# samson6460/tf2_YOLO

Hardware: AMD Instinct MI355X
Metric: images/sec training YOLOv3 416x416 bs=32/GPU (higher is better)
Workload: dtype f32-storage/fp16x2-mfma

## Files before the change

### include/yolo_hip.h

```cpp
#ifndef YOLO_HIP_H_
#define YOLO_HIP_H_

#include <stddef.h>
#include <stdint.h>

#ifdef __cplusplus
extern "C" {
#endif

typedef enum yolo_status {
  YOLO_OK = 0,
  YOLO_ERR_INVALID_ARG = -1,
  YOLO_ERR_LAUNCH = -2,
  YOLO_ERR_WORKSPACE = -3
} yolo_status;

enum { YOLO_ACT_LINEAR = 0, YOLO_ACT_LEAKY = 1, YOLO_ACT_MISH = 2 };
enum { YOLO_HEAD_V3 = 3, YOLO_HEAD_V2 = 2, YOLO_HEAD_V1 = 1, YOLO_HEAD_V4 = 4 };
enum { YOLO_NMS_HARD = 1, YOLO_NMS_SOFT = 2, YOLO_NMS_DIOU = 3 };

const char* yolo_last_error(void);
int yolo_abi_version(void);
int yolo_device_available(void);
int yolo_mfma_probe(const void* operands_f16, float* sink, int workgroups, int iters, double* flops_host, void* stream);
// ... 8 lines not shown
int yolo_set_debug_buffer(void* p, size_t bytes);

typedef struct yolo_conv_desc {
  int N, H, W, Cin;
  int Cout, kh, kw;
  int Ho, Wo;
  int sh, sw;
  int pad_t, pad_l;
} yolo_conv_desc;

#define YOLO_BN_STAT_SLOTS 64
#define YOLO_BN_RED_SLOTS 512
#define YOLO_SPLIT_BATCH_UNITS 4

int yolo_conv2d_fwd(const yolo_conv_desc* d, const float* x, const float* w,
                    const float* bias, float* y, double* stats, void* stream);
int yolo_conv2d_fwd_absmax(const yolo_conv_desc* d, const float* x, const float* w, const float* bias,
                           float* y, double* stats, unsigned* absmax, void* stream);

int yolo_conv2d_dgrad(const yolo_conv_desc* d, const float* dy, const float* wT,
                      float* dx, int accumulate, void* stream);

int yolo_conv2d_wgrad(const yolo_conv_desc* d, const float* x, const float* dy,
                      float* dw, float* dbias, void* stream);

int yolo_conv2d_wgrad_bias(const float* dy, long long P, int Cout, float* dbias, void* stream);

int yolo_filter_transpose(const float* w, float* wT, int Cout, int taps, int Cin, void* stream);

size_t yolo_planes_bytes(long long rows, int C);
int yolo_split_planes(const float* x, long long rows, int C, void* planes, void* stream);
int yolo_split_planes_padded(const float* x, long long rows, int C_src, int C, void* planes, void* stream);

int yolo_split_planes_batch(const void* jobs, int njobs, long long total_blocks, void* stream);
int yolo_filter_transpose_batch(const void* jobs, int njobs, long long total_blocks, void* stream);

int yolo_conv2d_fwd_planes(const yolo_conv_desc* d, const void* x_planes, const void* w_planes,
                           const float* bias, float* y, double* stats, unsigned* absmax, void* stream);
int yolo_conv2d_dgrad_planes(const yolo_conv_desc* d, const void* dy_planes, const void* wT_planes,
                             float* dx, int accumulate, void* stream);
enum { YOLO_EPI_NONE = 0, YOLO_EPI_AFFINE = 1, YOLO_EPI_AFFINE_LEAKY = 2, YOLO_EPI_AFFINE_MISH = 3 };
int yolo_conv2d_fwd_planes_epi(const yolo_conv_desc* d, const void* x_planes, const void* w_planes, const float* bias,
                               int epilogue, const float* scale, const float* shift, const float* residual, float* y,
                               unsigned* absmax, void* stream);
int yolo_split_planes_absmax(const float* x, long long rows, int C, const unsigned* absmax, const float* extra_bound,
                             void* planes, float* out_bound, void* stream);
#define YOLO_INFER_BOUND_WORDS 4096
int yolo_conv_pred_bound(const float* w, int Cout, int kdim, const float* scale, const float* shift, const float* bias,
                         float* pred2, void* stream);
int yolo_conv2d_fwd_infer_unit(const yolo_conv_desc* d, const void* x_planes, const void* w_planes, const float* bias,
                               int epilogue, const float* scale, const float* shift, const float* residual, float* y,
                               unsigned* absmax, const float* pred2, const void* in_bound, int in_n,
                               const void* residual_bound, int residual_n, void* out_planes, unsigned* out_words,
                               float* out_bound, int* out_n_host, void* stream);
int yolo_fold_bound(const void* words, int n, float* out_bound, void* stream);
int yolo_absmax_words(const float* x, long long n, unsigned* words, int* n_words_host, void* stream);
int yolo_stem_filter_prep(const float* w, const float* bias, float* wt, void* stream);
int yolo_stem_fwd_infer_unit(const yolo_conv_desc* d, const float* x, const float* wt, int epilogue, const float* scale,
                             const float* shift, const float* pred2, const void* in_bound, int in_n, float* y,
                             void* out_planes, unsigned* out_words, int* out_n_host, void* stream);
int yolo_split_planes_concat(const float* const* srcs_host, const int* channels_host, const float* const* bounds_host,
                             int nsrc, long long rows, void* planes, float* dst32, float* out_bound, void* stream);
int yolo_split_planes_concat_ex(const float* const* srcs_host, const int* channels_host, const float* const* bounds_host,
                                const int* bound_words_host, const int* upsample_host, int H, int W, int nsrc,
                                long long rows, void* planes, float* dst32, float* out_bound, void* stream);
int yolo_conv2d_fwd_head_unit(const yolo_conv_desc* d, const void* x_planes, const void* w_planes, const float* bias,
                              int A, int C, int version, const float* anchors, float* t, float* y, void* stream);
enum { YOLO_PREC_F32 = 0, YOLO_PREC_F16 = 1 };
int yolo_conv2d_fwd_planes_ex(const yolo_conv_desc* d, const void* x_planes, const void* w_planes, const float* bias,
                              float* y, double* stats, unsigned* absmax, int precision, void* stream);
int yolo_conv2d_fwd_planes_epi_ex(const yolo_conv_desc* d, const void* x_planes, const void* w_planes, const float* bias,
                                  int epilogue, const float* scale, const float* shift, const float* residual, float* y,
                                  unsigned* absmax, int precision, void* stream);
int yolo_conv2d_fwd_infer_unit_ex(const yolo_conv_desc* d, const void* x_planes, const void* w_planes, const float* bias,
                                  int epilogue, const float* scale, const float* shift, const float* residual, float* y,
                                  unsigned* absmax, const float* pred2, const void* in_bound, int in_n,
                                  const void* residual_bound, int residual_n, void* out_planes, unsigned* out_words,
                                  float* out_bound, int* out_n_host, int precision, void* stream);
int yolo_conv2d_fwd_head_unit_ex(const yolo_conv_desc* d, const void* x_planes, const void* w_planes, const float* bias,
                                 int A, int C, int version, const float* anchors, float* t, float* y, int precision,
                                 void* stream);
int yolo_conv2d_wgrad_planes(const yolo_conv_desc* d, const void* x_planes, const void* dy_planes,
                             float* dw, void* stream);

size_t yolo_wgrad_workspace_bytes(void);
int yolo_set_wgrad_workspace(void* p, size_t bytes);


int yolo_bn_stats(const float* x, long long P, int C, double* stats, void* stream);

int yolo_bn_finalize(double* stats, long long P, int C, const float* gamma, const float* beta,
                     float eps, float momentum, int unbiased_moving_var,
                     float* moving_mean, float* moving_var,
                     float* scale, float* shift, float* save_mean, float* save_invstd,
                     void* stream);

int yolo_bn_fold_inference(int C, const float* gamma, const float* beta,
                           const float* moving_mean, const float* moving_var, float eps,
                           float* scale, float* shift, void* stream);

int yolo_bn_act_fwd(const float* x, long long P, int C, const float* scale, const float* shift,
                    int act, const float* residual, float* out, void* stream);

int yolo_bn_act_bwd_reduce(const float* x, const float* dout, long long P, int C,
                           const float* scale, const float* shift,
                           const float* save_mean, const float* save_invstd,
                           int act, double* red, void* stream);
int yolo_bn_act_bwd_apply(const float* x, const float* dout, long long P, int C,
                          const float* gamma, const float* scale, const float* shift,
                          const float* save_mean, const float* save_invstd,
                          int act, double* red, float* dgamma, float* dbeta,
                          float* dx, void* stream);

int yolo_bn_finalize_bound(double* stats, long long P, int C, const float* gamma, const float* beta, float eps,
                           float momentum, int unbiased_moving_var, float* moving_mean, float* moving_var,
                           float* scale, float* shift, float* save_mean, float* save_invstd,
                           const unsigned* absmax, unsigned* bound, void* stream);
int yolo_bn_finalize_offset(double* stats, long long P, int C, const float* gamma, const float* beta, float eps,
                            float momentum, int unbiased_moving_var, float* moving_mean, float* moving_var, float* scale,
                            float* shift, float* save_mean, float* save_invstd, const unsigned* absmax, unsigned* bound,
                            const float* mean_offset, void* stream);
int yolo_bn_infer_bound(int C, const float* scale, const float* shift, const unsigned* absmax,
                        unsigned* bound, void* stream);
int yolo_bn_act_fwd_planes(const float* x, long long P, int C, const float* scale, const float* shift,
                           int act, const float* residual, float* out, void* planes,
                           const unsigned* bn_bound, const float* residual_bound, float* out_bound,
                           void* stream);
int yolo_bn_act_maxpool2x2_fwd(const float* y, int N, int Ho, int Wo, int C, const float* scale, const float* shift,
                               int act, float* out, int* argmax, void* planes, const unsigned* bn_bound,
                               float* out_bound, void* stream);
int yolo_bn_act_fwd_res_planes(const float* x, long long P, int C, const float* scale, const float* shift, int act,
                               const void* residual_planes, float* out, void* planes, const unsigned* bn_bound,
                               float* out_bound, void* stream);
int yolo_bn_act_bwd_reduce_bound(const float* x, const float* dout, long long P, int C, const float* scale,
                                 const float* shift, const float* save_mean, const float* save_invstd,
                                 int act, double* red, unsigned* bound_aux, void* stream);
size_t yolo_stem_bwd_scratch_bytes(void);
int yolo_stem_bn_bwd_wgrad(const yolo_conv_desc* d, const float* y, const float* dout, const float* image, const float* scale,
                           const float* shift, const float* save_mean, const float* save_invstd, int act, const double* red,
                           float* dgamma, float* dbeta, float* dw, void* scratch, size_t scratch_bytes, void* stream);
int yolo_bn_act_bwd_apply_planes(const float* x, const float* dout, long long P, int C, const float* gamma,
                                 const float* scale, const float* shift, const float* save_mean,
                                 const float* save_invstd, int act, double* red, float* dgamma, float* dbeta,
                                 float* dx, void* planes, const unsigned* bound_aux, void* stream);
int yolo_bn_act_bwd_reduce_bound_ld(const float* x, const float* dout, long long ld_dout, long long P, int C,
                                    const float* scale, const float* shift, const float* save_mean,
                                    const float* save_invstd, int act, double* red, unsigned* bound_aux, void* stream);
#define YOLO_BN_FOLD_TICKET_WORDS 36
int yolo_bn_act_bwd_reduce_fold_ld(const float* x, const float* dout, long long ld_dout, long long P, int C,
                                   const float* scale, const float* shift, const float* save_mean,
                                   const float* save_invstd, int act, double* red, unsigned* bound_aux,
                                   unsigned* tickets, void* stream);
int yolo_bn_act_bwd_apply_planes_ld(const float* x, const float* dout, long long ld_dout, long long P, int C,
                                    const float* gamma, const float* scale, const float* shift, const float* save_mean,
                                    const float* save_invstd, int act, double* red, float* dgamma, float* dbeta,
                                    float* dx, void* planes, const unsigned* bound_aux, void* stream);

int yolo_bnred_slots_cap(const yolo_conv_desc* d);
int yolo_conv2d_dgrad_planes_bnred(const yolo_conv_desc* d, const void* dy_planes, const void* wT_planes, float* dx,
                                   int accumulate, const float* y, const float* scale, const float* shift,
                                   const float* save_mean, const float* save_invstd, int act, float* partials,
                                   int slots_cap, unsigned* bound_aux, int* nslots, void* stream);
int yolo_bn_act_bwd_sum_partials(const float* partials, int nslots, long long P, int C, const float* scale, double* red,
                                 unsigned* bound_aux, void* stream);

int yolo_act_fwd(const float* x, long long n, int act, float* out, void* stream);
int yolo_act_bwd(const float* x, const float* dout, long long n, int act, float* dx, void* stream);

int yolo_copy_channels_in(const float* src, long long P, int Csrc, float* dst, int Cdst,
                          int c_off, void* stream);
int yolo_copy_channels_out(const float* src, long long P, int Csrc, int c_off, float* dst,
                           int Cdst, int accumulate, void* stream);
int yolo_upsample2x_fwd(const float* x, int N, int H, int W, int C, float* y, int Cy, int c_off,
                        void* stream);
int yolo_upsample2x_bwd(const float* dy, int N, int H, int W, int C, int Cy, int c_off, float* dx,
                        int accumulate, void* stream);
int yolo_axpy(float* a, const float* b, long long n, void* stream);
int yolo_maxpool_fwd(const float* x, int N, int H, int W, int C, int k, int s, int pad_t, int pad_l,
                     int Ho, int Wo, float* y, int Cy, int c_off, int* argmax, void* stream);
int yolo_maxpool_bwd(const float* dy, int N, int Ho, int Wo, int C, int Cy, int c_off,
                     const int* argmax, float* dx, void* stream);
int yolo_maxpool_bwd_same(const float* dy, int N, int H, int W, int C, int Cy, int c_off, const int* argmax, int k,
                          int pad_t, int pad_l, float* dx, void* stream);
int yolo_maxpool2x2_bwd(const float* dy, int N, int Ho, int Wo, int C, const int* argmax, float* dx, int accumulate,
                        void* stream);
int yolo_space_to_depth2_fwd(const float* x, int N, int H, int W, int C, float* y, int Cy, int c_off,
                             void* stream);
int yolo_space_to_depth2_bwd(const float* dy, int N, int H, int W, int C, int Cy, int c_off, float* dx,
                             int accumulate, void* stream);

int yolo_head_act_fwd(const float* t, long long P, int A, int C, int version,
                      const float* anchors, float* y, void* stream);
int yolo_head_act_bwd(const float* y, const float* dy, long long P, int A, int C, int version,
                      const float* anchors, float* dt, float* danchors, void* stream);

typedef struct yolo_loss_cfg {
  int version;
  int N, gh, gw, A, C;
  float anchors[32];
  int   use_anchors;
  float binary_weight;
  float loss_weight[4];
  float ignore_thresh;
  int   use_focal_loss;
  float focal_gamma;
  int   use_scale;
  float wh_reg_weight;
  float truth_thresh;
  float label_smooth;
} yolo_loss_cfg;

size_t yolo_loss_workspace_bytes(const yolo_loss_cfg* cfg);
int yolo_loss_fwd_bwd(const yolo_loss_cfg* cfg, const float* y_true, const float* y_pred,
                      double* loss_out, float* dpred, float grad_scale,
                      void* workspace, size_t workspace_bytes, void* stream);

int yolo_metrics(const yolo_loss_cfg* cfg, const float* y_true, const float* y_pred,
                 float recall_thresh, double* out, void* stream);

int yolo_adam_step(float* p, float* g, float* m, float* v, long long n, float lr, float beta1,
                   float beta2, float eps, int step, float grad_scale, int zero_grad, void* stream);
float yolo_adam_lr_t(float lr, float beta1, float beta2, int step);
int yolo_adam_step_dev(float* p, float* g, float* m, float* v, long long n, const float* hyper, int zero_grad, void* stream);
int yolo_sgd_step(float* p, float* g, long long n, float lr, float grad_scale, int zero_grad,
                  void* stream);
int yolo_fill(float* p, long long n, float value, void* stream);

size_t yolo_grad_sqnorm_workspace_bytes(int n_chunks);
int yolo_grad_sqnorm(const float* g, const long long* chunk_off, const int* chunk_len, int n_chunks,
                     const int* var_first, int n_vars, double* var_sq, double* total_sq, void* workspace,
                     size_t workspace_bytes, void* stream);
int yolo_clip_factors(const double* var_sq, int n_vars, const double* total_sq, const double* total_sq_extra,
                      const float* hyper, int mode, float* factors, float* norm_out, void* stream);
int yolo_adam_step_clip(float* p, float* g, float* m, float* v, float* vhat, const long long* chunk_off,
                        const int* chunk_len, const int* chunk_var, int n_chunks, const float* hyper,
                        const float* factors, int clip_mode, int zero_grad, void* stream);
int yolo_sgd_step_clip(float* p, float* g, float* accum, int nesterov, const long long* chunk_off,
                       const int* chunk_len, const int* chunk_var, int n_chunks, const float* hyper,
                       const float* factors, int clip_mode, int zero_grad, void* stream);

int yolo_decode_level(const float* pred, int gh, int gw, int A, int C, int version,
                      float threshold, double* rows_out, int max_rows, int* count,
                      void* workspace, size_t workspace_bytes, void* stream);
int yolo_decode_level_f64(const double* pred, int gh, int gw, int A, int C, int version,
                          double threshold, double* rows_out, int max_rows, int* count,
                          void* workspace, size_t workspace_bytes, void* stream);
size_t yolo_decode_workspace_bytes(int gh, int gw, int A, int C);

size_t yolo_nms_workspace_bytes(int n, int class_num);
int yolo_nms(const double* rows, int n, int class_num, int mode, double nms_threshold,
             double conf_threshold, double sigma, unsigned char* keep_out,
             void* workspace, size_t workspace_bytes, void* stream);
int yolo_nms_select(const double* rows, int n, int class_num, int mode, double nms_threshold, double conf_threshold,
                    double sigma, unsigned char* keep_out, double* rows_out, int* count_out, void* workspace,
                    size_t workspace_bytes, void* stream);

int yolo_cal_iou(const void* xywh_true, const void* xywh_pred, void* out, void* out2, int is_f64, int mode, int ndim,
                 const long long* shape_host, const long long* true_strides_host, const long long* pred_strides_host,
                 double grid_w, double grid_h, void* stream);


int yolo_match_detections(const double* gt_rows, int ngt, const double* det_rows, int ndet, int class_num,
                          double iou_threshold, int* best_gt, unsigned char* matched, double* best_iou,
                          unsigned char* gt_flags, long long* class_counts, void* stream);

int yolo_rank_desc(const double* key, const int* segment, int n, int* rank, void* stream);

size_t yolo_pr_curve_workspace_bytes(int n, int num_gts);
int yolo_pr_curve(const double* joint, const int* gt_id, const unsigned char* matched, int n, int num_gts,
                  int precision_mode, void* workspace, size_t workspace_bytes, double* precision,
                  double* recall, void* stream);

int yolo_allreduce_bucket(void* rccl_comm, float* grads, long long count, void* stream);

int yolo_encode_labels(const double* boxes, const int* cls, const int* first, int N, double img_h, double img_w,
                       int gh, int gw, int C, double* label64, float* label32, void* stream);
int yolo_down2xlabel(const double* label_in, int N, int gh, int gw, int ch, double* label_out, float* out32,
                     void* stream);

#ifdef __cplusplus
}
#endif
#endif
```

### tf2_yolo_amd/_lib.py

```python
import ctypes
import os
from ctypes import (POINTER, Structure, c_char_p, c_double, c_float, c_int, c_longlong,
                    c_size_t, c_void_p)

from . import tape as _tape

_HERE = os.path.dirname(os.path.abspath(__file__))
LIB_PATH = os.path.join(_HERE, "libyolo_hip.so")

ACT_LINEAR, ACT_LEAKY, ACT_MISH = 0, 1, 2
PREC_F32, PREC_F16 = 0, 1
_PRECISIONS = {"fp32": PREC_F32, "fp16": PREC_F16}


def precision_enum(precision):
    try:
        return _PRECISIONS[precision]
    except (KeyError, TypeError):
        raise ValueError(f"precision must be 'fp32' or 'fp16', got {precision!r}") from None
NMS_HARD, NMS_SOFT, NMS_DIOU = 1, 2, 3


class YoloHipError(RuntimeError):
    pass


class ConvDesc(Structure):
    _fields_ = [(n, c_int) for n in
                ("N", "H", "W", "Cin", "Cout", "kh", "kw", "Ho", "Wo", "sh", "sw", "pad_t", "pad_l")]


class LossCfg(Structure):
    _fields_ = [("version", c_int), ("N", c_int), ("gh", c_int), ("gw", c_int), ("A", c_int),
                ("C", c_int), ("anchors", c_float * 32), ("use_anchors", c_int),
                ("binary_weight", c_float), ("loss_weight", c_float * 4),
                ("ignore_thresh", c_float), ("use_focal_loss", c_int), ("focal_gamma", c_float),
                ("use_scale", c_int), ("wh_reg_weight", c_float), ("truth_thresh", c_float),
                ("label_smooth", c_float)]


_P = c_void_p
_LL = c_longlong
SIGNATURES = {
    "yolo_last_error": (c_char_p, []),
    "yolo_abi_version": (c_int, []),
    "yolo_device_available": (c_int, []),
    "yolo_set_option": (c_int, [c_int, c_int]),
    "yolo_last_conv_kernel": (c_char_p, [POINTER(c_int)]),
    "yolo_mfma_probe": (c_int, [_P, _P, c_int, c_int, POINTER(c_double), _P]),
    "yolo_set_debug_buffer": (c_int, [_P, c_size_t]),
    "yolo_encode_labels": (c_int, [_P, _P, _P, c_int, c_double, c_double, c_int, c_int, c_int, _P, _P, _P]),
    "yolo_down2xlabel": (c_int, [_P, c_int, c_int, c_int, c_int, _P, _P, _P]),
    "yolo_conv_workspace_bytes": (c_size_t, []),
    "yolo_set_conv_workspace": (c_int, [_P, c_size_t, _P]),
    "yolo_conv2d_fwd": (c_int, [POINTER(ConvDesc), _P, _P, _P, _P, _P, _P]),
    "yolo_conv2d_dgrad": (c_int, [POINTER(ConvDesc), _P, _P, _P, c_int, _P]),
    "yolo_conv2d_wgrad": (c_int, [POINTER(ConvDesc), _P, _P, _P, _P, _P]),
    "yolo_conv2d_wgrad_bias": (c_int, [_P, _LL, c_int, _P, _P]),
    "yolo_filter_transpose": (c_int, [_P, _P, c_int, c_int, c_int, _P]),
    "yolo_planes_bytes": (c_size_t, [_LL, c_int]),
    "yolo_split_planes": (c_int, [_P, _LL, c_int, _P, _P]),
    "yolo_split_planes_padded": (c_int, [_P, _LL, c_int, c_int, _P, _P]),
    "yolo_split_planes_batch": (c_int, [_P, c_int, _LL, _P]),
    "yolo_filter_transpose_batch": (c_int, [_P, c_int, _LL, _P]),
    "yolo_conv2d_fwd_planes": (c_int, [POINTER(ConvDesc), _P, _P, _P, _P, _P, _P, _P]),
    "yolo_stem_bwd_scratch_bytes": (c_size_t, []),
    "yolo_stem_bn_bwd_wgrad": (c_int, [POINTER(ConvDesc), _P, _P, _P, _P, _P, _P, _P, c_int, _P, _P, _P, _P, _P, c_size_t, _P]),
    "yolo_conv2d_fwd_planes_epi": (c_int, [POINTER(ConvDesc), _P, _P, _P, c_int, _P, _P, _P, _P, _P, _P]),
    "yolo_split_planes_absmax": (c_int, [_P, _LL, c_int, _P, _P, _P, _P, _P]),
    "yolo_conv_pred_bound": (c_int, [_P, c_int, c_int, _P, _P, _P, _P, _P]),
    "yolo_conv2d_fwd_infer_unit": (c_int, [POINTER(ConvDesc), _P, _P, _P, c_int, _P, _P, _P, _P, _P, _P, _P, c_int, _P, c_int,
                                           _P, _P, _P, POINTER(c_int), _P]),
    "yolo_fold_bound": (c_int, [_P, c_int, _P, _P]),
    "yolo_absmax_words": (c_int, [_P, _LL, _P, POINTER(c_int), _P]),
    "yolo_stem_filter_prep": (c_int, [_P, _P, _P, _P]),
    "yolo_stem_fwd_infer_unit": (c_int, [POINTER(ConvDesc), _P, _P, c_int, _P, _P, _P, _P, c_int, _P, _P, _P, POINTER(c_int), _P]),
    "yolo_split_planes_concat": (c_int, [POINTER(c_void_p), POINTER(c_int), POINTER(c_void_p), c_int, _LL, _P, _P, _P, _P]),
    "yolo_split_planes_concat_ex": (c_int, [POINTER(c_void_p), POINTER(c_int), POINTER(c_void_p), POINTER(c_int), POINTER(c_int),
                                            c_int, c_int, c_int, _LL, _P, _P, _P, _P]),
    "yolo_conv2d_fwd_head_unit": (c_int, [POINTER(ConvDesc), _P, _P, _P, c_int, c_int, c_int, _P, _P, _P, _P]),
    "yolo_conv2d_fwd_planes_ex": (c_int, [POINTER(ConvDesc), _P, _P, _P, _P, _P, _P, c_int, _P]),
    "yolo_conv2d_fwd_planes_epi_ex": (c_int, [POINTER(ConvDesc), _P, _P, _P, c_int, _P, _P, _P, _P, _P, c_int, _P]),
    "yolo_conv2d_fwd_infer_unit_ex": (c_int, [POINTER(ConvDesc), _P, _P, _P, c_int, _P, _P, _P, _P, _P, _P, _P, c_int, _P, c_int,
                                              _P, _P, _P, POINTER(c_int), c_int, _P]),
    "yolo_conv2d_fwd_head_unit_ex": (c_int, [POINTER(ConvDesc), _P, _P, _P, c_int, c_int, c_int, _P, _P, _P, c_int, _P]),
    "yolo_conv2d_fwd_absmax": (c_int, [POINTER(ConvDesc), _P, _P, _P, _P, _P, _P, _P]),
    "yolo_conv2d_dgrad_planes": (c_int, [POINTER(ConvDesc), _P, _P, _P, c_int, _P]),
    "yolo_conv2d_wgrad_planes": (c_int, [POINTER(ConvDesc), _P, _P, _P, _P]),
    "yolo_wgrad_workspace_bytes": (c_size_t, []),
    "yolo_set_wgrad_workspace": (c_int, [_P, c_size_t]),
    "yolo_bn_stats": (c_int, [_P, _LL, c_int, _P, _P]),
    "yolo_bn_finalize": (c_int, [_P, _LL, c_int, _P, _P, c_float, c_float, c_int, _P, _P, _P, _P, _P, _P, _P]),
    "yolo_bn_fold_inference": (c_int, [c_int, _P, _P, _P, _P, c_float, _P, _P, _P]),
    "yolo_bn_act_fwd": (c_int, [_P, _LL, c_int, _P, _P, c_int, _P, _P, _P]),
    "yolo_bn_act_bwd_reduce": (c_int, [_P, _P, _LL, c_int, _P, _P, _P, _P, c_int, _P, _P]),
    "yolo_bn_act_bwd_apply": (c_int, [_P, _P, _LL, c_int, _P, _P, _P, _P, _P, c_int, _P, _P, _P, _P, _P]),
    "yolo_bn_act_fwd_planes": (c_int, [_P, _LL, c_int, _P, _P, c_int, _P, _P, _P, _P, _P, _P, _P]),
    "yolo_bn_act_fwd_res_planes": (c_int, [_P, _LL, c_int, _P, _P, c_int, _P, _P, _P, _P, _P, _P]),
    "yolo_bn_act_bwd_apply_planes": (c_int, [_P, _P, _LL, c_int, _P, _P, _P, _P, _P, c_int, _P, _P, _P, _P, _P, _P,
                                             _P]),
    "yolo_bn_infer_bound": (c_int, [c_int, _P, _P, _P, _P, _P]),
    "yolo_bn_finalize_bound": (c_int, [_P, _LL, c_int, _P, _P, c_float, c_float, c_int, _P, _P, _P, _P, _P, _P, _P,
                                       _P, _P]),
    "yolo_bn_finalize_offset": (c_int, [_P, _LL, c_int, _P, _P, c_float, c_float, c_int, _P, _P, _P, _P, _P, _P, _P,
                                        _P, _P, _P]),
    "yolo_bn_act_bwd_reduce_bound": (c_int, [_P, _P, _LL, c_int, _P, _P, _P, _P, c_int, _P, _P, _P]),
    "yolo_bn_act_bwd_reduce_bound_ld": (c_int, [_P, _P, _LL, _LL, c_int, _P, _P, _P, _P, c_int, _P, _P, _P]),
    "yolo_bn_act_bwd_reduce_fold_ld": (c_int, [_P, _P, _LL, _LL, c_int, _P, _P, _P, _P, c_int, _P, _P, _P, _P]),
    "yolo_bn_act_bwd_apply_planes_ld": (c_int, [_P, _P, _LL, _LL, c_int, _P, _P, _P, _P, _P, c_int, _P, _P, _P, _P, _P, _P,
                                                _P]),
    "yolo_bnred_slots_cap": (c_int, [POINTER(ConvDesc)]),
    "yolo_conv2d_dgrad_planes_bnred": (c_int, [POINTER(ConvDesc), _P, _P, _P, c_int, _P, _P, _P, _P, _P, c_int, _P, c_int, _P,
                                               POINTER(c_int), _P]),
    "yolo_bn_act_bwd_sum_partials": (c_int, [_P, c_int, _LL, c_int, _P, _P, _P, _P]),
    "yolo_allreduce_bucket": (c_int, [_P, _P, _LL, _P]),
    "yolo_act_fwd": (c_int, [_P, _LL, c_int, _P, _P]),
    "yolo_act_bwd": (c_int, [_P, _P, _LL, c_int, _P, _P]),
    "yolo_copy_channels_in": (c_int, [_P, _LL, c_int, _P, c_int, c_int, _P]),
    "yolo_copy_channels_out": (c_int, [_P, _LL, c_int, c_int, _P, c_int, c_int, _P]),
    "yolo_upsample2x_fwd": (c_int, [_P, c_int, c_int, c_int, c_int, _P, c_int, c_int, _P]),
    "yolo_upsample2x_bwd": (c_int, [_P, c_int, c_int, c_int, c_int, c_int, c_int, _P, c_int, _P]),
    "yolo_axpy": (c_int, [_P, _P, _LL, _P]),
    "yolo_maxpool_fwd": (c_int, [_P, c_int, c_int, c_int, c_int, c_int, c_int, c_int, c_int, c_int, c_int,
                                 _P, c_int, c_int, _P, _P]),
    "yolo_maxpool_bwd": (c_int, [_P, c_int, c_int, c_int, c_int, c_int, c_int, _P, _P, _P]),
    "yolo_maxpool2x2_bwd": (c_int, [_P, c_int, c_int, c_int, c_int, _P, _P, c_int, _P]),
    "yolo_bn_act_maxpool2x2_fwd": (c_int, [_P, c_int, c_int, c_int, c_int, _P, _P, c_int, _P, _P, _P, _P, _P, _P]),
    "yolo_maxpool_bwd_same": (c_int, [_P, c_int, c_int, c_int, c_int, c_int, c_int, _P, c_int, c_int, c_int, _P, _P]),
    "yolo_space_to_depth2_fwd": (c_int, [_P, c_int, c_int, c_int, c_int, _P, c_int, c_int, _P]),
    "yolo_space_to_depth2_bwd": (c_int, [_P, c_int, c_int, c_int, c_int, c_int, c_int, _P, c_int, _P]),
    "yolo_head_act_fwd": (c_int, [_P, _LL, c_int, c_int, c_int, _P, _P, _P]),
    "yolo_head_act_bwd": (c_int, [_P, _P, _LL, c_int, c_int, c_int, _P, _P, _P, _P]),
    "yolo_loss_workspace_bytes": (c_size_t, [POINTER(LossCfg)]),
    "yolo_loss_fwd_bwd": (c_int, [POINTER(LossCfg), _P, _P, _P, _P, c_float, _P, c_size_t, _P]),
    "yolo_metrics": (c_int, [POINTER(LossCfg), _P, _P, c_float, _P, _P]),
    "yolo_adam_step": (c_int, [_P, _P, _P, _P, _LL, c_float, c_float, c_float, c_float, c_int, c_float, c_int, _P]),
    "yolo_adam_lr_t": (c_float, [c_float, c_float, c_float, c_int]),
    "yolo_adam_step_dev": (c_int, [_P, _P, _P, _P, _LL, _P, c_int, _P]),
    "yolo_sgd_step": (c_int, [_P, _P, _LL, c_float, c_float, c_int, _P]),
    "yolo_fill": (c_int, [_P, _LL, c_float, _P]),
    "yolo_grad_sqnorm_workspace_bytes": (c_size_t, [c_int]),
    "yolo_grad_sqnorm": (c_int, [_P, _P, _P, c_int, _P, c_int, _P, _P, _P, c_size_t, _P]),
    "yolo_clip_factors": (c_int, [_P, c_int, _P, _P, _P, c_int, _P, _P, _P]),
    "yolo_adam_step_clip": (c_int, [_P, _P, _P, _P, _P, _P, _P, _P, c_int, _P, _P, c_int, c_int, _P]),
    "yolo_sgd_step_clip": (c_int, [_P, _P, _P, c_int, _P, _P, _P, c_int, _P, _P, c_int, c_int, _P]),
    "yolo_decode_level": (c_int, [_P, c_int, c_int, c_int, c_int, c_int, c_float, _P, c_int, _P, _P, c_size_t, _P]),
    "yolo_decode_level_f64": (c_int, [_P, c_int, c_int, c_int, c_int, c_int, c_double, _P, c_int, _P, _P,
                                      c_size_t, _P]),
    "yolo_decode_workspace_bytes": (c_size_t, [c_int, c_int, c_int, c_int]),
    "yolo_nms_workspace_bytes": (c_size_t, [c_int, c_int]),
    "yolo_cal_iou": (c_int, [_P, _P, _P, _P, c_int, c_int, c_int, POINTER(c_longlong), POINTER(c_longlong),
                             POINTER(c_longlong), c_double, c_double, _P]),
    "yolo_match_detections": (c_int, [_P, c_int, _P, c_int, c_int, c_double, _P, _P, _P, _P, _P, _P]),
    "yolo_rank_desc": (c_int, [_P, _P, c_int, _P, _P]),
    "yolo_pr_curve_workspace_bytes": (c_size_t, [c_int, c_int]),
    "yolo_pr_curve": (c_int, [_P, _P, _P, c_int, c_int, c_int, _P, c_size_t, _P, _P, _P]),
    "yolo_nms": (c_int, [_P, c_int, c_int, c_int, c_double, c_double, c_double, _P, _P, c_size_t, _P]),
    "yolo_nms_select": (c_int, [_P, c_int, c_int, c_int, c_double, c_double, c_double, _P, _P, _P, _P, c_size_t, _P]),
}

_lib = None

_QUERIES = {"yolo_last_error", "yolo_last_conv_kernel", "yolo_abi_version", "yolo_bnred_slots_cap", "yolo_device_available", "yolo_conv_workspace_bytes", "yolo_planes_bytes",
            "yolo_stem_bwd_scratch_bytes", "yolo_loss_workspace_bytes", "yolo_decode_workspace_bytes",
            "yolo_nms_workspace_bytes", "yolo_pr_curve_workspace_bytes", "yolo_wgrad_workspace_bytes", "yolo_adam_lr_t",
            "yolo_grad_sqnorm_workspace_bytes",
            "yolo_set_option", "yolo_set_debug_buffer", "yolo_set_conv_workspace", "yolo_set_wgrad_workspace"}


class _Recorded:
    __slots__ = ("f", "name")
# ... 53 lines not shown
```

### tf2_yolo_amd/capture.py

```python
import torch

from ._lib import YoloHipError


_LEAKED = []


class _StaticInputs:

    def __init__(self, x, y_list):
        self.x = x.clone()
        self.ys = [y.clone() for y in y_list]
        self._last = [(x, x._version)] + [(y, y._version) for y in y_list]

    def load(self, x, y_list):
        for i, (dst, src) in enumerate(zip([self.x] + self.ys, [x] + list(y_list))):
            last, ver = self._last[i]
            if src is last and src._version == ver:
                continue
            dst.copy_(src, non_blocking=True)
            self._last[i] = (src, src._version)


class StepGraphs:

    def __init__(self, model, x, y_list):
        self.model = model
        self.key = self.key_of(model, x)
        net = model.net
        opt = model.optimizer
        if not getattr(opt, "capturable", False):
            raise YoloHipError("this optimizer has no capturable form")
        self.inputs = _StaticInputs(x, y_list)
        self.x, self.ys = self.inputs.x, self.inputs.ys
        self.segments = []
        opt._hyper_buffers()
        net.mark_params_changed()
        torch.cuda.synchronize()
        self._capture(net, opt)

    @staticmethod
    def key_of(model, x):
        return (tuple(x.shape), getattr(model.net, "alloc_gen", 0), tuple(id(l) for l in model.loss), id(model.optimizer),
                id(model._reducer), model.net.anchors_trainable)

    def _capture(self, net, opt):
        model = self.model
        red = model._reducer if (model._reducer is not None and model._reducer.active) else None
        pool = torch.cuda.graph_pool_handle()
        stream = torch.cuda.Stream()
        stream.wait_stream(torch.cuda.current_stream())
        state = {"g": None}

        def begin():
            g = torch.cuda.CUDAGraph()
            g.capture_begin(pool=pool, capture_error_mode="thread_local")
            state["g"] = g

        def end(action):
            state["g"].capture_end()
            self.segments.append((state["g"], action))
            state["g"] = None

        net._dyp_events = [None, None]
        net._wp_event = net._wT_event = None
        old_hook, old_overlap = net.grad_ready_hook, net._overlap_wgrad
        net._overlap_wgrad = False
        if red is not None:
            index = model._dp_unit_index

            def cut_hook(u):
                for b in red.closes[index[id(u)]]:
                    net._join_wgrad()
                    net._dyp_events = [None, None]
                    end(("reduce", b))
                    begin()
            net.grad_ready_hook = cut_hook
        try:
            with torch.cuda.stream(stream):
                begin()
                outs = net.forward(self.x, training=True)
                for i, (o, yt) in enumerate(zip(outs, self.ys)):
                    model.loss[i].fwd_bwd(yt, o, grad_scale=1.0, dpred=model._dpred[i], loss_out=model._loss_bufs[i])
                net.backward(model._dpred)
                net._dyp_events = [None, None]
                if red is not None:
                    end(("finish",))
                    begin()
                opt.step_captured()
                end(None)
        except Exception:
            _LEAKED.extend(g for g, _ in self.segments)
            if state["g"] is not None:
                _LEAKED.append(state["g"])
                try:
                    if net._wgrad_stream is not None:
                        torch.cuda.current_stream().wait_stream(net._wgrad_stream)
                    state["g"].capture_end()
                except Exception:
                    pass
            self.segments = []
            net._dyp_events = [None, None]
            net._wp_event = net._wT_event = None
            net._wgrad_pending = False
            raise
        finally:
            net.grad_ready_hook = old_hook
            net._overlap_wgrad = old_overlap
        torch.cuda.current_stream().wait_stream(stream)
        net.mark_params_changed()

    def replay(self, x, y_list):
        model, net, opt = self.model, self.model.net, self.model.optimizer
        red = model._reducer if (model._reducer is not None and model._reducer.active) else None
        self.inputs.load(x, y_list)
        opt.refresh_hyper(grad_scale=(1.0 / red.world) if red is not None else 1.0)
        for g, action in self.segments:
            g.replay()
            if action is None:
                continue
            if action[0] == "reduce":
                red.reduce_bucket(action[1])
            else:
                if net.anchors_trainable and red.world > 1:
                    import torch.distributed as dist
                    dist.all_reduce(net.anchor_grads, group=red.pg)
                red.finish()
        net.mark_params_changed()
        return model._loss_bufs


class StepTape:

    def __init__(self, model, x, y_list):
        from . import tape as tape_mod
        self.model = model
        self.key = StepGraphs.key_of(model, x)
        opt, net = model.optimizer, model.net
        if not getattr(opt, "capturable", False):
            raise YoloHipError("this optimizer has no capturable form")
        self.inputs = _StaticInputs(x, y_list)
        self.x, self.ys = self.inputs.x, self.inputs.ys
        opt._hyper_buffers()
        red = model._reducer if (model._reducer is not None and model._reducer.active) else None
        net._dyp_events = [None, None]
        net.mark_params_changed()
        self.tape = tape_mod.Tape()
        opt.refresh_hyper(grad_scale=(1.0 / red.world) if red is not None else 1.0)
        tape_mod.ACTIVE = self.tape
        try:
            outs = net.forward(self.x, training=True)
            for i, (o, yt) in enumerate(zip(outs, self.ys)):
                model.loss[i].fwd_bwd(yt, o, grad_scale=1.0, dpred=model._dpred[i], loss_out=model._loss_bufs[i])
            net.backward(model._dpred)
            if red is not None:
                if net.anchors_trainable and red.world > 1:
                    import torch.distributed as dist
                    tape_mod.host_call(lambda: dist.all_reduce(net.anchor_grads, group=red.pg))
                tape_mod.host_call(red.finish)
            opt.step_captured()
        finally:
            tape_mod.ACTIVE = None
        net.mark_params_changed()

    def replay(self, x, y_list):
        model, net, opt = self.model, self.model.net, self.model.optimizer
        red = model._reducer if (model._reducer is not None and model._reducer.active) else None
        self.inputs.load(x, y_list)
        opt.refresh_hyper(grad_scale=(1.0 / red.world) if red is not None else 1.0)
        self.tape.replay()
        net.mark_params_changed()
        return model._loss_bufs
```

### tf2_yolo_amd/csrc/conv.hip

```cpp
#include "conv_args.hpp"
#include <cstdlib>
#include <type_traits>

namespace yolo {

template <int BM, int BN, int WGM, int WGN, bool FLAT>
__global__ __launch_bounds__(256) void gather_conv_kernel(const GatherConvArgs a) {
  constexpr int BK = 32;
  constexpr int LD = BK + 4;
  constexpr int TM = BM / WGM / 32;
  constexpr int TN = BN / WGN / 32;
  constexpr int AR = BM / 32;
  constexpr int BR = BN / 32;
  static_assert(WGM * WGN == 4, "4 waves per block");
  static_assert(TM >= 1 && TN >= 1, "wave tile");

  extern __shared__ __attribute__((aligned(16))) float smem[];
  constexpr int BUF = (BM + BN) * LD;

  const int tid = threadIdx.x;
  const int lane = tid & 63;
  const int wave = tid >> 6;
  const int wm = wave / WGN, wn = wave % WGN;

// ... 1161 lines not shown
          a.taps[nt++] = Tap{ty / d->sh, tx / d->sw, (r * d->kw + s) * d->Cout};
        }
      }
      a.ntaps = nt;
      if (nt == 0) {
        if (!accumulate) {
          a.ntaps = 1;
          a.taps[0] = Tap{-(1 << 20), -(1 << 20), 0};
        } else {
          continue;
        }
      }
      if (planes) {
        YOLO_REQUIRE(gather_planes_supported(a), "conv_dgrad_planes: needs Cout %% 16 == 0 and Cin >= 32");
        set_bnred(a, bnred);
        if (int rc = launch_gather_planes(a, as_stream(stream))) return rc;
        if (bnred != nullptr) bnred->nslots = a.bwd_nslots;
      } else if (int rc = dispatch_gather(a, flat, as_stream(stream))) {
        return rc;
      }
    }
  }
  return YOLO_OK;
}

extern "C" int yolo_conv2d_dgrad(const yolo_conv_desc* d, const float* dy, const float* wT, float* dx, int accumulate,
                                 void* stream) {
  return dgrad_impl(d, dy, wT, dx, accumulate, stream, false);
}

extern "C" int yolo_conv2d_dgrad_planes(const yolo_conv_desc* d, const void* dy_planes, const void* wT_planes, float* dx,
                                        int accumulate, void* stream) {
  return dgrad_impl(d, reinterpret_cast<const float*>(dy_planes), reinterpret_cast<const float*>(wT_planes), dx,
                    accumulate, stream, true);
}

extern "C" int yolo_bnred_slots_cap(const yolo_conv_desc* d) {
  if (d == nullptr) return 0;
  const long long px = (long long)d->N * d->H * d->W;
  const long long cap = px / 64 + 2LL * d->N + 64;
  return cap > 0x7fffffffLL ? 0 : (int)cap;
}

extern "C" int yolo_conv2d_dgrad_planes_bnred(const yolo_conv_desc* d, const void* dy_planes, const void* wT_planes, float* dx,
                                              int accumulate, const float* y, const float* scale, const float* shift,
                                              const float* save_mean, const float* save_invstd, int act, float* partials,
                                              int slots_cap, unsigned* bound_aux, int* nslots, void* stream) {
  YOLO_REQUIRE(d && y && scale && shift && save_mean && save_invstd && partials && nslots && slots_cap > 0,
               "conv_dgrad_planes_bnred: bad args");
  YOLO_REQUIRE(d->Cin % 4 == 0, "conv_dgrad_planes_bnred: Cin=%d must be a multiple of 4", d->Cin);
  YOLO_REQUIRE(act >= 0 && act <= 2, "conv_dgrad_planes_bnred: bad activation %d", act);
  BnRedArgs b{y, scale, shift, save_mean, save_invstd, act, partials, slots_cap, bound_aux, 0};
  const int rc = dgrad_impl(d, reinterpret_cast<const float*>(dy_planes), reinterpret_cast<const float*>(wT_planes), dx,
                            accumulate, stream, true, &b);
  *nslots = b.nslots;
  return rc;
}

static void fill_wgrad_args(const yolo_conv_desc* d, WgradArgs& a) {
  a.N = d->N; a.Hs = d->H; a.Ws = d->W; a.Cs = d->Cin;
  a.Hg = d->Ho; a.Wg = d->Wo;
  a.sy = d->sh; a.sx = d->sw;
  a.Cout = d->Cout;
  a.ldw = d->kh * d->kw * d->Cin;
  a.ntaps = d->kh * d->kw;
  a.kw = d->kw; a.pad_t = d->pad_t; a.pad_l = d->pad_l;
  a.M = (long long)d->N * d->Ho * d->Wo;
}

extern "C" int yolo_conv2d_wgrad_planes(const yolo_conv_desc* d, const void* x_planes, const void* dy_planes, float* dw,
                                        void* stream) {
  if (int rc = validate_desc(d)) return rc;
  YOLO_REQUIRE(x_planes && dy_planes && dw, "conv_wgrad_planes: null pointer");
  WgradArgs a{};
  a.src = reinterpret_cast<const float*>(x_planes);
  a.dy = reinterpret_cast<const float*>(dy_planes);
  a.dw = dw;
  fill_wgrad_args(d, a);
  YOLO_REQUIRE(wgrad_planes_supported(a),
               "conv_wgrad_planes: needs Cin %% 16 == 0, Cout %% 16 == 0, Cout >= 32 and kh*kw*Cin >= 64");
  return launch_wgrad_planes(a, as_stream(stream));
}

extern "C" int yolo_conv2d_wgrad(const yolo_conv_desc* d, const float* x, const float* dy, float* dw, float* dbias,
                                 void* stream) {
  if (int rc = validate_desc(d)) return rc;
  YOLO_REQUIRE(x && dy && dw, "conv_wgrad: null pointer");
  WgradArgs a{};
  a.src = x;
  a.dy = dy;
  a.dw = dw;
  fill_wgrad_args(d, a);
  const bool ascalar = (d->Cout % 4) != 0;
  const bool bflat = (d->Cin % 4) != 0;
  int rc;
  hipStream_t st = as_stream(stream);
  if (g_conv_mode == 1 && wgrad_split_supported(a)) rc = launch_wgrad_split(a, st);
  else if (ascalar && bflat) rc = dispatch_wgrad<true, true>(a, st);
  else if (ascalar) rc = dispatch_wgrad<true, false>(a, st);
  else if (bflat) rc = dispatch_wgrad<false, true>(a, st);
  else rc = dispatch_wgrad<false, false>(a, st);
  if (rc) return rc;
  if (dbias != nullptr) return yolo_conv2d_wgrad_bias(dy, a.M, d->Cout, dbias, stream);
  return YOLO_OK;
}

extern "C" int yolo_conv2d_wgrad_bias(const float* dy, long long P, int Cout, float* dbias, void* stream) {
  YOLO_REQUIRE(dy && dbias && P > 0 && Cout > 0, "conv_wgrad_bias: bad args");
  int cw = 32;
  while (cw < Cout && cw < 256) cw <<= 1;
  dim3 block(cw, 256 / cw);
  const int gy = (Cout + cw - 1) / cw;
  long long gx = (P + block.y * 64 - 1) / (block.y * 64);
  if (gx > 1024) gx = 1024;
  if (gx < 1) gx = 1;
  size_t ws_bytes = 0;
  float* part = reinterpret_cast<float*>(wgrad_workspace(&ws_bytes));
  if (part != nullptr) {
    const long long cap = (long long)(WGRAD_WS_COLSUM_BYTES / 4) / ((long long)block.y * Cout);
    if (cap < 1) part = nullptr;
    else if (gx > cap) gx = cap;
  }
  hipLaunchKernelGGL(colsum_kernel, dim3((unsigned)gx, gy), block, 0, as_stream(stream), dy, P, Cout, dbias, part);
  if (int rc = check_launch("colsum_kernel")) return rc;
  if (part != nullptr) {
    hipLaunchKernelGGL(colsum_finish_kernel, dim3((Cout + 63) / 64), dim3(64, 16), 0, as_stream(stream), part,
                       (int)(gx * block.y), Cout, dbias);
    return check_launch("colsum_finish_kernel");
  }
  return YOLO_OK;
}

extern "C" int yolo_filter_transpose(const float* w, float* wT, int Cout, int taps, int Cin, void* stream) {
  YOLO_REQUIRE(w && wT && Cout > 0 && taps > 0 && Cin > 0, "filter_transpose: bad args");
  dim3 grid((Cin + 31) / 32, (Cout + 31) / 32, taps);
  hipLaunchKernelGGL(filter_transpose_kernel, grid, dim3(256), 0, as_stream(stream), w, wT, Cout, taps, Cin);
  return check_launch("filter_transpose_kernel");
}
```

### tf2_yolo_amd/csrc/conv_args.hpp

```cpp
#pragma once
#include "common.hpp"

namespace yolo {

constexpr int MAX_TAPS = 49;

struct Tap {
  int oy, ox, woff;
};

struct ClassGeom {
  long long M;
  int Hg, Wg, ooy, oox, tap0, ntaps;
};

struct GatherConvArgs {
  const float* src;
  const float* wgt;
  const float* bias;
  float* dst;
  double* stats;
  unsigned* absmax;
  long long M;
  int N, Hs, Ws, Cs;
  int Hg, Wg;
  int sy, sx;
  int Hd, Wd, Cd;
  int osy, osx, ooy, oox;
  int Cout, ldw;
  int ntaps, accumulate;
  int kw, pad_t, pad_l;
  int tiles_n;
  int nblocks;
  unsigned src_bytes, wgt_bytes;
  int zero_blk_src, zero_blk_wgt;
  int nt_store;
  int vec_store;
  int kc;
  int dbg;
  int one_pass;
  const float* epi_scale;
  const float* epi_shift;
  const float* epi_res;
  int epi_act;
  unsigned char* out_planes;
  const float* pl_pred;
  const unsigned* pl_in_bound;
  const unsigned* pl_res_bound;
  int pl_in_n, pl_res_n;
  unsigned* pl_out_words;
  float* head_y;
  const float* head_anchors;
  int head_A, head_C;
  int sk_grid;
  int tile_order;
  float* sk_slabs;
  unsigned* sk_tickets;
  int split_parts;
  int ncls;
  ClassGeom cls[4];
  unsigned long long* stamps;
  const float* bwd_y;
  const float* bwd_scale;
  const float* bwd_shift;
  const float* bwd_mean;
  const float* bwd_invstd;
  float* bwd_part;
  unsigned* bwd_aux;
  int bwd_act;
  int bwd_nslots;
  int bwd_cap;
  Tap taps[MAX_TAPS];
};

#define YOLO_BNRED_CHECK(a)                                                                                          \
  if ((a).bwd_y != nullptr && (a).bwd_nslots > (a).bwd_cap) {                                                        \
    set_error("conv_dgrad(bn reduce): %d partial slots needed, room for %d", (a).bwd_nslots, (a).bwd_cap);           \
    return YOLO_ERR_INVALID_ARG;                                                                                     \
  }

__device__ __forceinline__ int xcd_remap(int bid, int nblocks) {
  const int xcd = bid & 7, idx = bid >> 3;
  const int q = nblocks >> 3, r = nblocks & 7;
  const int start = (xcd < r) ? xcd * (q + 1) : r * (q + 1) + (xcd - r) * q;
  return start + idx;
}


struct WgradArgs {
  const float* src;
  const float* dy;
  float* dw;
  long long M;
  int N, Hs, Ws, Cs;
  int Hg, Wg;
  int sy, sx;
  int Cout, ldw;
  int ntaps;
  int kw, pad_t, pad_l;
  int tiles_co, tiles_j;
  int nblocks;
  long long chunk;
  unsigned src_bytes, dy_bytes;
  int zero_blk_src, zero_blk_dy;
  float* slabs;
  int splits;
};

int launch_gather_split(GatherConvArgs& a, hipStream_t st);
bool gather_split_supported(const GatherConvArgs& a);
long long planes_bytes(long long rows, int C);
int launch_split_planes(const float* x, long long rows, int C, void* planes, hipStream_t st);
int launch_split_planes_absmax(const float* x, long long rows, int C, const unsigned* absmax, const float* extra_bound, int extra_n,
                               void* planes, float* out_bound, hipStream_t st);
int launch_split_planes_concat(const float* const* xs, const int* Cs, const float* const* bounds, int nsrc, long long rows,
                               void* planes, float* dst32, float* out_bound, hipStream_t st,
                               const int* bound_words = nullptr, const int* upsample = nullptr, int H = 0, int W = 0);
int launch_split_planes_padded(const float* x, long long rows, int Csrc, int C, void* planes, hipStream_t st);
int launch_split_planes_batch(const void* jobs, int njobs, long long total_blocks, hipStream_t st);
int launch_filter_transpose_batch(const void* jobs, int njobs, long long total_blocks, hipStream_t st);
int launch_gather_planes(GatherConvArgs& a, hipStream_t st);
bool conv_small_supported(const GatherConvArgs& a);
bool conv_small_head_supported(const GatherConvArgs& a);
int launch_conv_small(GatherConvArgs& a, hipStream_t st, int* nwg);
bool gather_planes_supported(const GatherConvArgs& a);
int conv_split_parts(const GatherConvArgs& a, long long nb, int bm, int min_cb, int idle_div);
int launch_split_reduce(GatherConvArgs& a, int bm, hipStream_t st);
float* conv_split_slabs();
int launch_conv_win(GatherConvArgs& a, int variant, hipStream_t st);
bool conv_win_supported(const GatherConvArgs& a);
enum { OPT_CONV_WIN = 0, OPT_STAMPS = 1, OPT_CONV_SK = 2, OPT_DBG = 3, OPT_TILE_ORDER = 4, OPT_CONV_PATCH = 5, OPT_WGRAD_WIN = 6, OPT_NMS_WALK = 7, OPT_EXP = 8, OPT_COUNT = 16 };
int set_conv_workspace(void* p, size_t bytes, hipStream_t st);
extern void* g_dbg_buf;
extern size_t g_dbg_bytes;
extern int g_opt[OPT_COUNT];
void init_options();
void note_conv_launch(const char* family, int a = 0, int b = 0, int c = 0, int d = 0);
int launch_wgrad_planes(WgradArgs& a, hipStream_t st);
bool wgrad_planes_supported(const WgradArgs& a);
int launch_wgrad_win(WgradArgs& a, hipStream_t st);
bool wgrad_win_supported(const WgradArgs& a);
constexpr size_t WGRAD_WS_COLSUM_BYTES = 1 << 20;
void* wgrad_workspace(size_t* bytes);
bool stem_fwd_supported(const yolo_conv_desc* d);
struct StemEpiArgs {
  const float* scale;
  const float* shift;
  int act;
  void* planes;
  const float* pred;
  const unsigned* in_words;
  int in_n;
  unsigned* out_words;
};
bool stem_infer_supported(const yolo_conv_desc* d);
int launch_stem_filter_prep(const float* w, const float* bias, float* wt, hipStream_t st);
int launch_absmax_words(const float* x, long long n, unsigned* words, int* n_words, hipStream_t st);
int launch_stem_infer(const yolo_conv_desc* d, const float* x, const float* wt, float* y, const StemEpiArgs& e, int* out_n,
                      hipStream_t st);
size_t stem_bwd_scratch_bytes();
int launch_stem_bn_bwd_wgrad(const yolo_conv_desc* d, const float* y, const float* dout, const float* img, const float* scale,
                             const float* shift, const float* smean, const float* sinv, int act, const double* redsum,
                             float* dgamma, float* dbeta, float* dw, float* scratch, size_t scratch_bytes, hipStream_t st);
int launch_stem_fwd(const yolo_conv_desc* d, const float* x, const float* w, const float* bias, float* y, double* stats,
                    unsigned* absmax, hipStream_t st);
int launch_wgrad_split(WgradArgs& a, hipStream_t st);
bool wgrad_split_supported(const WgradArgs& a);

}
```

### tf2_yolo_amd/csrc/conv_wgrad_planes.hip

```cpp
#include "planes.hpp"
#include <type_traits>
#include <cstdlib>

namespace yolo {

typedef short s16x4 __attribute__((ext_vector_type(4)));
typedef short s16x8 __attribute__((ext_vector_type(8)));

template <int BM, int BN, int WGM, int WGN, int NB = 3, int KO = 0>
__global__ __launch_bounds__(64 * WGM * WGN, (NB * (BM / 32 + BN / 32) * PL_PLANES * 1024 > 80 * 1024 ? 1 : 2)) void wgrad_planes_kernel(const WgradArgs a) {
  constexpr int NW = WGM * WGN;
  constexpr int TM = BM / WGM / 32;
  constexpr int TN = BN / WGN / 32;
  constexpr int RBA = BM / 32, RBB = BN / 32;
  constexpr int STAGE_BYTES = (RBA + RBB) * PL_PLANES * 1024;
  constexpr int NBUF = NB;

  extern __shared__ __attribute__((aligned(16))) unsigned char smem[];
  const unsigned lds_base = (unsigned)(size_t)smem;

  const int tid = threadIdx.x;
  const int lane = tid & 63;
  const int wave = __builtin_amdgcn_readfirstlane(tid >> 6);
  const int wm = wave / WGN, wn = wave % WGN;

  const int lid = xcd_remap(blockIdx.x, a.nblocks);
  const int tiles = a.tiles_co * a.tiles_j;
  const int split = lid / tiles;
  const int tile = lid - split * tiles;
  const int tile_co = tile % a.tiles_co;
  const int j0 = (tile / a.tiles_co) * BN;
  const int co0 = tile_co * BM;
  const long long p_begin = (long long)split * a.chunk;
  long long p_end = p_begin + a.chunk;
  if (p_end > a.M) p_end = a.M;
  if (p_begin >= p_end) return;
  const int nk = (int)((p_end - p_begin + 15) / 16);
  const int Ktot = a.ntaps * a.Cs;

  constexpr bool BOTH = (RBA + RBB > NW);
  constexpr int NA = BOTH ? RBA / NW : 1, NQ = BOTH ? RBB / NW : 1;
  static_assert(!BOTH || (RBA % NW == 0 && RBB % NW == 0), "loader layout");
  constexpr int ND = PL_PLANES * (BOTH ? NA + NQ : 1);
  const bool hasA = BOTH || wave < RBA, hasB = BOTH || wave >= RBA;
  const int lpix = 4 * (lane >> 4) + (lane & 3);
  const int lsb = (lane >> 2) & 3;
  const unsigned strideA = (unsigned)((a.Cout >> 4) * PL_RECORD);
  const unsigned strideB = (unsigned)((a.Cs >> 4) * PL_RECORD);
  const unsigned zeroA = (unsigned)a.zero_blk_dy * strideA, zeroB = (unsigned)a.zero_blk_src * strideB;
  const i32x4 rsrcA = planes_rsrc(a.dy, a.dy_bytes), rsrcB = planes_rsrc(a.src, a.src_bytes);
  unsigned ldsA[NA], ldsB[NQ];

  bool okA[NA], okB[NQ];
  unsigned voffA[NA], voffB[NQ];
  int b_oy[NQ], b_ox[NQ], b_chan[NQ];
  int pn = 0, py = 0, px = 0;
  long long pcur = p_begin + lpix;
#pragma unroll
  for (int i = 0; i < NA; ++i) {
    const int rb = BOTH ? wave + i * NW : wave;
    ldsA[i] = lds_base + rb * PL_PLANES * 1024;
    okA[i] = false;
    voffA[i] = zeroA;
    if (hasA) {
      const int co16 = ((co0 + rb * 32) >> 4) + (lsb >> 1);
      okA[i] = co16 * 16 < a.Cout;
      voffA[i] = okA[i] ? (unsigned)(p_begin >> 4) * strideA + (unsigned)co16 * PL_RECORD + (lsb & 1) * 256 + lpix * 16 : zeroA;
    }
  }
#pragma unroll
  for (int i = 0; i < NQ; ++i) {
    const int rb = BOTH ? wave + i * NW : (wave - RBA) % RBB;
    ldsB[i] = lds_base + (RBA + rb) * PL_PLANES * 1024;
    okB[i] = false;
    voffB[i] = zeroB;
    b_oy[i] = b_ox[i] = b_chan[i] = 0;
    if (hasB) {
      const int j16 = ((j0 + rb * 32) >> 4) + (lsb >> 1);
      okB[i] = j16 * 16 < Ktot;
      const int cpt = a.Cs >> 4;
      const int t = okB[i] ? j16 / cpt : 0;
      const int r = t / a.kw;
      b_oy[i] = r - a.pad_t;
// ... 131 lines not shown
    asm volatile("s_waitcnt lgkmcnt(0)" ::: "memory");
    __builtin_amdgcn_s_barrier();
    read_frags(rbuf, NXT);
    __builtin_amdgcn_sched_barrier(0);
    mfma_stage(CUR, wbuf);
  };
  {
    int rbuf = 1, wbuf = 0;
    int kt = 0;
    for (; kt + 1 < nk; kt += 2) {
      step(rbuf, wbuf, S0{}, S1{});
      rbuf = (rbuf + 1 == NBUF) ? 0 : rbuf + 1;
      wbuf = (wbuf + 1 == NBUF) ? 0 : wbuf + 1;
      step(rbuf, wbuf, S1{}, S0{});
      rbuf = (rbuf + 1 == NBUF) ? 0 : rbuf + 1;
      wbuf = (wbuf + 1 == NBUF) ? 0 : wbuf + 1;
    }
    if (kt < nk) step(rbuf, wbuf, S0{}, S1{});
  }
  asm volatile("s_waitcnt vmcnt(0)" ::: "memory");

  const float unscale =
      reinterpret_cast<const float*>(reinterpret_cast<const unsigned char*>(a.dy) + a.dy_bytes - PL_HEADER)[2] *
      reinterpret_cast<const float*>(reinterpret_cast<const unsigned char*>(a.src) + a.src_bytes - PL_HEADER)[2];
  if (a.slabs != nullptr) {
    float* mine = a.slabs + (size_t)lid * (BM * BN);
#pragma unroll
    for (int i = 0; i < TM; ++i)
#pragma unroll
      for (int j = 0; j < TN; ++j)
#pragma unroll
        for (int q4 = 0; q4 < 4; ++q4) {
          const f32x4 f = {acc[i][j][4 * q4], acc[i][j][4 * q4 + 1], acc[i][j][4 * q4 + 2], acc[i][j][4 * q4 + 3]};
          *reinterpret_cast<f32x4*>(mine + ((((wave * TM + i) * TN + j) * 4 + q4) * 64 + lane) * 4) = f;
        }
    return;
  }
#pragma unroll
  for (int j = 0; j < TN; ++j) {
    const int cj = j0 + (wn * TN + j) * 32 + (lane & 31);
    const bool cok = cj < Ktot;
#pragma unroll
    for (int i = 0; i < TM; ++i) {
#pragma unroll
      for (int r = 0; r < 16; ++r) {
        const int co = co0 + (wm * TM + i) * 32 + (r & 3) + 8 * (r >> 2) + 4 * (lane >> 5);
        if (cok && co < a.Cout) atomicAdd(&a.dw[(long long)co * a.ldw + cj], acc[i][j][r] * unscale);
      }
    }
  }
}

template <int BM, int BN, int WGM, int WGN>
__global__ __launch_bounds__(256) void wgrad_reduce_kernel(const WgradArgs a) {
  constexpr int TM = BM / WGM / 32, TN = BN / WGN / 32;
  constexpr int PER_TILE = BM * BN / 4;
  const int tiles = a.tiles_co * a.tiles_j;
  const long long idx = (long long)blockIdx.x * 256 + threadIdx.x;
  const int tile = (int)(idx / PER_TILE);
  if (tile >= tiles) return;
  const int q = (int)(idx - (long long)tile * PER_TILE);
  const int lane = q & 63, piece = q >> 6;
  const int q4 = piece & 3, j = (piece >> 2) % TN, i = (piece / (4 * TN)) % TM, wave = piece / (4 * TN * TM);
  const int wm = wave / WGN, wn = wave % WGN;
  const int co0 = (tile % a.tiles_co) * BM, j0 = (tile / a.tiles_co) * BN;
  const int cj = j0 + (wn * TN + j) * 32 + (lane & 31);
  const int co = co0 + (wm * TM + i) * 32 + 8 * q4 + 4 * (lane >> 5);
  if (cj >= a.ntaps * a.Cs || co >= a.Cout) return;
  const f32x4* sl = reinterpret_cast<const f32x4*>(a.slabs) + (size_t)tile * PER_TILE + q;
  const size_t sstride = (size_t)tiles * PER_TILE;
  f32x4 t = {0.f, 0.f, 0.f, 0.f};
  int s = 0;
  for (; s + 8 <= a.splits; s += 8) {
    f32x4 v[8];
#pragma unroll
    for (int u = 0; u < 8; ++u) v[u] = __builtin_nontemporal_load(sl + (size_t)(s + u) * sstride);
#pragma unroll
    for (int u = 0; u < 8; ++u) t = t + v[u];
  }
  for (; s < a.splits; ++s) t = t + __builtin_nontemporal_load(sl + (size_t)s * sstride);
  const float unscale =
      reinterpret_cast<const float*>(reinterpret_cast<const unsigned char*>(a.dy) + a.dy_bytes - PL_HEADER)[2] *
      reinterpret_cast<const float*>(reinterpret_cast<const unsigned char*>(a.src) + a.src_bytes - PL_HEADER)[2];
#pragma unroll
  for (int e = 0; e < 4; ++e)
    if (co + e < a.Cout) a.dw[(long long)(co + e) * a.ldw + cj] += t[e] * unscale;
}

static void* g_wgrad_ws = nullptr;
static size_t g_wgrad_ws_bytes = 0;
void* wgrad_workspace(size_t* bytes) {
  if (bytes != nullptr) *bytes = g_wgrad_ws_bytes;
  return g_wgrad_ws;
}

template <int BM, int BN, int WGM, int WGN, int NB = 3, int KO = 0>
static int launch_wp(WgradArgs& a, hipStream_t st) {
  a.tiles_co = (a.Cout + BM - 1) / BM;
  const int cols = a.ntaps * a.Cs;
  a.tiles_j = (cols + BN - 1) / BN;
  const long long tiles = (long long)a.tiles_co * a.tiles_j;
  static const long long target_env = env_ll("YOLO_WGRAD_TARGET", 0LL);
  constexpr size_t lds = NB * (BM / 32 + BN / 32) * PL_PLANES * 1024;
  constexpr auto kernel = &wgrad_planes_kernel<BM, BN, WGM, WGN, NB, KO>;
  int resident = resident_workgroups<kernel, lds>(64 * WGM * WGN, "wgrad_planes_kernel");
  if (resident <= 0) resident = 512;
  static const long long target_1x1_env = env_ll("YOLO_WGRAD_TARGET_1X1", 0LL);
  long long target = a.ntaps == 1 ? (target_1x1_env > 0 ? target_1x1_env : 256)
                                  : (target_env > 0 ? target_env : 1024);
  if (target_env <= 0 && a.ntaps > 1) {
    const long long s1 = resident / tiles, s2 = 2LL * resident / tiles;
    if (s1 >= 1 && tiles * s1 * 10 >= 7LL * resident) target = tiles * s1;
    else if (s2 >= 1 && tiles * s2 * 10 >= 17LL * resident) target = tiles * s2;
  }
  long long splits = target / tiles > 0 ? (target_env > 0 || a.ntaps == 1 ? (target + tiles - 1) / tiles : target / tiles) : 1;
  const long long max_splits = (a.M + 255) / 256;
  if (splits > max_splits) splits = max_splits;
  if (splits > 65535) splits = 65535;
  if (splits < 1) splits = 1;
  a.slabs = nullptr;
  static const bool det_env = env_int("YOLO_WGRAD_DETERMINISTIC", 1) != 0;
  if (det_env && g_wgrad_ws != nullptr && g_wgrad_ws_bytes > WGRAD_WS_COLSUM_BYTES) {
    const long long cap = (long long)((g_wgrad_ws_bytes - WGRAD_WS_COLSUM_BYTES) / ((size_t)BM * BN * 4));
    if (cap >= tiles) {
      if (tiles * splits > cap) splits = cap / tiles;
      a.slabs = reinterpret_cast<float*>(reinterpret_cast<unsigned char*>(g_wgrad_ws) + WGRAD_WS_COLSUM_BYTES);
    }
  }
  long long chunk = (a.M + splits - 1) / splits;
  chunk = (chunk + 15) / 16 * 16;
  splits = (a.M + chunk - 1) / chunk;
  a.chunk = chunk;
  a.splits = (int)splits;
  if (tiles * splits > 0x7fffffffLL || splits > 65535) {
    set_error("wgrad(planes): bad grid %lld x %lld", tiles, splits);
    return YOLO_ERR_INVALID_ARG;
  }
  a.nblocks = (int)(tiles * splits);
  note_conv_launch("wgrad_planes_kernel<%d,%d,%d,%d>", BM, BN, WGM, WGN);
  if (int rc = launch_lds<kernel, lds>(dim3((unsigned)(tiles * splits)), dim3(64 * WGM * WGN), st, a, "wgrad_planes_kernel")) return rc;
  if (a.slabs != nullptr) {
    const long long pieces = tiles * (BM * BN / 4);
    hipLaunchKernelGGL((wgrad_reduce_kernel<BM, BN, WGM, WGN>), dim3((unsigned)((pieces + 255) / 256)), dim3(256), 0, st, a);
    return check_launch("wgrad_reduce_kernel");
  }
  return YOLO_OK;
}

bool wgrad_planes_supported(const WgradArgs& a) {
  return (a.Cout % 16) == 0 && (a.Cs % 16) == 0 && a.Cout >= 32 && a.ntaps * a.Cs >= 64;
}

int launch_wgrad_planes(WgradArgs& a, hipStream_t st) {
  const long long rowsX = (long long)a.N * a.Hs * a.Ws;
  const long long bytesX = planes_bytes(rowsX, a.Cs), bytesDy = planes_bytes(a.M, a.Cout);
  if (bytesX >= (1LL << 32) || bytesDy >= (1LL << 32)) {
    set_error("wgrad(planes): operand planes exceed 4 GiB (%lld, %lld bytes)", bytesX, bytesDy);
    return YOLO_ERR_INVALID_ARG;
  }
  a.src_bytes = (unsigned)bytesX;
  a.dy_bytes = (unsigned)bytesDy;
  a.zero_blk_src = (int)((rowsX + 15) / 16);
  a.zero_blk_dy = (int)((a.M + 15) / 16);
  const int cols = a.ntaps * a.Cs;
  init_options();
  if (g_opt[OPT_WGRAD_WIN] != 0 && wgrad_win_supported(a)) {
// ... 36 lines not shown
```

### tf2_yolo_amd/csrc/conv_wgrad_win.hip

```cpp
#include "planes.hpp"
#include <cstdlib>

namespace yolo {

typedef short ws16x4 __attribute__((ext_vector_type(4)));
typedef short ws16x8 __attribute__((ext_vector_type(8)));

constexpr int WW_CO = 128;
constexpr int WW_CI = 32;
constexpr int WW_STAGE_PX = 32;
constexpr int WW_TILE_FLOATS = WW_CO * 9 * WW_CI;

template <int RING, int KO = 0, int PF = 1>
__global__ __launch_bounds__(256, 2) void wgrad_win_kernel(const WgradArgs a) {
  constexpr int A_STAGE = 2 * 4 * PL_PLANES * 1024;
  constexpr int WIN_PLANE = RING * 64 + 64;
  constexpr int WIN_OFF = 2 * A_STAGE;
  constexpr unsigned RMASK = RING * 64 - 1;
  constexpr unsigned ZSLOT = RING * 64;

  extern __shared__ __attribute__((aligned(16))) unsigned char smem[];
  const unsigned lds_base = (unsigned)(size_t)smem;

  const int tid = threadIdx.x;
  const int lane = tid & 63;
  const int wave = __builtin_amdgcn_readfirstlane(tid >> 6);

  const int lid = xcd_remap(blockIdx.x, a.nblocks);
  const int tiles = a.tiles_co * a.tiles_j;
  const int split = lid / tiles;
  const int tile = lid - split * tiles;
  const int co0 = (tile % a.tiles_co) * WW_CO;
  const int ci0 = (tile / a.tiles_co) * WW_CI;
  const int p_begin = (int)((long long)split * a.chunk);
  int p_end = p_begin + (int)a.chunk;
  if (p_end > (int)a.M) p_end = (int)a.M;
  if (p_begin >= p_end) return;
  const int nst = (p_end - p_begin + WW_STAGE_PX - 1) / WW_STAGE_PX;
  const int W = a.Ws, H = a.Hs, M = (int)a.M;

  if (tid < 32) reinterpret_cast<unsigned*>(smem + WIN_OFF + (tid >> 4) * WIN_PLANE + ZSLOT)[tid & 15] = 0u;

  const unsigned strideA = (unsigned)((a.Cout >> 4) * PL_RECORD);
  const unsigned strideB = (unsigned)((a.Cs >> 4) * PL_RECORD);
  const unsigned zeroA = (unsigned)a.zero_blk_dy * strideA, zeroB = (unsigned)a.zero_blk_src * strideB;
  const i32x4 rsrcA = planes_rsrc(a.dy, a.dy_bytes), rsrcB = planes_rsrc(a.src, a.src_bytes);
  const int lpix = 4 * (lane >> 4) + (lane & 3), lsb = (lane >> 2) & 3;
  const unsigned a_lane = (unsigned)(((co0 + wave * 32) >> 4) + (lsb >> 1)) * PL_RECORD + (lsb & 1) * 256 + lpix * 16;
  auto issue_A = [&](int stage, int buf) {
#pragma unroll
    for (int j = 0; j < 2; ++j) {
      const int pb16 = p_begin + stage * WW_STAGE_PX + j * 16;
      const unsigned v = (pb16 < p_end) ? (unsigned)(pb16 >> 4) * strideA + a_lane : zeroA;
#pragma unroll
      for (int p = 0; p < PL_PLANES; ++p) {
        const unsigned l = __builtin_amdgcn_readfirstlane(lds_base + buf * A_STAGE + ((j * 4 + wave) * PL_PLANES + p) * 1024);
        dma16(rsrcA, v, (unsigned)(p * 512), l);
      }
    }
  };
  const int bpx = lane >> 2, bch = lane & 3;
  const unsigned b_lane = (unsigned)((ci0 >> 4) + (bch >> 1)) * PL_RECORD + (bch & 1) * 256;
  auto issue_B = [&](int P0, int plane) {
    const int P = P0 + bpx;
    const unsigned v = ((unsigned)P < (unsigned)M) ? (unsigned)(P >> 4) * strideB + b_lane + (P & 15) * 16 : zeroB;
    const unsigned l = __builtin_amdgcn_readfirstlane(lds_base + WIN_OFF + plane * WIN_PLANE + (unsigned)((P0 & (RING - 1)) * 64));
    dma16(rsrcB, v, (unsigned)(plane * 512), l);
  };

  const int lo = (p_begin - W - 1) & ~15;
  const int Lbase = (p_begin + W + 33 + 15) & ~15;
  {
    const int npieces = ((Lbase - lo) >> 4) * PL_PLANES;
    for (int idx = wave; idx < npieces; idx += 4) issue_B(lo + (idx >> 1) * 16, idx & 1);
  }
  issue_A(0, 0);

  const int grp = lane >> 4, i16 = lane & 15;
  const int qq = i16 >> 2, pq = i16 & 3;
  const int tr_off = ((2 * (grp >> 1)) * 16 + ((grp & 1) * 2 + (pq >> 1)) * 4 + qq) * 16 + (pq & 1) * 8;
  const unsigned lc = (unsigned)((2 * (grp & 1) + (pq >> 1)) * 16 + (pq & 1) * 8);
  typedef ws16x4 __attribute__((address_space(3))) * lds_p;
  unsigned pb[2][2];
// ... 328 lines not shown
            x -= W;
            ++y;
          }
          if (y >= H) y -= H;
          px[jj][r] = x;
          py[jj][r] = y;
        }
        __builtin_amdgcn_sched_barrier(0);
      }
    }
    asm volatile("s_waitcnt vmcnt(0)" ::: "memory");
    asm volatile("s_waitcnt lgkmcnt(0)" ::: "memory");
    __builtin_amdgcn_s_barrier();
  }

  if (half == 1) {
#pragma unroll
    for (int t = 0; t < 9; ++t)
#pragma unroll
      for (int q4 = 0; q4 < 4; ++q4) {
        const f32x4 f = {acc[t][4 * q4], acc[t][4 * q4 + 1], acc[t][4 * q4 + 2], acc[t][4 * q4 + 3]};
        *reinterpret_cast<f32x4*>(smem + ((((wave * 9 + t) * 4 + q4) * 64 + lane) * 16)) = f;
      }
  }
  __syncthreads();
  if (half == 1) return;
  if (a.slabs != nullptr) {
    float* mine = a.slabs + (size_t)lid * WW_TILE_FLOATS;
#pragma unroll
    for (int t = 0; t < 9; ++t)
#pragma unroll
      for (int q4 = 0; q4 < 4; ++q4) {
        const f32x4 u = *reinterpret_cast<const f32x4*>(smem + ((((wave * 9 + t) * 4 + q4) * 64 + lane) * 16));
        const f32x4 f = {acc[t][4 * q4] + u[0], acc[t][4 * q4 + 1] + u[1], acc[t][4 * q4 + 2] + u[2], acc[t][4 * q4 + 3] + u[3]};
        *reinterpret_cast<f32x4*>(mine + (((wave * 9 + t) * 4 + q4) * 64 + lane) * 4) = f;
      }
    return;
  }
  const float unscale =
      reinterpret_cast<const float*>(reinterpret_cast<const unsigned char*>(a.dy) + a.dy_bytes - PL_HEADER)[2] *
      reinterpret_cast<const float*>(reinterpret_cast<const unsigned char*>(a.src) + a.src_bytes - PL_HEADER)[2];
#pragma unroll
  for (int t = 0; t < 9; ++t) {
    const long long cj = (long long)t * a.Cs + ci0 + (lane & 31);
#pragma unroll
    for (int q4 = 0; q4 < 4; ++q4) {
      const f32x4 u = *reinterpret_cast<const f32x4*>(smem + ((((wave * 9 + t) * 4 + q4) * 64 + lane) * 16));
#pragma unroll
      for (int e = 0; e < 4; ++e) {
        const int r = 4 * q4 + e;
        const int co = co0 + wave * 32 + (r & 3) + 8 * (r >> 2) + 4 * (lane >> 5);
        atomicAdd(&a.dw[(long long)co * a.ldw + cj], (acc[t][r] + u[e]) * unscale);
      }
    }
  }
}

__global__ __launch_bounds__(256) void wgrad_win_reduce_kernel(const WgradArgs a) {
  constexpr int PER_TILE = WW_TILE_FLOATS / 4;
  const int tiles = a.tiles_co * a.tiles_j;
  const long long idx = (long long)blockIdx.x * 256 + threadIdx.x;
  const int tile = (int)(idx / PER_TILE);
  if (tile >= tiles) return;
  const int q = (int)(idx - (long long)tile * PER_TILE);
  const int lane = q & 63, piece = q >> 6;
  const int q4 = piece & 3, t = (piece >> 2) % 9, wave = piece / 36;
  const int co = (tile % a.tiles_co) * WW_CO + wave * 32 + 8 * q4 + 4 * (lane >> 5);
  const long long cj = (long long)t * a.Cs + (tile / a.tiles_co) * WW_CI + (lane & 31);
  const f32x4* sl = reinterpret_cast<const f32x4*>(a.slabs) + (size_t)tile * PER_TILE + q;
  const size_t sstride = (size_t)tiles * PER_TILE;
  f32x4 sum = {0.f, 0.f, 0.f, 0.f};
  int s = 0;
  for (; s + 8 <= a.splits; s += 8) {
    f32x4 v[8];
#pragma unroll
    for (int u = 0; u < 8; ++u) v[u] = __builtin_nontemporal_load(sl + (size_t)(s + u) * sstride);
#pragma unroll
    for (int u = 0; u < 8; ++u) sum = sum + v[u];
  }
  for (; s < a.splits; ++s) sum = sum + __builtin_nontemporal_load(sl + (size_t)s * sstride);
  const float unscale =
      reinterpret_cast<const float*>(reinterpret_cast<const unsigned char*>(a.dy) + a.dy_bytes - PL_HEADER)[2] *
      reinterpret_cast<const float*>(reinterpret_cast<const unsigned char*>(a.src) + a.src_bytes - PL_HEADER)[2];
#pragma unroll
  for (int e = 0; e < 4; ++e) a.dw[(long long)(co + e) * a.ldw + cj] += sum[e] * unscale;
}


template <int RING, int KO = 0>
__global__ __launch_bounds__(256, 2) void wgrad_win16_kernel(const WgradArgs a) {
  constexpr int A_STAGE = 2 * 4 * PL_PLANES * 1024;
  constexpr int WIN_PLANE = RING * 64 + 64;
  constexpr int WIN_OFF = 2 * A_STAGE;
  constexpr unsigned RMASK = RING * 64 - 1;
  constexpr unsigned ZSLOT = RING * 64;

  extern __shared__ __attribute__((aligned(16))) unsigned char smem[];
  const unsigned lds_base = (unsigned)(size_t)smem;
  const int tid = threadIdx.x;
  const int lane = tid & 63;
  const int wave = __builtin_amdgcn_readfirstlane(tid >> 6);
  const int lid = xcd_remap(blockIdx.x, a.nblocks);
  const int tiles = a.tiles_co * a.tiles_j;
  const int split = lid / tiles;
  const int tile = lid - split * tiles;
  const int co0 = (tile % a.tiles_co) * WW_CO;
  const int ci0 = (tile / a.tiles_co) * WW_CI;
  const int p_begin = (int)((long long)split * a.chunk);
  int p_end = p_begin + (int)a.chunk;
  if (p_end > (int)a.M) p_end = (int)a.M;
  if (p_begin >= p_end) return;
  const int nst = (p_end - p_begin + WW_STAGE_PX - 1) / WW_STAGE_PX;
  const int W = a.Ws, H = a.Hs, M = (int)a.M;
  if (tid < 32) reinterpret_cast<unsigned*>(smem + WIN_OFF + (tid >> 4) * WIN_PLANE + ZSLOT)[tid & 15] = 0u;

  const unsigned strideA = (unsigned)((a.Cout >> 4) * PL_RECORD);
  const unsigned strideB = (unsigned)((a.Cs >> 4) * PL_RECORD);
  const unsigned zeroA = (unsigned)a.zero_blk_dy * strideA, zeroB = (unsigned)a.zero_blk_src * strideB;
  const i32x4 rsrcA = planes_rsrc(a.dy, a.dy_bytes), rsrcB = planes_rsrc(a.src, a.src_bytes);
  const int lq = lane >> 4, lpix = 4 * lq + (lane & 3), lsb = ((lane >> 2) & 3) ^ (2 * (lq >> 1));
  const unsigned a_lane = (unsigned)(((co0 + wave * 32) >> 4) + (lsb >> 1)) * PL_RECORD + (lsb & 1) * 256 + lpix * 16;
  auto issue_A = [&](int stage, int buf) {
#pragma unroll
    for (int j = 0; j < 2; ++j) {
      const int pb16 = p_begin + stage * WW_STAGE_PX + j * 16;
      const unsigned v = (pb16 < p_end) ? (unsigned)(pb16 >> 4) * strideA + a_lane : zeroA;
#pragma unroll
      for (int p = 0; p < PL_PLANES; ++p) {
        const unsigned l = __builtin_amdgcn_readfirstlane(lds_base + buf * A_STAGE + ((j * 4 + wave) * PL_PLANES + p) * 1024);
        dma16(rsrcA, v, (unsigned)(p * 512), l);
      }
    }
  };
  const int bpx = lane >> 2, bch = (lane & 3) ^ (2 * (bpx >> 3));
  const unsigned b_lane = (unsigned)((ci0 >> 4) + (bch >> 1)) * PL_RECORD + (bch & 1) * 256;
  auto issue_B = [&](int P0, int plane) {
    const int P = P0 + bpx;
    const unsigned v = ((unsigned)P < (unsigned)M) ? (unsigned)(P >> 4) * strideB + b_lane + (P & 15) * 16 : zeroB;
    const unsigned l = __builtin_amdgcn_readfirstlane(lds_base + WIN_OFF + plane * WIN_PLANE + (unsigned)((P0 & (RING - 1)) * 64));
    dma16(rsrcB, v, (unsigned)(plane * 512), l);
  };
  const int lo = (p_begin - W - 1) & ~15;
  const int Lbase = (p_begin + W + 33 + 15) & ~15;
  {
    const int npieces = ((Lbase - lo) >> 4) * PL_PLANES;
    for (int idx = wave; idx < npieces; idx += 4) issue_B(lo + (idx >> 1) * 16, idx & 1);
  }
  issue_A(0, 0);

  const int grp = lane >> 4, i16 = lane & 15;
  const int qq = i16 >> 2, pq = i16 & 3;
  typedef ws16x4 __attribute__((address_space(3))) * lds_p;
  auto rd_pair = [&](unsigned a0, unsigned a1, int off) -> f16x8 {
    const ws16x4 v0 = __builtin_amdgcn_ds_read_tr16_b64_v4i16((lds_p)(size_t)(a0 + off));
    const ws16x4 v1 = __builtin_amdgcn_ds_read_tr16_b64_v4i16((lds_p)(size_t)(a1 + off));
    const ws16x8 v = {v0[0], v0[1], v0[2], v0[3], v1[0], v1[1], v1[2], v1[3]};
    return __builtin_bit_cast(f16x8, v);
  };
  unsigned abase[2];
#pragma unroll
  for (int m = 0; m < 2; ++m)
    abase[m] = (unsigned)((grp >> 1) * 4 * PL_PLANES * 1024 + wave * PL_PLANES * 1024 + 512 * (grp & 1) +
                          64 * ((2 * m + (pq >> 1)) ^ (2 * (grp & 1))) + 16 * qq + 8 * (pq & 1));
  const unsigned lc = (unsigned)((pq >> 1) * 16 + (pq & 1) * 8);
  unsigned pb[2];
  int px[2], py[2];
// ... 88 lines not shown
      if (hf == 0 && t + 1 < 9) calc(t + 1, adt[(t + 1) & 1]);
      __builtin_amdgcn_sched_barrier(0);
      if constexpr (!(KO & 4)) {
        acc[t][hf][0] = __builtin_amdgcn_mfma_f32_16x16x32_f16(ah[0], bh[cur], acc[t][hf][0], 0, 0, 0);
        acc[t][hf][1] = __builtin_amdgcn_mfma_f32_16x16x32_f16(ah[1], bh[cur], acc[t][hf][1], 0, 0, 0);
      }
      __builtin_amdgcn_sched_barrier(0);
      if (i == 17) {
#pragma unroll
        for (int r = 0; r < 2; ++r) {
          pb[r] = (pb[r] + WW_STAGE_PX * 64) & RMASK;
          int x = px[r] + adv_rem, y = py[r] + adv_rows;
          if (x >= W) {
            x -= W;
            ++y;
          }
          if (y >= H) y -= H;
          px[r] = x;
          py[r] = y;
        }
        __builtin_amdgcn_sched_barrier(0);
      }
    }
    asm volatile("s_waitcnt vmcnt(0)" ::: "memory");
    asm volatile("s_waitcnt lgkmcnt(0)" ::: "memory");
    __builtin_amdgcn_s_barrier();
  }

  const float unscale =
      reinterpret_cast<const float*>(reinterpret_cast<const unsigned char*>(a.dy) + a.dy_bytes - PL_HEADER)[2] *
      reinterpret_cast<const float*>(reinterpret_cast<const unsigned char*>(a.src) + a.src_bytes - PL_HEADER)[2];
  if (a.slabs != nullptr) {
    float* mine = a.slabs + (size_t)lid * WW_TILE_FLOATS;
#pragma unroll
    for (int t = 0; t < 9; ++t)
#pragma unroll
      for (int hf = 0; hf < 2; ++hf)
#pragma unroll
        for (int m = 0; m < 2; ++m)
          *reinterpret_cast<f32x4*>(mine + (((((wave * 9 + t) * 2 + hf) * 2 + m) * 64) + lane) * 4) = acc[t][hf][m];
    return;
  }
#pragma unroll
  for (int t = 0; t < 9; ++t)
#pragma unroll
    for (int hf = 0; hf < 2; ++hf) {
      const long long cj = (long long)t * a.Cs + ci0 + 16 * hf + (lane & 15);
#pragma unroll
      for (int m = 0; m < 2; ++m)
#pragma unroll
        for (int e = 0; e < 4; ++e) {
          const int co = co0 + wave * 32 + 16 * m + 4 * (lane >> 4) + e;
          atomicAdd(&a.dw[(long long)co * a.ldw + cj], acc[t][hf][m][e] * unscale);
        }
    }
}

__global__ __launch_bounds__(256) void wgrad_win16_reduce_kernel(const WgradArgs a) {
  constexpr int PER_TILE = WW_TILE_FLOATS / 4;
  const int tiles = a.tiles_co * a.tiles_j;
  const long long idx = (long long)blockIdx.x * 256 + threadIdx.x;
  const int tile = (int)(idx / PER_TILE);
  if (tile >= tiles) return;
  const int q = (int)(idx - (long long)tile * PER_TILE);
  const int lane = q & 63, piece = q >> 6;
  const int m = piece & 1, hf = (piece >> 1) & 1, t = (piece >> 2) % 9, wave = piece / 36;
  const int co = (tile % a.tiles_co) * WW_CO + wave * 32 + 16 * m + 4 * (lane >> 4);
  const long long cj = (long long)t * a.Cs + (tile / a.tiles_co) * WW_CI + 16 * hf + (lane & 15);
  const f32x4* sl = reinterpret_cast<const f32x4*>(a.slabs) + (size_t)tile * PER_TILE + q;
  const size_t sstride = (size_t)tiles * PER_TILE;
  f32x4 sum = {0.f, 0.f, 0.f, 0.f};
  int s = 0;
  for (; s + 8 <= a.splits; s += 8) {
    f32x4 v[8];
#pragma unroll
    for (int u = 0; u < 8; ++u) v[u] = __builtin_nontemporal_load(sl + (size_t)(s + u) * sstride);
#pragma unroll
    for (int u = 0; u < 8; ++u) sum = sum + v[u];
  }
  for (; s < a.splits; ++s) sum = sum + __builtin_nontemporal_load(sl + (size_t)s * sstride);
  const float unscale =
      reinterpret_cast<const float*>(reinterpret_cast<const unsigned char*>(a.dy) + a.dy_bytes - PL_HEADER)[2] *
      reinterpret_cast<const float*>(reinterpret_cast<const unsigned char*>(a.src) + a.src_bytes - PL_HEADER)[2];
#pragma unroll
  for (int e = 0; e < 4; ++e) a.dw[(long long)(co + e) * a.ldw + cj] += sum[e] * unscale;
}

bool wgrad_win_supported(const WgradArgs& a) {
  if (a.ntaps != 9 || a.kw != 3 || a.sy != 1 || a.sx != 1 || a.pad_t != 1 || a.pad_l != 1) return false;
  if (a.Hg != a.Hs || a.Wg != a.Ws) return false;
  if ((a.Cout % WW_CO) != 0 || (a.Cs % WW_CI) != 0 || a.ldw != 9 * a.Cs) return false;
  if (a.Ws < 4 || 2 * a.Ws + 81 > 512 || 32 / a.Ws + 2 > a.Hs) return false;
  if (a.M < 64 || a.M >= (1LL << 31) - 4096) return false;
  return true;
}

template <auto Kernel>
static bool lds_starts_at_zero() {
  static const bool ok = [] {
    hipFuncAttributes fa{};
    return hipFuncGetAttributes(&fa, reinterpret_cast<const void*>(Kernel)) == hipSuccess && fa.sharedSizeBytes == 0;
  }();
  return ok;
}

template <int RING, int KO, int PF, bool M16>
constexpr auto ww_kernel = M16 ? &wgrad_win16_kernel<RING, KO> : &wgrad_win_kernel<RING, KO, PF>;

template <int RING, int KO, int PF = 1, bool M16 = false>
static int launch_ww(WgradArgs& a, hipStream_t st) {
  constexpr auto kernel = ww_kernel<RING, KO, PF, M16>;
  a.tiles_co = a.Cout / WW_CO;
  a.tiles_j = a.Cs / WW_CI;
  const long long tiles = (long long)a.tiles_co * a.tiles_j;
  constexpr size_t lds = 2 * (2 * 4 * PL_PLANES * 1024) + 2 * (RING * 64 + 64);
  if (!lds_starts_at_zero<kernel>() || !lds_limit_ok<kernel, lds>("wgrad_win_kernel")) return 1;
  int resident = resident_workgroups<kernel, lds>(256, "wgrad_win_kernel");
  if (resident <= 0) resident = 512;
  static const long long target_env = env_ll("YOLO_WGRAD_WIN_TARGET", 0LL);
  const long long target = target_env > 0 ? target_env : (resident >= 2 ? resident / 2 : resident);
  long long splits = target / tiles;
  const long long max_splits = (a.M + 255) / 256;
  if (splits > max_splits) splits = max_splits;
  if (splits < 1) splits = 1;
  a.slabs = nullptr;
  static const bool det_env = env_int("YOLO_WGRAD_DETERMINISTIC", 1) != 0;
  size_t ws_bytes = 0;
  void* ws = wgrad_workspace(&ws_bytes);
  if (det_env && ws != nullptr && ws_bytes > WGRAD_WS_COLSUM_BYTES) {
    const long long cap = (long long)((ws_bytes - WGRAD_WS_COLSUM_BYTES) / ((size_t)WW_TILE_FLOATS * 4));
    if (cap >= tiles) {
      if (tiles * splits > cap) splits = cap / tiles;
      a.slabs = reinterpret_cast<float*>(reinterpret_cast<unsigned char*>(ws) + WGRAD_WS_COLSUM_BYTES);
    }
  }
  long long chunk = (a.M + splits - 1) / splits;
  chunk = (chunk + 31) / 32 * 32;
  splits = (a.M + chunk - 1) / chunk;
  a.chunk = chunk;
  a.splits = (int)splits;
  a.nblocks = (int)(tiles * splits);
  note_conv_launch(M16 ? "wgrad_win_planes_kernel<%d,%d,mfma16>" : "wgrad_win_planes_kernel<%d,%d>", WW_CO, 9 * WW_CI);
  if (int rc = launch_lds<kernel, lds>(dim3((unsigned)a.nblocks), dim3(256), st, a, "wgrad_win_kernel")) return rc;
  if (a.slabs != nullptr) {
    const long long pieces = tiles * (WW_TILE_FLOATS / 4);
    if constexpr (M16) hipLaunchKernelGGL(wgrad_win16_reduce_kernel, dim3((unsigned)((pieces + 255) / 256)), dim3(256), 0, st, a);
    else hipLaunchKernelGGL(wgrad_win_reduce_kernel, dim3((unsigned)((pieces + 255) / 256)), dim3(256), 0, st, a);
    return check_launch("wgrad_win_reduce_kernel");
  }
  return YOLO_OK;
}

static int launch_ww2(WgradArgs& a, hipStream_t st) {
  constexpr int RING = 256;
  constexpr auto kernel = &wgrad_win2_kernel<RING>;
  a.tiles_co = a.Cout / WW_CO;
  a.tiles_j = a.Cs / WW_CI;
  const long long tiles = (long long)a.tiles_co * a.tiles_j;
  constexpr size_t half_bytes = 2 * (2 * 4 * PL_PLANES * 1024) + 2 * (RING * 64 + 64);
  constexpr size_t handover = (size_t)WW_TILE_FLOATS * 4;
  constexpr size_t lds = 2 * half_bytes > handover ? 2 * half_bytes : handover;
  if (!lds_starts_at_zero<kernel>()) return 1;
  const int resident = resident_workgroups<kernel, lds>(512, "wgrad_win2_kernel");
  if (resident <= 0) return 1;
  size_t ws_bytes = 0;
  void* ws = wgrad_workspace(&ws_bytes);
// ... 48 lines not shown
```

### tf2_yolo_amd/csrc/elementwise.hip

```cpp
#include "common.hpp"
#include "planes.hpp"
#include <cfloat>

namespace yolo {

__global__ void copy_in_kernel(const float* __restrict__ src, long long P, int Cs, float* __restrict__ dst, int Cd,
                               int c_off, int vec) {
  if (vec) {
    const int Cs4 = Cs >> 2;
    const long long n = P * Cs4;
    for (long long i = (long long)blockIdx.x * blockDim.x + threadIdx.x; i < n;
         i += (long long)gridDim.x * blockDim.x) {
      const long long p = i / Cs4;
      const int c = (int)(i - p * Cs4) * 4;
      *reinterpret_cast<f32x4*>(dst + p * Cd + c_off + c) = *reinterpret_cast<const f32x4*>(src + p * Cs + c);
    }
  } else {
    const long long n = P * Cs;
    for (long long i = (long long)blockIdx.x * blockDim.x + threadIdx.x; i < n;
         i += (long long)gridDim.x * blockDim.x) {
      const long long p = i / Cs;
      const int c = (int)(i - p * Cs);
      dst[p * Cd + c_off + c] = src[i];
    }
  }
}

__global__ void copy_out_kernel(const float* __restrict__ src, long long P, int Cs, int c_off,
                                float* __restrict__ dst, int Cd, int accumulate, int vec) {
  if (vec) {
    const int Cd4 = Cd >> 2;
    const long long n = P * Cd4;
    for (long long i = (long long)blockIdx.x * blockDim.x + threadIdx.x; i < n;
         i += (long long)gridDim.x * blockDim.x) {
      const long long p = i / Cd4;
      const int c = (int)(i - p * Cd4) * 4;
      f32x4 v = *reinterpret_cast<const f32x4*>(src + p * Cs + c_off + c);
      if (accumulate) {
        const f32x4 o = *reinterpret_cast<const f32x4*>(dst + p * Cd + c);
        v += o;
      }
      *reinterpret_cast<f32x4*>(dst + p * Cd + c) = v;
    }
  } else {
    const long long n = P * Cd;
    for (long long i = (long long)blockIdx.x * blockDim.x + threadIdx.x; i < n;
         i += (long long)gridDim.x * blockDim.x) {
      const long long p = i / Cd;
      const int c = (int)(i - p * Cd);
      float v = src[p * Cs + c_off + c];
      if (accumulate) v += dst[i];
      dst[i] = v;
    }
  }
}

__global__ void upsample_fwd_kernel(const float* __restrict__ x, int N, int H, int W, int C4, float* __restrict__ y,
                                    int Cy, int c_off) {
  const int Ho = 2 * H, Wo = 2 * W;
  const long long n = (long long)N * Ho * Wo * C4;
  for (long long i = (long long)blockIdx.x * blockDim.x + threadIdx.x; i < n; i += (long long)gridDim.x * blockDim.x) {
    const int c = (int)(i % C4);
    long long p = i / C4;
    const int wo = (int)(p % Wo);
    p /= Wo;
    const int ho = (int)(p % Ho);
    const int b = (int)(p / Ho);
    const f32x4 v = *reinterpret_cast<const f32x4*>(x + (((long long)b * H + (ho >> 1)) * W + (wo >> 1)) * (C4 * 4) + c * 4);
    *reinterpret_cast<f32x4*>(y + (((long long)b * Ho + ho) * Wo + wo) * Cy + c_off + c * 4) = v;
  }
}

__global__ void upsample_bwd_kernel(const float* __restrict__ dy, int N, int H, int W, int C4, int Cy, int c_off,
                                    float* __restrict__ dx, int accumulate) {
  const int Ho = 2 * H, Wo = 2 * W;
  const long long n = (long long)N * H * W * C4;
  for (long long i = (long long)blockIdx.x * blockDim.x + threadIdx.x; i < n; i += (long long)gridDim.x * blockDim.x) {
    const int c = (int)(i % C4);
    long long p = i / C4;
    const int w = (int)(p % W);
    p /= W;
    const int h = (int)(p % H);
    const int b = (int)(p / H);
// ... 256 lines not shown
    const float v = t[i];
    float o;
    if (k == 2 || k == 3) o = expf(v) * anchors[a * 2 + (k - 2)];
    else o = sigmoid_f(v);
    y[i] = o;
  }
}

__global__ void head_softmax_fwd_kernel(const float* __restrict__ t, long long groups, int D, int off, int C,
                                        float* __restrict__ y) {
  for (long long g = (long long)blockIdx.x * blockDim.x + threadIdx.x; g < groups;
       g += (long long)gridDim.x * blockDim.x) {
    const float* tp = t + g * D + off;
    float* yp = y + g * D + off;
    float m = -FLT_MAX;
    for (int c = 0; c < C; ++c) m = fmaxf(m, tp[c]);
    float s = 0.f;
    for (int c = 0; c < C; ++c) s += expf(tp[c] - m);
    const float inv = 1.f / s;
    for (int c = 0; c < C; ++c) yp[c] = expf(tp[c] - m) * inv;
  }
}

__global__ void head_sigmoid_fwd_kernel(const float* __restrict__ t, long long P, int D, int nsig,
                                        float* __restrict__ y) {
  const long long n = P * nsig;
  for (long long i = (long long)blockIdx.x * blockDim.x + threadIdx.x; i < n; i += (long long)gridDim.x * blockDim.x) {
    const long long p = i / nsig;
    const int k = (int)(i - p * nsig);
    y[p * D + k] = sigmoid_f(t[p * D + k]);
  }
}

__global__ void head_bwd_pointwise_kernel(const float* __restrict__ y, const float* __restrict__ dy, long long P,
                                          int A, int C, int sigmoid_classes, float* __restrict__ dt) {
  const int D = 5 + C;
  const long long n = P * A * D;
  for (long long i = (long long)blockIdx.x * blockDim.x + threadIdx.x; i < n; i += (long long)gridDim.x * blockDim.x) {
    const int k = (int)(i % D);
    if (k >= 5 && !sigmoid_classes) continue;
    const float yv = y[i], g = dy[i];
    dt[i] = (k == 2 || k == 3) ? g * yv : g * yv * (1.f - yv);
  }
}

__global__ void head_softmax_bwd_kernel(const float* __restrict__ y, const float* __restrict__ dy, long long groups,
                                        int D, int off, int C, float* __restrict__ dt) {
  for (long long g = (long long)blockIdx.x * blockDim.x + threadIdx.x; g < groups;
       g += (long long)gridDim.x * blockDim.x) {
    const float* yp = y + g * D + off;
    const float* gp = dy + g * D + off;
    float* dp = dt + g * D + off;
    float dot = 0.f;
    for (int c = 0; c < C; ++c) dot += gp[c] * yp[c];
    for (int c = 0; c < C; ++c) dp[c] = yp[c] * (gp[c] - dot);
  }
}

__global__ void head_sigmoid_bwd_kernel(const float* __restrict__ y, const float* __restrict__ dy, long long P, int D,
                                        int nsig, float* __restrict__ dt) {
  const long long n = P * nsig;
  for (long long i = (long long)blockIdx.x * blockDim.x + threadIdx.x; i < n; i += (long long)gridDim.x * blockDim.x) {
    const long long p = i / nsig;
    const int k = (int)(i - p * nsig);
    const float yv = y[p * D + k];
    dt[p * D + k] = dy[p * D + k] * yv * (1.f - yv);
  }
}

__global__ void head_danchor_kernel(const float* __restrict__ y, const float* __restrict__ dy, long long P, int A,
                                    int C, const float* __restrict__ anchors, float* __restrict__ danchors) {
  const int D = 5 + C;
  const int slot = blockIdx.y;
  const int a = slot >> 1, j = slot & 1;
  double s = 0.0;
  for (long long p = (long long)blockIdx.x * blockDim.x + threadIdx.x; p < P; p += (long long)gridDim.x * blockDim.x) {
    const long long i = (p * A + a) * D + 2 + j;
    s += (double)dy[i] * (double)y[i];
  }
  s = wave_reduce_sum(s);
  if ((threadIdx.x & 63) == 0) atomicAdd(&danchors[slot], (float)(s / (double)anchors[slot]));
}

__global__ __launch_bounds__(256) void adam_kernel(float* __restrict__ p, float* __restrict__ g,
                                                   float* __restrict__ m, float* __restrict__ v, long long n,
                                                   float lr_t, float b1, float b2, float eps, float gs, int zero,
                                                   const float* __restrict__ hyper) {
  if (hyper != nullptr) {
    lr_t = hyper[0];
    b1 = hyper[1];
    b2 = hyper[2];
    eps = hyper[3];
    gs = hyper[4];
  }
  const long long n4 = n >> 2;
  for (long long i = (long long)blockIdx.x * blockDim.x + threadIdx.x; i < n4; i += (long long)gridDim.x * blockDim.x) {
    f32x4 pv = reinterpret_cast<f32x4*>(p)[i];
    f32x4 gv = reinterpret_cast<f32x4*>(g)[i];
    f32x4 mv = reinterpret_cast<f32x4*>(m)[i];
    f32x4 vv = reinterpret_cast<f32x4*>(v)[i];
#pragma unroll
    for (int e = 0; e < 4; ++e) {
      const float gg = gv[e] * gs;
      mv[e] = b1 * mv[e] + (1.f - b1) * gg;
      vv[e] = b2 * vv[e] + (1.f - b2) * gg * gg;
      pv[e] -= lr_t * mv[e] / (sqrtf(vv[e]) + eps);
    }
    reinterpret_cast<f32x4*>(p)[i] = pv;
    reinterpret_cast<f32x4*>(m)[i] = mv;
    reinterpret_cast<f32x4*>(v)[i] = vv;
    if (zero) reinterpret_cast<f32x4*>(g)[i] = f32x4{0.f, 0.f, 0.f, 0.f};
  }
  for (long long i = (n4 << 2) + (long long)blockIdx.x * blockDim.x + threadIdx.x; i < n;
       i += (long long)gridDim.x * blockDim.x) {
    const float gg = g[i] * gs;
    const float mm = b1 * m[i] + (1.f - b1) * gg;
    const float vv = b2 * v[i] + (1.f - b2) * gg * gg;
    m[i] = mm;
    v[i] = vv;
    p[i] -= lr_t * mm / (sqrtf(vv) + eps);
    if (zero) g[i] = 0.f;
  }
}

__global__ void sgd_kernel(float* __restrict__ p, float* __restrict__ g, long long n, float lr, float gs, int zero) {
  for (long long i = (long long)blockIdx.x * blockDim.x + threadIdx.x; i < n; i += (long long)gridDim.x * blockDim.x) {
    p[i] -= lr * gs * g[i];
    if (zero) g[i] = 0.f;
  }
}

}

using namespace yolo;

extern "C" int yolo_copy_channels_in(const float* src, long long P, int Csrc, float* dst, int Cdst, int c_off,
                                     void* stream) {
  YOLO_REQUIRE(src && dst && P > 0 && Csrc > 0 && c_off >= 0 && c_off + Csrc <= Cdst, "copy_channels_in: bad args");
  const int vec = (Csrc % 4 == 0 && Cdst % 4 == 0 && c_off % 4 == 0) ? 1 : 0;
  const long long n = vec ? P * (Csrc / 4) : P * Csrc;
  hipLaunchKernelGGL(copy_in_kernel, dim3(stream_grid(n, 256)), dim3(256), 0, as_stream(stream), src, P, Csrc, dst,
                     Cdst, c_off, vec);
  return check_launch("copy_in_kernel");
}

extern "C" int yolo_copy_channels_out(const float* src, long long P, int Csrc, int c_off, float* dst, int Cdst,
                                      int accumulate, void* stream) {
  YOLO_REQUIRE(src && dst && P > 0 && Cdst > 0 && c_off >= 0 && c_off + Cdst <= Csrc, "copy_channels_out: bad args");
  const int vec = (Csrc % 4 == 0 && Cdst % 4 == 0 && c_off % 4 == 0) ? 1 : 0;
  const long long n = vec ? P * (Cdst / 4) : P * Cdst;
  hipLaunchKernelGGL(copy_out_kernel, dim3(stream_grid(n, 256)), dim3(256), 0, as_stream(stream), src, P, Csrc, c_off,
                     dst, Cdst, accumulate, vec);
  return check_launch("copy_out_kernel");
}

extern "C" int yolo_upsample2x_fwd(const float* x, int N, int H, int W, int C, float* y, int Cy, int c_off,
                                   void* stream) {
  YOLO_REQUIRE(x && y && N > 0 && H > 0 && W > 0 && C > 0 && c_off >= 0 && c_off + C <= Cy, "upsample_fwd: bad args");
  YOLO_REQUIRE(C % 4 == 0 && Cy % 4 == 0 && c_off % 4 == 0, "upsample_fwd: channels must be multiples of 4");
  const long long n = (long long)N * 4 * H * W * (C / 4);
  hipLaunchKernelGGL(upsample_fwd_kernel, dim3(stream_grid(n, 256)), dim3(256), 0, as_stream(stream), x, N, H, W,
                     C / 4, y, Cy, c_off);
  return check_launch("upsample_fwd_kernel");
}

extern "C" int yolo_upsample2x_bwd(const float* dy, int N, int H, int W, int C, int Cy, int c_off, float* dx,
                                   int accumulate, void* stream) {
  YOLO_REQUIRE(dy && dx && N > 0 && H > 0 && W > 0 && C > 0 && c_off >= 0 && c_off + C <= Cy, "upsample_bwd: bad args");
  YOLO_REQUIRE(C % 4 == 0 && Cy % 4 == 0 && c_off % 4 == 0, "upsample_bwd: channels must be multiples of 4");
  const long long n = (long long)N * H * W * (C / 4);
  hipLaunchKernelGGL(upsample_bwd_kernel, dim3(stream_grid(n, 256)), dim3(256), 0, as_stream(stream), dy, N, H, W,
                     C / 4, Cy, c_off, dx, accumulate);
  return check_launch("upsample_bwd_kernel");
}

extern "C" int yolo_axpy(float* a, const float* b, long long n, void* stream) {
// ... 88 lines not shown
  hipLaunchKernelGGL(s2d_fwd_kernel, dim3(stream_grid(n, 256)), dim3(256), 0, as_stream(stream), x, N, H, W, C, y, Cy,
                     c_off);
  return check_launch("s2d_fwd_kernel");
}

extern "C" int yolo_space_to_depth2_bwd(const float* dy, int N, int H, int W, int C, int Cy, int c_off, float* dx,
                                        int accumulate, void* stream) {
  YOLO_REQUIRE(dy && dx && N > 0 && H > 0 && W > 0 && C > 0 && (H % 2 == 0) && (W % 2 == 0), "space_to_depth_bwd: bad args");
  YOLO_REQUIRE(c_off >= 0 && c_off + 4 * C <= Cy, "space_to_depth_bwd: bad channel slice");
  const long long n = (long long)N * H * W * C;
  hipLaunchKernelGGL(s2d_bwd_kernel, dim3(stream_grid(n, 256)), dim3(256), 0, as_stream(stream), dy, N, H, W, C, Cy,
                     c_off, dx, accumulate);
  return check_launch("s2d_bwd_kernel");
}

extern "C" int yolo_head_act_fwd(const float* t, long long P, int A, int C, int version, const float* anchors,
                                 float* y, void* stream) {
  YOLO_REQUIRE(t && y && P > 0 && A > 0 && C > 0, "head_act_fwd: bad args");
  hipStream_t st = as_stream(stream);
  if (version == YOLO_HEAD_V3 || version == YOLO_HEAD_V4 || version == YOLO_HEAD_V2) {
    YOLO_REQUIRE(anchors != nullptr, "head_act_fwd: anchors required");
    const long long n = P * A * (5 + C);
    hipLaunchKernelGGL(head_fwd_pointwise_kernel, dim3(stream_grid(n, 256)), dim3(256), 0, st, t, P, A, C, anchors, y);
    if (int rc = check_launch("head_fwd_pointwise_kernel")) return rc;
    if (version == YOLO_HEAD_V2) {
      hipLaunchKernelGGL(head_softmax_fwd_kernel, dim3(stream_grid(P * A, 256)), dim3(256), 0, st, t, P * A, 5 + C, 5, C,
                         y);
      return check_launch("head_softmax_fwd_kernel");
    }
    return YOLO_OK;
  }
  if (version == YOLO_HEAD_V1) {
    const int D = 5 * A + C;
    hipLaunchKernelGGL(head_sigmoid_fwd_kernel, dim3(stream_grid(P * 5 * A, 256)), dim3(256), 0, st, t, P, D, 5 * A, y);
    if (int rc = check_launch("head_sigmoid_fwd_kernel")) return rc;
    hipLaunchKernelGGL(head_softmax_fwd_kernel, dim3(stream_grid(P, 256)), dim3(256), 0, st, t, P, D, 5 * A, C, y);
    return check_launch("head_softmax_fwd_kernel");
  }
  set_error("head_act_fwd: bad version %d", version);
  return YOLO_ERR_INVALID_ARG;
}

extern "C" int yolo_head_act_bwd(const float* y, const float* dy, long long P, int A, int C, int version,
                                 const float* anchors, float* dt, float* danchors, void* stream) {
  YOLO_REQUIRE(y && dy && dt && P > 0 && A > 0 && C > 0, "head_act_bwd: bad args");
  hipStream_t st = as_stream(stream);
  if (version == YOLO_HEAD_V3 || version == YOLO_HEAD_V4 || version == YOLO_HEAD_V2) {
    const long long n = P * A * (5 + C);
    hipLaunchKernelGGL(head_bwd_pointwise_kernel, dim3(stream_grid(n, 256)), dim3(256), 0, st, y, dy, P, A, C,
                       version == YOLO_HEAD_V2 ? 0 : 1, dt);
    if (int rc = check_launch("head_bwd_pointwise_kernel")) return rc;
    if (version == YOLO_HEAD_V2) {
      hipLaunchKernelGGL(head_softmax_bwd_kernel, dim3(stream_grid(P * A, 256)), dim3(256), 0, st, y, dy, P * A, 5 + C, 5,
                         C, dt);
      if (int rc = check_launch("head_softmax_bwd_kernel")) return rc;
    }
    if (danchors != nullptr) {
      YOLO_REQUIRE(anchors != nullptr, "head_act_bwd: anchors required for danchors");
      long long gx = (P + 255) / 256;
      if (gx > 256) gx = 256;
      hipLaunchKernelGGL(head_danchor_kernel, dim3((unsigned)gx, 2 * A), dim3(256), 0, st, y, dy, P, A, C, anchors,
                         danchors);
      return check_launch("head_danchor_kernel");
    }
    return YOLO_OK;
  }
  if (version == YOLO_HEAD_V1) {
    const int D = 5 * A + C;
    hipLaunchKernelGGL(head_sigmoid_bwd_kernel, dim3(stream_grid(P * 5 * A, 256)), dim3(256), 0, st, y, dy, P, D, 5 * A,
                       dt);
    if (int rc = check_launch("head_sigmoid_bwd_kernel")) return rc;
    hipLaunchKernelGGL(head_softmax_bwd_kernel, dim3(stream_grid(P, 256)), dim3(256), 0, st, y, dy, P, D, 5 * A, C, dt);
    return check_launch("head_softmax_bwd_kernel");
  }
  set_error("head_act_bwd: bad version %d", version);
  return YOLO_ERR_INVALID_ARG;
}

extern "C" int yolo_adam_step(float* p, float* g, float* m, float* v, long long n, float lr, float beta1, float beta2,
                              float eps, int step, float grad_scale, int zero_grad, void* stream) {
  YOLO_REQUIRE(p && g && m && v && n > 0 && step >= 1, "adam_step: bad args");
  const double lr_t = (double)lr * sqrt(1.0 - pow((double)beta2, (double)step)) / (1.0 - pow((double)beta1, (double)step));
  hipLaunchKernelGGL(adam_kernel, dim3(stream_grid(n / 4 + 1, 256)), dim3(256), 0, as_stream(stream), p, g, m, v, n,
                     (float)lr_t, beta1, beta2, eps, grad_scale, zero_grad, (const float*)nullptr);
  return check_launch("adam_kernel");
}

extern "C" float yolo_adam_lr_t(float lr, float beta1, float beta2, int step) {
  return (float)((double)lr * sqrt(1.0 - pow((double)beta2, (double)step)) / (1.0 - pow((double)beta1, (double)step)));
}

extern "C" int yolo_adam_step_dev(float* p, float* g, float* m, float* v, long long n, const float* hyper, int zero_grad,
                                  void* stream) {
  YOLO_REQUIRE(p && g && m && v && hyper && n > 0, "adam_step_dev: bad args");
  hipLaunchKernelGGL(adam_kernel, dim3(stream_grid(n / 4 + 1, 256)), dim3(256), 0, as_stream(stream), p, g, m, v, n, 0.f,
                     0.f, 0.f, 0.f, 0.f, zero_grad, hyper);
  return check_launch("adam_kernel");
}

extern "C" int yolo_sgd_step(float* p, float* g, long long n, float lr, float grad_scale, int zero_grad,
                             void* stream) {
  YOLO_REQUIRE(p && g && n > 0, "sgd_step: bad args");
  hipLaunchKernelGGL(sgd_kernel, dim3(stream_grid(n, 256)), dim3(256), 0, as_stream(stream), p, g, n, lr, grad_scale,
                     zero_grad);
  return check_launch("sgd_kernel");
}
```

### tf2_yolo_amd/csrc/optim.hip

```cpp
#include <cmath>
#include "common.hpp"

#pragma clang fp contract(off)

namespace yolo {

constexpr int OPT_THREADS = 256;
enum { CLIP_NONE = 0, CLIP_NORM = 1, CLIP_GLOBAL = 2, CLIP_VALUE = 3 };

__global__ __launch_bounds__(OPT_THREADS) void sqnorm_chunk_kernel(const float* __restrict__ g,
                                                                   const long long* __restrict__ chunk_off,
                                                                   const int* __restrict__ chunk_len,
                                                                   double* __restrict__ partial) {
  const long long off = chunk_off[blockIdx.x];
  const int len = chunk_len[blockIdx.x];
  const float* gc = g + off;
  const int n4 = (off & 3) == 0 ? len >> 2 : 0;
  double s = 0.0;
  for (int i = threadIdx.x; i < n4; i += OPT_THREADS) {
    const f32x4 x = reinterpret_cast<const f32x4*>(gc)[i];
#pragma unroll
    for (int e = 0; e < 4; ++e) s += (double)x[e] * (double)x[e];
  }
  for (int i = (n4 << 2) + threadIdx.x; i < len; i += OPT_THREADS) s += (double)gc[i] * (double)gc[i];
  s = wave_reduce_sum(s);
  __shared__ double wave_sum[OPT_THREADS / 64];
  if ((threadIdx.x & 63) == 0) wave_sum[threadIdx.x >> 6] = s;
  __syncthreads();
  if (threadIdx.x == 0) {
    double t = wave_sum[0];
#pragma unroll
    for (int w = 1; w < OPT_THREADS / 64; ++w) t += wave_sum[w];
    partial[blockIdx.x] = t;
  }
}

__device__ __forceinline__ double ordered_sum(const double* __restrict__ x, int first, int last) {
  const int lane = threadIdx.x & 63;
  double s = 0.0;
  for (int base = first; base < last; base += 64) {
    const double mine = base + lane < last ? x[base + lane] : 0.0;
#pragma unroll
    for (int l = 0; l < 64; ++l) s += __shfl(mine, l, 64);
  }
  return s;
}

constexpr int SUM_THREADS = 1024;
__global__ __launch_bounds__(SUM_THREADS) void sqnorm_sum_kernel(const double* __restrict__ partial,
                                                                 const int* __restrict__ var_first, int n_vars,
                                                                 double* __restrict__ var_sq, double* __restrict__ total_sq) {
  const int wave = threadIdx.x >> 6, lane = threadIdx.x & 63;
  for (int v = wave; v < n_vars; v += SUM_THREADS / 64) {
    const double s = ordered_sum(partial, var_first[v], var_first[v + 1]);
    if (lane == 0) var_sq[v] = s;
  }
  __syncthreads();
  if (wave == 0) {
    const double t = ordered_sum(var_sq, 0, n_vars);
    if (lane == 0) *total_sq = t;
  }
}

__global__ void clip_factors_kernel(const double* __restrict__ var_sq, int n_vars, const double* __restrict__ total_a,
                                    const double* __restrict__ total_b, const float* __restrict__ hyper, int mode,
                                    float* __restrict__ factors, float* __restrict__ norm_out) {
  const double gs = fabs((double)hyper[4]);
  const double thr = (double)hyper[6];
  const double total = total_b != nullptr ? *total_a + *total_b : *total_a;
  const double gnorm = gs * sqrt(total);
  const int i = blockIdx.x * blockDim.x + threadIdx.x;
  if (i == 0 && norm_out != nullptr) *norm_out = (float)gnorm;
  if (mode == CLIP_GLOBAL) {
    if (i == 0) factors[0] = (float)(thr / fmax(gnorm, thr));
  } else if (i < n_vars) {
    factors[i] = (float)(thr / fmax(gs * sqrt(var_sq[i]), thr));
  }
}

struct ClipArgs {
  float gs, c, t;
  int value;
};
__device__ __forceinline__ float clipped(float g, const ClipArgs& k) {
  const float x = g * k.gs;
  return k.value ? fminf(fmaxf(x, -k.t), k.t) : x * k.c;
}
__device__ __forceinline__ ClipArgs clip_args(const float* __restrict__ hyper, const float* __restrict__ factors, int mode,
                                              int var) {
  ClipArgs k;
  k.gs = hyper[4];
  k.t = hyper[6];
  k.value = mode == CLIP_VALUE;
  k.c = mode == CLIP_NORM ? factors[var] : mode == CLIP_GLOBAL ? factors[0] : 1.f;
  return k;
}

struct AdamArgs {
  float lr_t, b1, b2, eps;
};
template <bool AMSGRAD>
__device__ __forceinline__ void adam_update(float& p, float& m, float& v, float& vhat, float gg, const AdamArgs& h) {
  m = fmaf(h.b1, m, (1.f - h.b1) * gg);
  v = fmaf(h.b2, v, ((1.f - h.b2) * gg) * gg);
  if (AMSGRAD) {
    vhat = fmaxf(vhat, v);
    p -= (h.lr_t * m) / (sqrtf(vhat) + h.eps);
  } else {
    p -= (h.lr_t * m) / (sqrtf(v) + h.eps);
  }
}

template <bool AMSGRAD>
__global__ __launch_bounds__(OPT_THREADS) void adam_clip_kernel(float* __restrict__ p, float* __restrict__ g,
                                                                float* __restrict__ m, float* __restrict__ v,
                                                                float* __restrict__ vhat,
                                                                const long long* __restrict__ chunk_off,
                                                                const int* __restrict__ chunk_len,
                                                                const int* __restrict__ chunk_var,
                                                                const float* __restrict__ hyper,
                                                                const float* __restrict__ factors, int mode, int zero) {
  const long long off = chunk_off[blockIdx.x];
  const int len = chunk_len[blockIdx.x];
  const ClipArgs k = clip_args(hyper, factors, mode, chunk_var[blockIdx.x]);
  const AdamArgs h = {hyper[0], hyper[1], hyper[2], hyper[3]};
  const int n4 = (off & 3) == 0 ? len >> 2 : 0;
  for (int i = threadIdx.x; i < n4; i += OPT_THREADS) {
    f32x4 pv = reinterpret_cast<f32x4*>(p + off)[i];
    f32x4 gv = reinterpret_cast<f32x4*>(g + off)[i];
    f32x4 mv = reinterpret_cast<f32x4*>(m + off)[i];
    f32x4 vv = reinterpret_cast<f32x4*>(v + off)[i];
    f32x4 hv = {0.f, 0.f, 0.f, 0.f};
    if (AMSGRAD) hv = reinterpret_cast<f32x4*>(vhat + off)[i];
#pragma unroll
    for (int e = 0; e < 4; ++e) {
      float pp = pv[e], mm = mv[e], v1 = vv[e], hh = hv[e];
      adam_update<AMSGRAD>(pp, mm, v1, hh, clipped(gv[e], k), h);
      pv[e] = pp;
      mv[e] = mm;
      vv[e] = v1;
      hv[e] = hh;
    }
    reinterpret_cast<f32x4*>(p + off)[i] = pv;
    reinterpret_cast<f32x4*>(m + off)[i] = mv;
    reinterpret_cast<f32x4*>(v + off)[i] = vv;
    if (AMSGRAD) reinterpret_cast<f32x4*>(vhat + off)[i] = hv;
    if (zero) reinterpret_cast<f32x4*>(g + off)[i] = f32x4{0.f, 0.f, 0.f, 0.f};
  }
  for (long long i = off + (n4 << 2) + threadIdx.x; i < off + len; i += OPT_THREADS) {
    float pp = p[i], mm = m[i], vv = v[i], hh = AMSGRAD ? vhat[i] : 0.f;
    adam_update<AMSGRAD>(pp, mm, vv, hh, clipped(g[i], k), h);
    p[i] = pp;
    m[i] = mm;
    v[i] = vv;
    if (AMSGRAD) vhat[i] = hh;
    if (zero) g[i] = 0.f;
  }
}

template <int KIND>
__device__ __forceinline__ void sgd_update(float& p, float& a, float gg, float lr, float mu) {
  if (KIND == 0) {
    p = fmaf(-lr, gg, p);
  } else {
    const float step = lr * gg;
    a = fmaf(mu, a, -step);
    if (KIND == 1) p += a;
    else p += fmaf(mu, a, -step);
  }
}

template <int KIND>
__global__ __launch_bounds__(OPT_THREADS) void sgd_clip_kernel(float* __restrict__ p, float* __restrict__ g,
                                                               float* __restrict__ a,
                                                               const long long* __restrict__ chunk_off,
                                                               const int* __restrict__ chunk_len,
                                                               const int* __restrict__ chunk_var,
                                                               const float* __restrict__ hyper,
                                                               const float* __restrict__ factors, int mode, int zero) {
  const long long off = chunk_off[blockIdx.x];
  const int len = chunk_len[blockIdx.x];
  const ClipArgs k = clip_args(hyper, factors, mode, chunk_var[blockIdx.x]);
  const float lr = hyper[0], mu = hyper[5];
  const int n4 = (off & 3) == 0 ? len >> 2 : 0;
  for (int i = threadIdx.x; i < n4; i += OPT_THREADS) {
    f32x4 pv = reinterpret_cast<f32x4*>(p + off)[i];
    f32x4 gv = reinterpret_cast<f32x4*>(g + off)[i];
    f32x4 av = {0.f, 0.f, 0.f, 0.f};
    if (KIND != 0) av = reinterpret_cast<f32x4*>(a + off)[i];
#pragma unroll
    for (int e = 0; e < 4; ++e) {
      float pp = pv[e], aa = av[e];
      sgd_update<KIND>(pp, aa, clipped(gv[e], k), lr, mu);
// ... 89 lines not shown
```

### tf2_yolo_amd/engine.py

```python
import math

import contextlib

import numpy as np
import torch

from . import ops
from . import plan
from . import tape
from ._lib import ACT_LEAKY, ACT_LINEAR, ACT_MISH, YoloHipError
from .plan import AUX_WORDS, has_filter

ACT_NAMES = {ACT_LINEAR: "linear", ACT_LEAKY: "leaky", ACT_MISH: "mish"}


class ParamSpec:
    __slots__ = ("name", "shape", "offset", "size", "init", "trainable")

    def __init__(self, name, shape, offset, init, trainable):
        self.name, self.shape, self.offset = name, tuple(shape), offset
        self.size = int(np.prod(shape))
        self.init, self.trainable = init, trainable


# ... 136 lines not shown
        self.inputs = [src]


class GraphBuilder:

    def __init__(self, input_shape, kernel_init=he_normal_krsc):
        h, w, c = input_shape
        self.tensors = []
        self.units = []
        self.kernel_init = kernel_init
        self.input = self._tensor(h, w, c, "input")
        self.outputs = []

    def _tensor(self, h, w, c, name, producer=None):
        t = TensorRef(len(self.tensors), h, w, c, name, producer)
        self.tensors.append(t)
        return t

    def _push(self, unit, h, w, c):
        unit.out = self._tensor(h, w, c, unit.name, unit)
        self.units.append(unit)
        return unit.out

    def conv(self, src, cout, k, name, stride=1, padding=None, bn=True, act=ACT_LEAKY, bias=False, residual=None,
             kernel_init=None):
        if padding is None:
            padding = "same"
        d = ops.conv_desc((1, src.h, src.w, src.c), cout, k, k, stride, padding)
        if residual is not None and (residual.h, residual.w, residual.c) != (d.Ho, d.Wo, cout):
            raise ValueError(f"{name}: residual shape mismatch")
        u = ConvUnit(name, src, cout, k, stride, padding, bn, act, bias, residual, kernel_init or self.kernel_init)
        return self._push(u, d.Ho, d.Wo, cout)

    def upsample(self, src, name):
        return self._push(UpsampleUnit(name, src), src.h * 2, src.w * 2, src.c)

    def concat(self, srcs, name):
        h, w = srcs[0].h, srcs[0].w
        for s in srcs:
            if (s.h, s.w) != (h, w):
                raise ValueError(f"{name}: concat of different spatial sizes")
        return self._push(ConcatUnit(name, srcs), h, w, sum(s.c for s in srcs))

    def maxpool(self, src, k, name, stride=None, padding="valid"):
        stride = stride or k
        if padding == "same":
            ho, wo = -(-src.h // stride), -(-src.w // stride)
        else:
            ho, wo = (src.h - k) // stride + 1, (src.w - k) // stride + 1
        return self._push(MaxPoolUnit(name, src, k, stride, padding), ho, wo, src.c)

    def space_to_depth(self, src, name):
        return self._push(SpaceToDepthUnit(name, src), src.h // 2, src.w // 2, src.c * 4)

    def head(self, src, A, C, version, anchors, name, level):
        u = HeadUnit(name, src, A, C, version, anchors, level, self.kernel_init)
        out = self._push(u, src.h, src.w, u.cout)
        self.outputs.append(out)
        return out


def count_params(builder):
    train = state = 0
    for u in builder.units:
        if has_filter(u):
            train += u.cout * u.k * u.k * u.src.c + (u.cout if u.bias else 0) + (2 * u.cout if u.bn else 0)
            state += 2 * u.cout if u.bn else 0
    return train, state


def conv_flops_per_image(builder):
    total = 0
    for u in builder.units:
        if has_filter(u):
            total += 2 * u.out.h * u.out.w * u.cout * u.src.c * u.k * u.k
    return total


_EPILOGUES = {ACT_LEAKY: ops.EPI_AFFINE_LEAKY, ACT_MISH: ops.EPI_AFFINE_MISH}


def _epilogue(u):
    return _EPILOGUES.get(u.act, ops.EPI_AFFINE)


class Network:
    def __init__(self, builder, device="cuda", seed=1234, unbiased_moving_var=True):
        if not torch.cuda.is_available():
            raise YoloHipError("tf2_yolo_amd needs a HIP device: there is no CPU fallback")
        self.device = torch.device(device)
        if self.device.index is not None and self.device.index != torch.cuda.current_device():
            raise YoloHipError(f"Network(device={device!r}): the kernels launch on the current device "
                               f"(cuda:{torch.cuda.current_device()}); call torch.cuda.set_device first "
                               "(one process per GPU)")
        self.tensors = builder.tensors
        self.units = builder.units
        self.input = builder.input
        self.outputs = list(builder.outputs)
        self.unbiased_moving_var = unbiased_moving_var
        self._opts = plan.Options.from_env()
        for k, v in vars(self._opts).items():
            setattr(self, "_" + k, v)
        g = self._plan = plan.plan_graph(self.units, self.tensors, self.input, self.outputs, self._opts)
        self._needs_grad, self._n_consumers = g.needs_grad, g.n_consumers
        self._bound_alias, self._up_producer = g.bound_alias, g.up_producer
        self.params = ParamStore()
        self.state = ParamStore()
        self._declare_params()
        rng = np.random.default_rng(seed)
        self.params.materialize(self.device, rng)
        self.state.materialize(self.device, rng)
        self.grads = torch.zeros_like(self.params.data)
        self._init_anchors()
        ops.create_side_streams(self.device)
        ops.ensure_conv_workspace()
        ops.ensure_wgrad_workspace()
        self._alloc_planned_buffers(g)
        self._wT_valid = self._wp_valid = self._wTp_valid = False
        self._jobs_wp = self._jobs_wTp = self._jobs_wT = None
        self._wp_event = self._wT_event = None
        self._infer_graphs = {}
        self._wgrad_stream = None
        self._wgrad_pending = False
        self.batch = None
        self.act = {}
        self.training = False
        self._precision = "fp32"
        self.grad_ready_hook = None
        self.backward_begin_hook = None
        self._infer_scale_valid = False
        self._twords = None
        self._tword_n = {}
        self._xplanes_infer = {}
        for u in self.units:
            u.concat_reads_through = False

    def _declare_params(self):
        for u in self.units:
            if u.kind == "conv":
                u.p_kernel = self.params.add(f"{u.name}_conv/kernel", (u.cout, u.k, u.k, u.src.c), u.kernel_init)
                u.p_bias = self.params.add(f"{u.name}_conv/bias", (u.cout,), init_zeros) if u.bias else None
                if u.bn:
                    u.p_gamma = self.params.add(f"{u.name}_bn/gamma", (u.cout,), init_ones)
                    u.p_beta = self.params.add(f"{u.name}_bn/beta", (u.cout,), init_zeros)
                    u.s_mean = self.state.add(f"{u.name}_bn/moving_mean", (u.cout,), init_zeros)
                    u.s_var = self.state.add(f"{u.name}_bn/moving_variance", (u.cout,), init_ones)
            elif u.kind == "head":
                u.p_kernel = self.params.add(f"{u.name}/kernel", (u.cout, 1, 1, u.src.c), u.kernel_init)
                u.p_bias = self.params.add(f"{u.name}/bias", (u.cout,), init_zeros)

    def _init_anchors(self):
        self._anchors_dev, self._anchor_grad_views = {}, {}
        heads = [u for u in self.units if u.kind == "head" and u.anchors is not None]
        n_anch = sum(2 * len(u.anchors) for u in heads)
        self.anchors_flat = torch.zeros(max(n_anch, 1), device=self.device, dtype=torch.float32)
        self.anchor_grads = torch.zeros_like(self.anchors_flat)
        self.anchors_trainable = False
        off = 0
        for u in heads:
            n = 2 * len(u.anchors)
            self.anchors_flat[off:off + n] = torch.tensor(np.array(u.anchors, dtype=np.float32).reshape(-1))
            self._anchors_dev[u.name] = self.anchors_flat[off:off + n]
            self._anchor_grad_views[u.name] = self.anchor_grads[off:off + n]
            off += n
        self.has_anchors = n_anch > 0

    def _alloc_planned_buffers(self, g):
        dev = self.device
        self._wT = torch.empty(g.wT_total, device=dev, dtype=torch.float32)
        self._bn_f32 = torch.zeros(max(g.bn_f32_total, 1), device=dev, dtype=torch.float32)
        self._bn_f64 = torch.zeros(max(g.bn_f64_total, 1), device=dev, dtype=torch.float64)
        self._bn_stats_total = g.bn_stats_total
        self._wplanes = torch.empty(g.wplanes_total, device=dev, dtype=torch.uint8) if g.wplanes_total else None
        self._aux = torch.zeros(g.aux_total, device=dev, dtype=torch.int32)
        self._tbound = self._aux[g.tbound_off:].view(torch.float32)
        self._tb = [self._tbound[i:i + 1] for i in range(len(self.tensors))]
        self._pred = torch.zeros(g.pred_total, device=dev, dtype=torch.float32)
        for u in self.units:
            a = u.aux_off
            u.bound = self._aux[a:a + 1]
            u.red_bound = self._aux[a + 1:a + 69]
            u.tickets = self._aux[a + 69:a + 69 + ops.BN_FOLD_TICKET_WORDS]
            u.pred = self._pred[u.pred_off:u.pred_off + 2]
            if u.kind == "conv" and u.bn:
                u.amax = self._aux[a + AUX_WORDS:a + AUX_WORDS + u.cout]
            if not has_filter(u):
                continue
            u.wT = self._wT[u.wT_off:u.wT_off + u.cout * u.k * u.k * u.src.c]
            u.wp = self._wplanes[u.wp_off:u.wp_off + u.wp_bytes] if u.planes_fwd else None
            u.wTp = self._wplanes[u.wTp_off:u.wTp_off + u.wTp_bytes] if u.planes_dgrad else None
            if u.cpad:
                u.wTp_pad = self._wplanes[u.wTp_pad_off:u.wTp_pad_off + u.wTp_pad_bytes]
                n = u.cpad * u.src.c
                u.w_pad = torch.zeros(n, device=dev, dtype=torch.float32)
                u.wT_pad = torch.empty(n, device=dev, dtype=torch.float32)
                u.dw_pad = torch.empty(n, device=dev, dtype=torch.float32)

    @property
    def num_params(self):
        return sum(self.params.specs[n].size for n in self.params.order)

    @property
    def num_state(self):
        return sum(self.state.specs[n].size for n in self.state.order)

    def allocate(self, N):
        if self.batch == N:
            return
        worst = max((t.h * t.w * t.c * 4 for t in self.tensors), default=0)
        if worst and N * worst + (1 << 20) >= (1 << 32):
            raise YoloHipError(f"batch {N}: the largest activation ({worst / 2 ** 20:.1f} MiB per image) would exceed the "
                               f"4 GiB a conv operand may span; the largest per-GPU batch for this model is "
                               f"{((1 << 32) - (1 << 20)) // worst - 1}")
        self.batch = N
        self.alloc_gen = getattr(self, "alloc_gen", 0) + 1
        self._infer_graphs = {}
        self.act = {}
        bp = plan.plan_batch(self.units, N, self._opts)

        def new(u, dtype=torch.float32):
            return torch.empty((N, u.out.h, u.out.w, u.out.c), device=self.device, dtype=dtype)

        def new_bytes(n, make=torch.empty):
            return make(n, device=self.device, dtype=torch.uint8)
        for u in self.units:
            u.bnred = None
            if u.kind == "conv":
                u.desc = bp.desc[u.name]
                u.y = new(u)
                u.a = new(u) if (u.bn or u.act != ACT_LINEAR) else u.y
                self.act[u.out.tid] = u.a
            elif u.kind == "head":
# ... 336 lines not shown
        nw = ops.stem_fwd_infer_unit(u.desc, xin, u.stem_wt, _epilogue(u), scale, shift, u.pred, row[:n_in],
                                     u.a if u.a_needed else None, pl, self._tb_row(u.out.tid))
        self._tword_n[u.out.tid] = nw
        self._tbound_set.add(u.out.tid)
        self._xp_valid.add(u.out.tid)
        return True

    def _fused_infer_unit(self, u, bias, scale, shift):
        if not u.planes_fwd or u.cout % 16 != 0:
            return False
        pl = self._xplanes.get(u.out.tid)
        own_planes = pl is not None
        if pl is None and self._infer_small_fuse and self._infer_onepass:
            rows = self.batch * u.out.h * u.out.w
            if rows <= 4096:
                pl = self._xplanes_infer.get(u.out.tid)
                if pl is None:
                    pl = self._xplanes_infer[u.out.tid] = torch.zeros(ops.planes_bytes(rows, u.cout), device=self.device,
                                                                     dtype=torch.uint8)
        if pl is None or (u.residual is not None and u.residual.tid not in self._tbound_set):
            return False
        self._fold_infer_scale(u, scale, shift)
        res = self.act[u.residual.tid] if u.residual is not None else None
        src_slot = self._bound_alias.get(u.src.tid, u.src.tid)
        if self._infer_onepass and src_slot in self._tbound_set:
            if not self._infer_scale_valid:
                ops.zero_bytes(u.pred)
                ops.conv_pred_bound(self.params.view(u.p_kernel.name), u.cout, u.k * u.k * u.src.c, scale, shift, bias, u.pred)
            nw = ops.conv2d_fwd_infer_unit(u.desc, self._xp(u.src), u.wp, bias, _epilogue(u), scale, shift, res, u.a, u.amax,
                                           u.pred, self._tb_words(src_slot),
                                           self._tb_words(u.residual.tid) if u.residual is not None else None, pl,
                                           self._tb_row(u.out.tid), self._tb[u.out.tid], precision=self._precision)
            if nw:
                self._tword_n[u.out.tid] = nw
            self._tbound_set.add(u.out.tid)
            if own_planes:
                self._xp_valid.add(u.out.tid)
            return True
        if not own_planes:
            return False
        ops.conv2d_fwd_planes_epi(u.desc, self._xp(u.src), u.wp, bias, _epilogue(u), scale, shift, residual=res, out=u.a,
                                  absmax=u.amax, precision=self._precision)
        ops.split_planes_absmax(u.a, self.batch * u.out.h * u.out.w, u.cout, u.amax, pl,
                                extra_bound=self._tb_float(u.residual.tid) if u.residual is not None else None,
                                out_bound=self._tb[u.out.tid])
        self._tbound_set.add(u.out.tid)
        self._xp_valid.add(u.out.tid)
        return True

    def _stem_fused_bwd(self, u):
        return (self._stem_fused and not (u.planes_wgrad or u.planes_dgrad) and not self._needs_grad[u.src.tid]
                and ops.stem_bn_bwd_supported(u.desc))

    def _takes_grad_slice(self, u):
        return u.kind == "conv" and u.bn and u.residual is None and u.cout % 8 == 0 and not self._stem_fused_bwd(u)

    def _add_grad(self, grads, t, buf):
        if not self._needs_grad[t.tid]:
            return
        cur = grads.get(t.tid)
        if cur is None:
            grads[t.tid] = buf
        else:
            ops.axpy(cur, buf)

    def _grad_into(self, grads, t):
        cur = grads.get(t.tid)
        if cur is not None:
            return cur, True
        cur = grads[t.tid] = torch.empty((self.batch, t.h, t.w, t.c), device=self.device, dtype=torch.float32)
        return cur, False

    def _gview(self, spec):
        return self.grads[spec.offset:spec.offset + spec.size]

    def backward(self, douts):
        if not self.training:
            raise YoloHipError("backward() requires a preceding forward(training=True)")
        if self.backward_begin_hook is not None:
            tape.host_call(self.backward_begin_hook)
        if self._wT_event is not None:
            tape.wait_event(torch.cuda.current_stream(), self._wT_event)
            self._wT_event = None
        self._refresh_wT()
        self._refresh_wTplanes()
        for u in self.units:
            if getattr(u, "bnred", None) is not None:
                u.bnred_done = False
        grads = {t.tid: g for t, g in zip(self.outputs, douts)}
        for u in reversed(self.units):
            dout = grads.pop(u.out.tid, None)
            if dout is None:
                continue
            if isinstance(dout, ops.ChannelSlice) and not self._takes_grad_slice(u):
                dout = dout.dense((self.batch, u.out.h, u.out.w, u.out.c))
            getattr(self, "_bwd_" + u.kind)(u, dout, grads)
            if self.grad_ready_hook is not None and has_filter(u):
                tape.host_call(lambda u=u: self.grad_ready_hook(u))
        self._join_wgrad()

    def _bwd_conv(self, u, dout, grads):
        if u.bn:
            scale, shift, smean, sinv, _, red = self._bn_bufs(u)
            if u.residual is not None:
                self._add_grad(grads, u.residual, dout)
            if self._stem_fused_bwd(u):
                ops.stem_bn_bwd_wgrad(u.desc, self.act[u.src.tid], u.y, dout, scale, shift, smean, sinv, u.act, red,
                                      self._gview(u.p_gamma), self._gview(u.p_beta), self._gview(u.p_kernel),
                                      fused=self._take_fused(u, dout))
                return
            need_f32 = (not u.planes_wgrad) or (self._needs_grad[u.src.tid] and not u.planes_dgrad)
            dyp = self._next_dyp_buffer(u) if (u.planes_wgrad or u.planes_dgrad) else None
            dy = ops.bn_act_bwd(u.y, dout, u.cout, self.params.view(u.p_gamma.name), scale, shift, smean,
                                sinv, u.act, red, self._gview(u.p_gamma), self._gview(u.p_beta),
                                planes=dyp, want_dx=need_f32, bound_aux=u.red_bound, fused=self._take_fused(u, dout),
                                tickets=u.tickets if self._bn_fold else None)
        else:
            dy = ops.act_bwd(u.y, dout, u.act) if u.act != ACT_LINEAR else dout
            dyp = self._dyp(u, dy)
        dbias = self._gview(u.p_bias) if (u.p_bias is not None and not u.bn) else None
        self._filter_and_data_grad(u, dy, dyp, dbias, grads)

    def _bwd_head(self, u, dout, grads):
        dt = ops.head_act_bwd(u.yact, dout, u.A, u.C, u.version, self._anchors_dev.get(u.name),
                              danchors=self._anchor_grad_views.get(u.name) if self.anchors_trainable else None)
        if not u.cpad:
            return self._filter_and_data_grad(u, dt, self._dyp(u, dt), self._gview(u.p_bias), grads)
        rows = self.batch * u.out.h * u.out.w
        dtp = ops.split_planes_padded(dt, rows, u.out.c, out=self._next_dyp_buffer(u))
        with self._beside_backward(dt):
            ops.zero_bytes(u.dw_pad)
            ops.conv2d_wgrad_planes(u.desc_pad, self._xplanes[u.src.tid], dtp, u.dw_pad)
            ops.axpy(self._gview(u.p_kernel), u.dw_pad[:u.out.c * u.src.c])
            ops.conv2d_wgrad_bias(dt, rows, u.out.c, self._gview(u.p_bias))
        if self._needs_grad[u.src.tid]:
            had = grads.get(u.src.tid)
            b = self._bnred_of(u, had)
            cur, acc = self._grad_into(grads, u.src)
            ops.conv2d_dgrad_planes(u.desc_pad, dtp, u.wTp_pad, dx=cur, accumulate=acc, bnred=b)

    def _filter_and_data_grad(self, u, dy, dyp, dbias, grads):
        with self._beside_backward(dy):
            if u.planes_wgrad:
                ops.conv2d_wgrad_planes(u.desc, self._xplanes[u.src.tid], dyp, self._gview(u.p_kernel), dy=dy, dbias=dbias)
            else:
                ops.conv2d_wgrad(u.desc, self.act[u.src.tid], dy, self._gview(u.p_kernel), dbias)
        if not self._needs_grad[u.src.tid]:
            return
        b = self._bnred_of(u, grads.get(u.src.tid)) if u.planes_dgrad else None
        cur, acc = self._grad_into(grads, u.src)
        if u.planes_dgrad:
            ops.conv2d_dgrad_planes(u.desc, dyp, u.wTp, dx=cur, accumulate=acc, bnred=b)
        else:
            ops.conv2d_dgrad(u.desc, dy, u.wT, dx=cur, accumulate=acc)

    def _bwd_upsample(self, u, dout, grads):
        if self._needs_grad[u.src.tid]:
            cur, acc = self._grad_into(grads, u.src)
            ops.upsample2x_bwd(dout, u.out.c, 0, cur, accumulate=acc)

    def _bwd_concat(self, u, dout, grads):
        off = 0
        for s in u.srcs:
            if not self._needs_grad[s.tid]:
                pass
            elif (s.tid not in grads and self._concat_grad_slices and self._n_consumers.get(s.tid, 0) == 1
                    and s.producer is not None and self._takes_grad_slice(s.producer)
                    and s.c % 8 == 0 and off % 4 == 0 and u.out.c % 4 == 0):
                grads[s.tid] = ops.ChannelSlice(dout, u.out.c, off, s.c)
            else:
                cur, acc = self._grad_into(grads, s)
                ops.copy_channels_out(dout, u.out.c, off, cur, s.c, accumulate=acc)
            off += s.c

    def _bwd_maxpool(self, u, dout, grads):
        if not self._needs_grad[u.src.tid]:
            return
        N, had = self.batch, grads.get(u.src.tid)
        tiles = (u.k == 2 and u.stride == 2 and u.pad_t == 0 and u.pad_l == 0 and u.src.h == 2 * u.out.h
                 and u.src.w == 2 * u.out.w and u.out.c % 4 == 0 and torch.is_tensor(dout) and dout.is_contiguous()
                 and (had is None or torch.is_tensor(had)))
        cur, acc = self._grad_into(grads, u.src)
        if tiles:
            ops.maxpool2x2_bwd(dout, N, u.out.h, u.out.w, u.out.c, u.argmax, cur, acc)
            return
        if not acc:
            ops.zero_bytes(cur)
        if u.stride == 1 and (u.out.h, u.out.w) == (u.src.h, u.src.w):
            ops.maxpool_bwd_same(dout, N, u.out.h, u.out.w, u.out.c, u.out.c, 0, u.argmax, u.k, u.pad_t, u.pad_l, cur)
        else:
            ops.maxpool_bwd(dout, N, u.out.h, u.out.w, u.out.c, u.out.c, 0, u.argmax, cur)

    def _bwd_space_to_depth(self, u, dout, grads):
        if self._needs_grad[u.src.tid]:
            cur, acc = self._grad_into(grads, u.src)
            ops.space_to_depth2_bwd(dout, u.out.c, 0, cur, accumulate=acc)

    def _next_dyp_buffer(self, u=None):
        if u is not None and u.name in self._dyp_own:
            self._dyp_cur_own = True
            return self._dyp_own[u.name]
        self._dyp_cur_own = False
        self._dyp_idx ^= 1
        ev = self._dyp_events[self._dyp_idx]
        if ev is not None:
            tape.wait_event(torch.cuda.current_stream(), ev)
            self._dyp_events[self._dyp_idx] = None
        if self._dyplanes2[self._dyp_idx] is None and self._dyp_shared_bytes:
            self._dyplanes2[self._dyp_idx] = torch.empty(self._dyp_shared_bytes, device=self.device, dtype=torch.uint8)
        return self._dyplanes2[self._dyp_idx]

    @contextlib.contextmanager
    def _beside_backward(self, *tensors):
        if not self._overlap_wgrad:
            yield
            return
        if self._wgrad_stream is None:
            self._wgrad_stream = ops.concurrent_stream("wgrad", device=self.device)
        side = self._wgrad_stream
        tape.wait_stream(side, torch.cuda.current_stream())
        for t in tensors:
            if t is not None:
                t.record_stream(side)
        with torch.cuda.stream(side):
            yield
            ev = None if getattr(self, "_dyp_cur_own", False) else tape.record_event(side)
        if ev is not None:
            self._dyp_events[self._dyp_idx] = ev
        self._wgrad_pending = True

    def _join_wgrad(self):
        if self._wgrad_pending:
            tape.wait_stream(torch.cuda.current_stream(), self._wgrad_stream)
            self._wgrad_pending = False

    def _dyp(self, u, dy):
        if not (u.planes_wgrad or u.planes_dgrad):
            return None
        return ops.split_planes(dy, self.batch * u.out.h * u.out.w, u.cout, out=self._next_dyp_buffer(u))

    def _bnred_of(self, w, cur):
        p = w.bnred_for
        if p is None or p.bnred is None or (cur is not None and not torch.is_tensor(cur)):
            return None
        p.bnred_done = True
        return p.bnred

    def _take_fused(self, u, dout):
        b = getattr(u, "bnred", None)
        if b is None or not u.bnred_done:
            return None
        u.bnred_done = False
        if not torch.is_tensor(dout):
            raise YoloHipError(f"{u.name}: fused reduction made for a gradient that arrives as a channel slice")
        return b

    def named_weights(self):
        out = {}
        for store in (self.params, self.state):
            for name in store.order:
                s = store.specs[name]
                a = store.view(name).detach().cpu().numpy().reshape(s.shape)
                if name.endswith("/kernel"):
                    a = np.transpose(a, (1, 2, 3, 0))
                out[name] = a.copy()
        return out

    def load_named_weights(self, weights, strict=True):
        self.before_param_write()
        for store in (self.params, self.state):
            for name in store.order:
                if name not in weights:
                    if strict:
                        raise KeyError(f"missing weight {name}")
                    continue
                s = store.specs[name]
                a = np.asarray(weights[name], dtype=np.float32)
                if name.endswith("/kernel"):
                    a = np.transpose(a, (3, 0, 1, 2))
                if tuple(a.shape) != s.shape:
                    raise ValueError(f"{name}: shape {a.shape} != {s.shape}")
                store.view(name).copy_(torch.from_numpy(np.ascontiguousarray(a)).reshape(-1))
        self.mark_params_changed()
```

### tf2_yolo_amd/model.py

```python
import time

import numpy as np
import torch

from . import dp as dp_mod
from . import optimizers as opt_mod
from ._lib import YoloHipError, precision_enum
from .engine import Network


def _to_input(x):
    if torch.is_tensor(x):
        return x.to(device="cuda", dtype=torch.float32).contiguous()
    return torch.from_numpy(np.ascontiguousarray(np.asarray(x, dtype=np.float32))).cuda()


class LayerView:

    def __init__(self, model, name, getter, setter, trainable=True):
        self.model, self.name, self._get, self._set, self.trainable = model, name, getter, setter, trainable

    def get_weights(self):
        return self._get()

# ... 229 lines not shown
        self.optimizer = optimizer
        self.optimizer.bind(self.net)
        nout = len(self.net.outputs)
        self.loss = list(loss) if isinstance(loss, (list, tuple)) else [loss] * nout
        if len(self.loss) != nout:
            raise ValueError(f"need {nout} losses, got {len(self.loss)}")
        if metrics is None:
            metrics = [[] for _ in range(nout)]
        elif nout == 1 and (not metrics or not isinstance(metrics[0], (list, tuple))):
            metrics = [list(metrics)]
        self.metrics = [list(m) for m in metrics]
        self._loss_bufs = [torch.zeros(8, device="cuda", dtype=torch.float64) for _ in range(nout)]
        self._dpred = None
        self._drop_step_graphs()

    def enable_data_parallel(self, process_group=None, bucket_bytes=48 << 20):
        segs, units = dp_mod.network_segments(self.net)
        self._reducer = dp_mod.GradReducer(self.net.grads, segs, process_group, bucket_bytes)
        index = {id(u): i for i, u in enumerate(units)}
        self._dp_unit_index = index
        self._drop_step_graphs()
        self.net.grad_ready_hook = lambda u: self._reducer.segment_done(index[id(u)])
        self.net.backward_begin_hook = self._reducer.backward_begin
        net = self.net
        self._reducer.extra_streams = lambda: [net._wgrad_stream] if net._wgrad_stream is not None else []
        dp_mod.broadcast_parameters([self.net.params.data, self.net.state.data], 0, process_group)
        self.net.mark_params_changed()

    def _labels(self, y):
        ys = [y] if not isinstance(y, (list, tuple)) else list(y)
        out = []
        for a in ys:
            if torch.is_tensor(a):
                out.append(a.to(device="cuda", dtype=torch.float32).contiguous())
            else:
                out.append(torch.from_numpy(np.ascontiguousarray(np.asarray(a, dtype=np.float32))).cuda())
        return out

    def _drop_step_graphs(self):
        self._step_graphs = None
        self._eager_steps = {}

    def _captured_step(self, x, y_list):
        import os
        mode = os.environ.get("YOLO_STEP_MODE", "tape")
        if os.environ.get("YOLO_STEP_GRAPH", "1") == "0" or mode == "eager" or getattr(self, "_graphs_failed", False):
            return None
        if not getattr(self.optimizer, "capturable", False):
            return None
        if self.net.grad_ready_hook is not None and self._reducer is None:
            return None
        from .capture import StepGraphs, StepTape
        self.net.allocate(x.shape[0])
        key = StepGraphs.key_of(self, x)
        g = self._step_graphs
        if g is not None and g.key == key:
            return g.replay(x, y_list)
        n = self._eager_steps.get(key, 0)
        if os.environ.get("YOLO_STEP_DEBUG"):
            import sys
            print(f"[step] mode {mode} eager steps so far {n} key {key} known {list(self._eager_steps)}", file=sys.stderr)
        if n < 2 or self._dpred is None:
            self._eager_steps = {key: n + 1}
            self._step_graphs = None
            return None
        try:
            if mode == "graph":
                self._step_graphs = StepGraphs(self, x, y_list)
                return self._step_graphs.replay(x, y_list)
            self._step_graphs = StepTape(self, x, y_list)
            return self._loss_bufs
        except Exception as e:
            import sys
            import traceback
            print(f"[tf2_yolo_amd] step recording ({mode}) failed ({e!r}); training continues with eager launches\n"
                  + "".join(traceback.format_exc().splitlines(True)[-12:]), file=sys.stderr)
            self._graphs_failed = True
            self._step_graphs = None
            if mode != "graph":
                from . import ops as _ops
                _ops.zero_bytes(self.net.grads)
            return None

    def train_step_device(self, x, y_list, with_metrics=False):
        if self.optimizer is None:
            raise YoloHipError("compile() the model before training")
        from . import ops as _ops
        if not with_metrics and _ops.TIMER is None:
            bufs = self._captured_step(x, y_list)
            if bufs is not None:
                return bufs, None
        outs = self.net.forward(x, training=True)
        if self._dpred is None or self._dpred[0].shape != outs[0].shape:
            self._dpred = [torch.empty_like(o) for o in outs]
        for i, (o, yt) in enumerate(zip(outs, y_list)):
            self.loss[i].fwd_bwd(yt, o, grad_scale=1.0, dpred=self._dpred[i], loss_out=self._loss_bufs[i])
        mvals = None
        if with_metrics:
            mvals = [[m(yt, o) for m in ms] for ms, o, yt in zip(self.metrics, outs, y_list)]
        self.net.backward(self._dpred)
        if self._reducer is not None and self.net.anchors_trainable and self._reducer.world > 1:
            import torch.distributed as dist
            dist.all_reduce(self.net.anchor_grads, group=self._reducer.pg)
        scale = self._reducer.finish() if self._reducer is not None else 1.0
        self.optimizer.step(grad_scale=scale)
        return self._loss_bufs, mvals

    def train_on_batch(self, x, y, return_dict=False, **_):
        bufs, mvals = self.train_step_device(_to_input(x), self._labels(y), with_metrics=bool(self.metrics))
        losses = [float(b[0].item()) for b in bufs]
        total = sum(losses)
        flat = [float(v.item()) for ms in (mvals or []) for v in ms]
        res = [total] + (losses if len(losses) > 1 else []) + flat
        return res if len(res) > 1 else res[0]

    def test_on_batch(self, x, y):
        outs = self.net.forward(_to_input(x), training=False)
        ys = self._labels(y)
        losses = [float(l(yt, o).item()) for l, o, yt in zip(self.loss, outs, ys)]
        mvals = [float(m(yt, o).item()) for ms, o, yt in zip(self.metrics, outs, ys) for m in ms]
        return [sum(losses)] + (losses if len(losses) > 1 else []) + mvals

    def _iter_batches(self, x, y, batch_size, shuffle, rng):
        if y is None:
            order = np.arange(len(x))
            for i in order:
                yield x[int(i)]
            if hasattr(x, "on_epoch_end"):
                x.on_epoch_end()
            return
        n = len(x)
        order = rng.permutation(n) if shuffle else np.arange(n)
        ys = y if isinstance(y, (list, tuple)) else [y]
        for i in range(0, n, batch_size):
            sel = order[i:i + batch_size]
            yb = [a[sel] for a in ys]
            yield x[sel], (yb if isinstance(y, (list, tuple)) else yb[0])

    def _host_source(self, x, y, batch_size, shuffle, rng):
        if y is None:
            def batches():
                for i in range(len(x)):
                    yield x[int(i)]
                if hasattr(x, "on_epoch_end"):
                    x.on_epoch_end()
            return ("batches", batches())
        ys = list(y) if isinstance(y, (list, tuple)) else [y]
        if any(torch.is_tensor(a) and a.is_cuda for a in [x] + ys):
            return None
        n = len(x)
        order = rng.permutation(n) if shuffle else np.arange(n)
        return ("arrays", [x] + ys, order, batch_size)

    def fit(self, x=None, y=None, batch_size=None, epochs=1, verbose=1, validation_data=None, shuffle=True,
            initial_epoch=0, callbacks=None, **_):
        import os
        from .feeder import FeederBuffers, HostFeeder
        batch_size = batch_size or 32
        rng = np.random.default_rng(0)
        hist = {"loss": []}
        pipelined = os.environ.get("YOLO_FIT_PIPELINE", "1") != "0"
        cbs = list(callbacks or [])

        def _cb(hook, *args):
            for c in cbs:
                f = getattr(c, hook, None)
                if f is not None:
                    f(*args)
        for c in cbs:
            if hasattr(c, "set_model"):
                c.set_model(self)
        self.stop_training = False
        _cb("on_train_begin", {})
        for ep in range(initial_epoch, epochs):
            t0 = time.time()
            _cb("on_epoch_begin", ep, {})
            tot, nb = 0.0, 0
            src = self._host_source(x, y, batch_size, shuffle, rng) if pipelined else None
            if src is not None:
                if getattr(self, "_feed_bufs", None) is None:
                    self._feed_bufs = FeederBuffers()
                feeder = HostFeeder(src, self._feed_bufs)
                tot_dev = torch.zeros((), dtype=torch.float64, device="cuda")
# ... 41 lines not shown
```

### tf2_yolo_amd/ops.py

```python
import ctypes
from ctypes import byref, c_void_p

import torch

from . import _lib
from . import tape as _tape
from ._lib import ConvDesc, LossCfg, YoloHipError, check

BN_EPS = 1e-3
BN_MOMENTUM = 0.99
BN_STAT_SLOTS = 64
BN_RED_SLOTS = 512
SPLIT_BATCH_UNITS = 4


class KernelTimer:

    def __init__(self):
        self.pending = []

    def bracket(self, flops, fn, layer=None):
        last, n = _lib.load().yolo_last_conv_kernel, ctypes.c_int(0)
        last(None)
        s, e = torch.cuda.Event(enable_timing=True), torch.cuda.Event(enable_timing=True)
# ... 435 lines not shown
    check(_lib.load().yolo_split_planes_concat_ex(xs, cs, bs, bn, us, int(hw[0]), int(hw[1]), n, int(rows), _p(planes),
                                                  _p(dst32), _p(out_bound), _stream()), "yolo_split_planes_concat_ex")
    return planes


def conv2d_fwd_head_unit(d, xp, wp, bias, A, C, version, anchors_dev, t, y, precision="fp32"):
    prec = precision_enum(precision)
    _chk_f32(t, y)
    n = d.N * d.Ho * d.Wo * d.Cout
    if t.numel() != n or y.numel() != n:
        raise YoloHipError("conv2d_fwd_head_unit: output size does not match the descriptor")
    if xp.numel() < planes_bytes(d.N * d.H * d.W, d.Cin) or wp.numel() < planes_bytes(d.Cout, d.kh * d.kw * d.Cin):
        raise YoloHipError("conv2d_fwd_head_unit: planes buffers do not match the descriptor")
    check(_lib.load().yolo_conv2d_fwd_head_unit_ex(ctypes.byref(d), _p(xp), _p(wp), _p(bias), int(A), int(C), int(version),
                                                   _p(anchors_dev), _p(t), _p(y), prec, _stream()),
          "yolo_conv2d_fwd_head_unit_ex")
    return y


class BnReduce:
    __slots__ = ("y", "scale", "shift", "mean", "invstd", "act", "partials", "cap", "aux", "nslots")

    def __init__(self, y, scale, shift, mean, invstd, act, partials, cap, aux):
        self.y, self.scale, self.shift, self.mean, self.invstd, self.act = y, scale, shift, mean, invstd, act
        self.partials, self.cap, self.aux, self.nslots = partials, cap, aux, 0


def bnred_slots_cap(d):
    return int(_lib.load().yolo_bnred_slots_cap(byref(d)))


def conv2d_dgrad_planes(d, dyp, wTp, dx=None, accumulate=False, bnred=None):
    if dx is None:
        dx = torch.empty((d.N, d.H, d.W, d.Cin), device=dyp.device, dtype=torch.float32)
        accumulate = False
    if (dyp.numel() < planes_bytes(d.N * d.Ho * d.Wo, d.Cout) or wTp.numel() < planes_bytes(d.Cin, d.kh * d.kw * d.Cout)
            or dx.numel() != d.N * d.H * d.W * d.Cin):
        raise YoloHipError("conv2d_dgrad_planes: buffers do not match the descriptor")
    if bnred is not None:
        b = bnred
        _chk_f32(b.y, b.scale, b.shift, b.mean, b.invstd, b.partials)
        if (b.y.numel() != dx.numel() or min(t.numel() for t in (b.scale, b.shift, b.mean, b.invstd)) < d.Cin
                or b.partials.numel() < b.cap * 2 * d.Cin or b.aux is None or b.aux.numel() < 68):
            raise YoloHipError("conv2d_dgrad_planes: the fused reduction's buffers do not match the descriptor")
    def run():
        if bnred is None:
            check(_lib.load().yolo_conv2d_dgrad_planes(byref(d), _p(dyp), _p(wTp), _p(dx), int(bool(accumulate)), _stream()),
                  "yolo_conv2d_dgrad_planes")
            return
        n = ctypes.c_int(0)
        check(_lib.load().yolo_conv2d_dgrad_planes_bnred(byref(d), _p(dyp), _p(wTp), _p(dx), int(bool(accumulate)), _p(b.y),
                                                         _p(b.scale), _p(b.shift), _p(b.mean), _p(b.invstd), int(b.act),
                                                         _p(b.partials), int(b.cap), _p(b.aux), byref(n), _stream()),
              "yolo_conv2d_dgrad_planes_bnred")
        b.nslots = n.value
    if TIMER is not None:
        TIMER.bracket(_conv_flops(d), run, _layer_key(d, "dgrad"))
    else:
        run()
    return dx


def conv2d_wgrad_planes(d, xp, dyp, dw, dy=None, dbias=None):
    _chk_f32(dw, dy, dbias)
    if dw.numel() != d.Cout * d.kh * d.kw * d.Cin:
        raise YoloHipError("conv2d_wgrad_planes: dw size does not match the descriptor")
    if xp.numel() < planes_bytes(d.N * d.H * d.W, d.Cin) or dyp.numel() < planes_bytes(d.N * d.Ho * d.Wo, d.Cout):
        raise YoloHipError("conv2d_wgrad_planes: planes buffers do not match the descriptor")
    def run():
        check(_lib.load().yolo_conv2d_wgrad_planes(byref(d), _p(xp), _p(dyp), _p(dw), _stream()),
              "yolo_conv2d_wgrad_planes")
    if TIMER is not None:
        TIMER.bracket(_conv_flops(d), run, _layer_key(d, "wgrad"))
    else:
        run()
    if dbias is not None:
        if dy is None:
            raise YoloHipError("conv2d_wgrad_planes: dbias needs the fp32 dy")
        check(_lib.load().yolo_conv2d_wgrad_bias(_p(dy), d.N * d.Ho * d.Wo, d.Cout, _p(dbias), _stream()),
              "yolo_conv2d_wgrad_bias")
    return dw


def conv2d_wgrad_bias(dy, rows, c, dbias):
    _chk_f32(dy, dbias)
    if dy.numel() != rows * c or dbias.numel() != c:
        raise YoloHipError("conv2d_wgrad_bias: sizes do not match")
    check(_lib.load().yolo_conv2d_wgrad_bias(_p(dy), int(rows), int(c), _p(dbias), _stream()), "yolo_conv2d_wgrad_bias")
    return dbias


def filter_transpose(w, cout, taps, cin, out=None):
    _chk_f32(w)
    if out is None:
        out = torch.empty(cin * taps * cout, device=w.device, dtype=torch.float32)
    check(_lib.load().yolo_filter_transpose(_p(w), _p(out), cout, taps, cin, _stream()), "yolo_filter_transpose")
    return out


def conv2d_dgrad(d, dy, wT, dx=None, accumulate=False):
    _chk_f32(dy, wT)
    if dx is None:
        dx = torch.empty((d.N, d.H, d.W, d.Cin), device=dy.device, dtype=torch.float32)
        accumulate = False
    if dy.numel() != d.N * d.Ho * d.Wo * d.Cout or dx.numel() != d.N * d.H * d.W * d.Cin:
        raise YoloHipError("conv2d_dgrad: tensor sizes do not match the descriptor")
    def run():
        check(_lib.load().yolo_conv2d_dgrad(byref(d), _p(dy), _p(wT), _p(dx), int(bool(accumulate)), _stream()),
              "yolo_conv2d_dgrad")
    if TIMER is not None:
        TIMER.bracket(_conv_flops(d), run)
    else:
        run()
    return dx


def conv2d_wgrad(d, x, dy, dw, dbias=None):
    _chk_f32(x, dy, dw, dbias)
    if dw.numel() != d.Cout * d.kh * d.kw * d.Cin:
        raise YoloHipError("conv2d_wgrad: dw size does not match the descriptor")
    def run():
        check(_lib.load().yolo_conv2d_wgrad(byref(d), _p(x), _p(dy), _p(dw), None, _stream()), "yolo_conv2d_wgrad")
    if TIMER is not None:
        TIMER.bracket(_conv_flops(d), run)
    else:
        run()
    if dbias is not None:
        check(_lib.load().yolo_conv2d_wgrad_bias(_p(dy), d.N * d.Ho * d.Wo, d.Cout, _p(dbias), _stream()),
              "yolo_conv2d_wgrad_bias")
    return dw


def bn_stats(x, C, stats):
    P = x.numel() // C
    check(_lib.load().yolo_bn_stats(_p(x), P, C, _p(stats), _stream()), "yolo_bn_stats")


def bn_finalize(stats, P, C, gamma, beta, moving_mean, moving_var, scale, shift, save_mean, save_invstd,
                eps=BN_EPS, momentum=BN_MOMENTUM, unbiased=False, bound=None, absmax=None, mean_offset=None):
    check(_lib.load().yolo_bn_finalize_offset(_p(stats), P, C, _p(gamma), _p(beta), eps, momentum, int(unbiased),
                                              _p(moving_mean), _p(moving_var), _p(scale), _p(shift), _p(save_mean),
                                              _p(save_invstd), _p(absmax), _p(bound), _p(mean_offset), _stream()),
          "yolo_bn_finalize")


def bn_infer_bound(C, scale, shift, absmax, bound):
    check(_lib.load().yolo_bn_infer_bound(C, _p(scale), _p(shift), _p(absmax), _p(bound), _stream()), "yolo_bn_infer_bound")


def bn_fold_inference(C, gamma, beta, moving_mean, moving_var, scale, shift, eps=BN_EPS):
    check(_lib.load().yolo_bn_fold_inference(C, _p(gamma), _p(beta), _p(moving_mean), _p(moving_var), eps,
                                             _p(scale), _p(shift), _stream()), "yolo_bn_fold_inference")


def bn_act_fwd(x, C, scale, shift, act, residual=None, out=None, planes=None, bn_bound=None, residual_bound=None,
               out_bound=None, want_out=True, residual_planes=None):
    if not want_out:
        if planes is None:
            raise YoloHipError("bn_act_fwd: nothing to produce")
        out = None
    elif out is None:
        out = torch.empty_like(x)
    P = x.numel() // C
    if planes is not None and planes.numel() < planes_bytes(P, C):
        raise YoloHipError("bn_act_fwd: planes buffer too small")
    if residual_planes is not None:
# ... 240 lines not shown
    cfg = LossCfg()
    cfg.version, cfg.N, cfg.gh, cfg.gw, cfg.A, cfg.C = version, N, gh, gw, A, C
    if anchors is not None:
        flat = [float(v) for pair in anchors for v in pair]
        if len(flat) != 2 * A or len(flat) > 32:
            raise ValueError(f"need {A} (w,h) anchors, at most 16; got {len(flat) // 2}")
        for i, v in enumerate(flat):
            cfg.anchors[i] = v
        cfg.use_anchors = 1
    else:
        cfg.use_anchors = 0
    cfg.binary_weight = float(binary_weight)
    lw = list(loss_weight) + [0.0] * (4 - len(loss_weight))
    for i in range(4):
        cfg.loss_weight[i] = float(lw[i])
    cfg.ignore_thresh = float(ignore_thresh)
    cfg.use_focal_loss = int(bool(use_focal_loss))
    cfg.focal_gamma = float(focal_gamma)
    cfg.use_scale = int(bool(use_scale))
    cfg.wh_reg_weight = float(wh_reg_weight)
    cfg.truth_thresh = float(truth_thresh)
    cfg.label_smooth = float(label_smooth)
    return cfg


def loss_fwd_bwd(cfg, y_true, y_pred, loss_out=None, dpred=None, grad_scale=1.0, want_grad=True, decisions=None):
    _chk_f32(y_true, y_pred, dpred)
    cells = cfg.N * cfg.gh * cfg.gw
    pd = (5 * cfg.A + cfg.C) if cfg.version == 1 else cfg.A * (5 + cfg.C)
    if y_true.numel() != cells * (5 + cfg.C) or y_pred.numel() != cells * pd:
        raise YoloHipError(f"loss: tensor sizes do not match cfg (cells={cells}, C={cfg.C}, A={cfg.A})")
    if loss_out is None:
        loss_out = torch.empty(8, device=y_pred.device, dtype=torch.float64)
    if want_grad and dpred is None:
        dpred = torch.empty_like(y_pred)
    if decisions is not None and (decisions.dtype != torch.int32 or decisions.numel() < 2 * cells or not decisions.is_cuda):
        raise YoloHipError("loss: decisions must be an int32 CUDA tensor with 2 entries per cell")
    check(_lib.load().yolo_loss_fwd_bwd(byref(cfg), _p(y_true), _p(y_pred), _p(loss_out),
                                        _p(dpred if want_grad else None), float(grad_scale), _p(decisions),
                                        0 if decisions is None else decisions.numel() * 4, _stream()), "yolo_loss_fwd_bwd")
    return loss_out, dpred


def metrics(cfg, y_true, y_pred, recall_thresh=0.5, out=None):
    _chk_f32(y_true, y_pred)
    if out is None:
        out = torch.empty(8, device=y_pred.device, dtype=torch.float64)
    check(_lib.load().yolo_metrics(byref(cfg), _p(y_true), _p(y_pred), float(recall_thresh), _p(out), _stream()),
          "yolo_metrics")
    return out


def encode_labels(boxes, cls, first, n_images, img_hw, grid_shape, class_num):
    if boxes.dtype != torch.float64 or cls.dtype != torch.int32 or first.dtype != torch.int32:
        raise YoloHipError("encode_labels: boxes float64, cls / first int32")
    gh, gw = grid_shape
    l64 = torch.empty((n_images, gh, gw, 5 + class_num), device=boxes.device, dtype=torch.float64)
    l32 = torch.empty((n_images, gh, gw, 5 + class_num), device=boxes.device, dtype=torch.float32)
    check(_lib.load().yolo_encode_labels(_p(boxes.contiguous()), _p(cls.contiguous()), _p(first.contiguous()), n_images,
                                         float(img_hw[0]), float(img_hw[1]), gh, gw, class_num, _p(l64), _p(l32),
                                         _stream()), "yolo_encode_labels")
    return l64, l32


def down2xlabel(label64):
    if label64.dtype != torch.float64 or not label64.is_cuda or not label64.is_contiguous():
        raise YoloHipError("down2xlabel: contiguous float64 CUDA tensor expected")
    n, gh, gw, ch = label64.shape
    o64 = torch.empty((n, gh // 2, gw // 2, ch), device=label64.device, dtype=torch.float64)
    o32 = torch.empty((n, gh // 2, gw // 2, ch), device=label64.device, dtype=torch.float32)
    check(_lib.load().yolo_down2xlabel(_p(label64), n, gh, gw, ch, _p(o64), _p(o32), _stream()), "yolo_down2xlabel")
    return o64, o32


def adam_step(p, g, m, v, lr, step, beta1=0.9, beta2=0.999, eps=1e-7, grad_scale=1.0, zero_grad=True):
    check(_lib.load().yolo_adam_step(_p(p), _p(g), _p(m), _p(v), p.numel(), lr, beta1, beta2, eps, int(step),
                                     float(grad_scale), int(bool(zero_grad)), _stream()), "yolo_adam_step")


def adam_lr_t(lr, step, beta1=0.9, beta2=0.999):
    return float(_lib.load().yolo_adam_lr_t(float(lr), float(beta1), float(beta2), int(step)))


def adam_step_dev(p, g, m, v, hyper, zero_grad=True):
    check(_lib.load().yolo_adam_step_dev(_p(p), _p(g), _p(m), _p(v), p.numel(), _p(hyper), int(zero_grad), _stream()),
          "yolo_adam_step_dev")


def sgd_step(p, g, lr, grad_scale=1.0, zero_grad=True):
    check(_lib.load().yolo_sgd_step(_p(p), _p(g), p.numel(), lr, float(grad_scale), int(bool(zero_grad)), _stream()),
          "yolo_sgd_step")


OPT_CHUNK = 8192
CLIP_NONE, CLIP_NORM, CLIP_GLOBAL, CLIP_VALUE = 0, 1, 2, 3
OPT_HYPER = 8


def build_chunk_table(variables, chunk=OPT_CHUNK):
    import numpy as np
    if chunk <= 0 or chunk % 4:
        raise ValueError("chunk must be a positive multiple of 4 floats")
    offs, lens, owner, first = [], [], [], [0]
    end = 0
    for v, (off, size) in enumerate(variables):
        off, size = int(off), int(size)
        if off < end or size < 0:
            raise ValueError(f"variable {v} (offset {off}, size {size}) overlaps the one before it")
        end = off + size
        for o in range(off, end, chunk):
            offs.append(o)
            lens.append(min(chunk, end - o))
            owner.append(v)
        first.append(len(offs))
    return (np.asarray(offs, dtype=np.int64), np.asarray(lens, dtype=np.int32), np.asarray(owner, dtype=np.int32),
            np.asarray(first, dtype=np.int32))


class ChunkTable:

    def __init__(self, variables, chunk=OPT_CHUNK, device="cuda"):
        off, ln, var, first = build_chunk_table(variables, chunk)
        if len(off) == 0:
            raise YoloHipError("ChunkTable: no elements")
        self.n_chunks, self.n_vars = len(off), len(first) - 1
        self.extent = int(off[-1] + ln[-1])
        self.off, self.len, self.var, self.first = (torch.from_numpy(a).to(device) for a in (off, ln, var, first))
        self.var_sq = torch.zeros(self.n_vars, dtype=torch.float64, device=device)
        self.total_sq = torch.zeros(1, dtype=torch.float64, device=device)
        nbytes = int(_lib.load().yolo_grad_sqnorm_workspace_bytes(self.n_chunks))
        self.workspace = torch.zeros((nbytes + 7) // 8, dtype=torch.float64, device=device)

    def covers(self, *ts):
        _chk_f32(*ts)
        for t in ts:
            if t is not None and t.numel() < self.extent:
                raise YoloHipError(f"chunk table reaches element {self.extent}, the buffer has {t.numel()}")


def _chk_hyper(hyper):
    _chk_f32(hyper)
    if hyper.numel() < OPT_HYPER:
        raise YoloHipError(f"hyper needs {OPT_HYPER} floats, got {hyper.numel()}")


def grad_sqnorm(g, table):
    table.covers(g)
    ws = table.workspace
    check(_lib.load().yolo_grad_sqnorm(_p(g), _p(table.off), _p(table.len), table.n_chunks, _p(table.first), table.n_vars,
                                       _p(table.var_sq), _p(table.total_sq), _p(ws), ws.numel() * ws.element_size(),
                                       _stream()), "yolo_grad_sqnorm")


def clip_factors(table, hyper, mode, factors, norm_out=None, extra=None):
    _chk_hyper(hyper)
    _chk_f32(factors, norm_out)
    if mode not in (CLIP_NORM, CLIP_GLOBAL) or factors.numel() < (table.n_vars if mode == CLIP_NORM else 1):
        raise YoloHipError("clip_factors: bad mode or too few factors")
    check(_lib.load().yolo_clip_factors(_p(table.var_sq), table.n_vars, _p(table.total_sq),
                                        _p(extra.total_sq if extra is not None else None), _p(hyper), int(mode),
                                        _p(factors), _p(norm_out), _stream()), "yolo_clip_factors")


def _chk_clip(table, mode, factors):
    if mode in (CLIP_NORM, CLIP_GLOBAL):
        _chk_f32(factors)
        if factors is None or factors.numel() < (table.n_vars if mode == CLIP_NORM else 1):
            raise YoloHipError("clipping by norm needs its factors (clip_factors)")
    elif mode not in (CLIP_NONE, CLIP_VALUE):
# ... 166 lines not shown
```

### tf2_yolo_amd/optimizers/__init__.py

```python
import torch

from .. import ops
from . import schedules


def _positive(name, x):
    if x is None:
        return None
    x = float(x)
    if not x > 0.0:
        raise ValueError(f"{name} must be positive, got {x}")
    return x


class Optimizer:
    capturable = False
    _HYPER_SLOTS = 64

    def _init_common(self, learning_rate, lr, clipnorm, clipvalue, global_clipnorm, decay, name):
        self.learning_rate = lr if lr is not None else learning_rate
        given = [(n, v) for n, v in (("clipnorm", clipnorm), ("clipvalue", clipvalue), ("global_clipnorm", global_clipnorm))
                 if v is not None]
        if len(given) > 1:
            raise ValueError(f"at most one of clipnorm, clipvalue and global_clipnorm may be set, got "
                             f"{', '.join(n for n, _ in given)}")
        self.clipnorm, self.clipvalue = _positive("clipnorm", clipnorm), _positive("clipvalue", clipvalue)
        self.global_clipnorm = _positive("global_clipnorm", global_clipnorm)
        self._clip_mode, self._clip_threshold = ops.CLIP_NONE, 0.0
        for mode, t in ((ops.CLIP_NORM, self.clipnorm), (ops.CLIP_GLOBAL, self.global_clipnorm),
                        (ops.CLIP_VALUE, self.clipvalue)):
            if t is not None:
                self._clip_mode, self._clip_threshold = mode, t
        self.decay = float(decay)
        if self.decay < 0.0:
            raise ValueError(f"decay must not be negative, got {self.decay}")
        self.name = name or type(self).__name__
        self.iterations = 0
        self._norm_steps = 0

    @property
    def learning_rate(self):
        return self._learning_rate

    @learning_rate.setter
    def learning_rate(self, value):
        self._learning_rate = value if callable(value) else float(value)

    lr = learning_rate

    def _lr_now(self):
        step = self.iterations - 1
        lr = self._learning_rate
        lr = float(lr(step)) if callable(lr) else lr
        if self.decay:
            lr = lr / (1.0 + self.decay * step)
        return lr

    def bind(self, net):
        self.net = net
        self._anch = None
        if not self._extended:
            return
        p = net.params
        self._table = ops.ChunkTable([(p.specs[n].offset, p.specs[n].size) for n in p.order])
        if net.has_anchors:
            self._anch = ops.ChunkTable([(2 * i, 2) for i in range(net.anchors_flat.numel() // 2)])
        self._factors = self._anch_factors = None
        if self._clip_mode in (ops.CLIP_NORM, ops.CLIP_GLOBAL):
            per_var = self._clip_mode == ops.CLIP_NORM
            self._factors = torch.ones(self._table.n_vars if per_var else 1, dtype=torch.float32, device="cuda")
            if self._anch is not None:
                self._anch_factors = (torch.ones(self._anch.n_vars, dtype=torch.float32, device="cuda") if per_var
                                      else self._factors)
        self._norm_dev = torch.zeros(1, dtype=torch.float32, device="cuda")
        self._norm_steps = 0

    def _with_anchors(self):
        return self.net.anchors_trainable and self.net.has_anchors

    def slots(self):
        return {}

    def _hyper_buffers(self):
        if getattr(self, "_hyper_dev", None) is None:
            self._hyper_host = torch.zeros(self._HYPER_SLOTS, ops.OPT_HYPER, dtype=torch.float32).pin_memory()
            self._hyper_events = [None] * self._HYPER_SLOTS
            self._hyper_dev = torch.zeros(ops.OPT_HYPER, dtype=torch.float32, device="cuda")
        return self._hyper_host, self._hyper_dev

    def _fill_hyper(self, host, grad_scale):
        raise NotImplementedError

    def refresh_hyper(self, grad_scale=1.0):
        self.iterations += 1
        ring, dev = self._hyper_buffers()
        slot = self.iterations % self._HYPER_SLOTS
        if self._hyper_events[slot] is not None:
            self._hyper_events[slot].synchronize()
        host = ring[slot]
        self._fill_hyper(host, float(grad_scale))
        dev.copy_(host, non_blocking=True)
        ev = torch.cuda.Event()
        ev.record(torch.cuda.current_stream())
        self._hyper_events[slot] = ev

    def _enqueue_clip(self, dev):
        if self._clip_mode not in (ops.CLIP_NORM, ops.CLIP_GLOBAL):
            return None, None
        net, anch = self.net, self._anch if self._with_anchors() else None
        ops.grad_sqnorm(net.grads, self._table)
        if anch is not None:
            ops.grad_sqnorm(net.anchor_grads, anch)
        ops.clip_factors(self._table, dev, self._clip_mode, self._factors, norm_out=self._norm_dev, extra=anch)
        if anch is not None and self._clip_mode == ops.CLIP_NORM:
            ops.clip_factors(anch, dev, self._clip_mode, self._anch_factors)
        self._norm_steps += 1
        return self._factors, self._anch_factors

    def _extended_step(self, grad_scale):
        self.net.before_param_write()
        self.refresh_hyper(grad_scale)
        self.step_captured()
        self.net.mark_params_changed()

    def last_grad_norm(self):
        if self._clip_mode not in (ops.CLIP_NORM, ops.CLIP_GLOBAL) or self._norm_steps == 0:
            return None
        return float(self._norm_dev.item())

    def step(self, grad_scale=1.0):
        raise NotImplementedError


class Adam(Optimizer):
    capturable = True

    def __init__(self, learning_rate=0.001, beta_1=0.9, beta_2=0.999, epsilon=1e-7, amsgrad=False, clipnorm=None,
                 clipvalue=None, global_clipnorm=None, decay=0.0, lr=None, name=None):
        self._init_common(learning_rate, lr, clipnorm, clipvalue, global_clipnorm, decay, name)
        self.beta_1, self.beta_2, self.epsilon = float(beta_1), float(beta_2), float(epsilon)
        self.amsgrad = bool(amsgrad)
        self.m = self.v = self.vhat = None

    @property
    def _extended(self):
        return self.amsgrad or self._clip_mode != ops.CLIP_NONE

    def bind(self, net):
        super().bind(net)
        self.m = torch.zeros_like(net.params.data)
        self.v = torch.zeros_like(net.params.data)
        self.am = torch.zeros_like(net.anchors_flat)
        self.av = torch.zeros_like(net.anchors_flat)
        self.vhat = torch.zeros_like(net.params.data) if self.amsgrad else None
        self.avhat = torch.zeros_like(net.anchors_flat) if self.amsgrad else None

    def slots(self):
        s = {"m": self.m, "v": self.v, "anchors/m": self.am, "anchors/v": self.av}
        if self.amsgrad:
            s.update({"vhat": self.vhat, "anchors/vhat": self.avhat})
        return s

    def step(self, grad_scale=1.0):
        if self._extended:
            return self._extended_step(grad_scale)
        self.iterations += 1
        lr = self._lr_now()
        self.net.before_param_write()
        ops.adam_step(self.net.params.data, self.net.grads, self.m, self.v, lr, self.iterations,
                      self.beta_1, self.beta_2, self.epsilon, grad_scale=grad_scale, zero_grad=True)
        if self._with_anchors():
            ops.adam_step(self.net.anchors_flat, self.net.anchor_grads, self.am, self.av, lr,
                          self.iterations, self.beta_1, self.beta_2, self.epsilon, grad_scale=grad_scale, zero_grad=True)
        self.net.mark_params_changed()

    def _fill_hyper(self, host, grad_scale):
        host[0] = ops.adam_lr_t(self._lr_now(), self.iterations, self.beta_1, self.beta_2)
        host[1], host[2], host[3], host[4] = self.beta_1, self.beta_2, self.epsilon, grad_scale
        host[5], host[6] = 0.0, self._clip_threshold

    def step_captured(self):
        _, dev = self._hyper_buffers()
        net = self.net
        if not self._extended:
            ops.adam_step_dev(net.params.data, net.grads, self.m, self.v, dev, zero_grad=True)
            if self._with_anchors():
                ops.adam_step_dev(net.anchors_flat, net.anchor_grads, self.am, self.av, dev, zero_grad=True)
            return
        f, fa = self._enqueue_clip(dev)
        ops.adam_step_clip(net.params.data, net.grads, self.m, self.v, self._table, dev, factors=f,
                           clip_mode=self._clip_mode, vhat=self.vhat, zero_grad=True)
        if self._with_anchors():
            ops.adam_step_clip(net.anchors_flat, net.anchor_grads, self.am, self.av, self._anch, dev, factors=fa,
                               clip_mode=self._clip_mode, vhat=self.avhat, zero_grad=True)


class SGD(Optimizer):
    def __init__(self, learning_rate=0.01, momentum=0.0, nesterov=False, clipnorm=None, clipvalue=None,
                 global_clipnorm=None, decay=0.0, lr=None, name=None):
        self._init_common(learning_rate, lr, clipnorm, clipvalue, global_clipnorm, decay, name)
        self.momentum = float(momentum)
        if not 0.0 <= self.momentum <= 1.0:
            raise ValueError(f"momentum must be in [0, 1], got {self.momentum}")
        self.nesterov = bool(nesterov)
        self.a = self.aa = None

    @property
    def _extended(self):
        return self.momentum > 0.0 or self._clip_mode != ops.CLIP_NONE

    @property
    def capturable(self):
        return self._extended

    def bind(self, net):
        super().bind(net)
        if self.momentum > 0.0:
            self.a = torch.zeros_like(net.params.data)
            self.aa = torch.zeros_like(net.anchors_flat)

    def slots(self):
        return {"momentum": self.a, "anchors/momentum": self.aa} if self.a is not None else {}

    def step(self, grad_scale=1.0):
        if self._extended:
            return self._extended_step(grad_scale)
        self.iterations += 1
        lr = self._lr_now()
        self.net.before_param_write()
        ops.sgd_step(self.net.params.data, self.net.grads, lr, grad_scale=grad_scale, zero_grad=True)
        if self._with_anchors():
            ops.sgd_step(self.net.anchors_flat, self.net.anchor_grads, lr, grad_scale=grad_scale,
                         zero_grad=True)
        self.net.mark_params_changed()

    def _fill_hyper(self, host, grad_scale):
        host[0], host[4], host[5], host[6] = self._lr_now(), grad_scale, self.momentum, self._clip_threshold

    def step_captured(self):
        _, dev = self._hyper_buffers()
        net = self.net
        f, fa = self._enqueue_clip(dev)
        nesterov = self.nesterov and self.a is not None
        ops.sgd_step_clip(net.params.data, net.grads, self._table, dev, accum=self.a, nesterov=nesterov, factors=f,
                          clip_mode=self._clip_mode, zero_grad=True)
        if self._with_anchors():
            ops.sgd_step_clip(net.anchors_flat, net.anchor_grads, self._anch, dev, accum=self.aa, nesterov=nesterov,
                              factors=fa, clip_mode=self._clip_mode, zero_grad=True)
```

### tf2_yolo_amd/plan.py

```python
import os
from types import SimpleNamespace

from . import ops

AUX_WORDS = 112


class Options:

    @classmethod
    def from_env(cls, env=None):
        env = os.environ if env is None else env
        o = cls()

        def on(name):
            return env.get(name, "1") != "0"
        o.overlap_wgrad = on("YOLO_BWD_OVERLAP")
        o.prep_beside = on("YOLO_PREP_OVERLAP")
        o.stem_fused = on("YOLO_STEM_FUSED_BWD")
        o.bn_tight = int(env.get("YOLO_BN_TIGHT_BOUND", "0"))
        o.res_from_planes = on("YOLO_RES_PLANES")
        o.use_infer_graph = on("YOLO_INFER_GRAPH")
        o.fuse_infer = on("YOLO_INFER_FUSE")
        o.concat_grad_slices = on("YOLO_CONCAT_GRAD_SLICE")
        o.dyp_per_layer = on("YOLO_DYP_PER_LAYER")
        o.bn_fold = env.get("YOLO_BN_FOLD", "0") == "1"
        o.bn_fused_reduce = env.get("YOLO_BN_FUSED_REDUCE", "0")
        o.head_pad = on("YOLO_HEAD_PAD")
        o.pool_fuse = on("YOLO_POOL_FUSE")
        o.concat_planes = on("YOLO_CONCAT_PLANES")
        o.infer_onepass = on("YOLO_INFER_ONEPASS")
        o.infer_small_fuse = on("YOLO_INFER_SMALL_FUSE")
        o.dgrad_classes = on("YOLO_DGRAD_CLASSES")
        return o


def has_filter(u):
    return u.kind in ("conv", "head")


def reads_as_planes(c, t):
    return has_filter(c) and c.src.tid == t.tid and c.residual is not t and c.planes_fwd and c.planes_wgrad


def _fp32_read(t, g, also=lambda c: False):
    cs = g.consumers.get(t.tid, [])
    return t.tid in g.out_tids or not cs or any(not (reads_as_planes(c, t) or also(c)) for c in cs)


def plan_graph(units, tensors, input, outputs, opts):
    g = SimpleNamespace(out_tids={t.tid for t in outputs})
    g.needs_grad = {input.tid: False}
    for u in units:
        g.needs_grad[u.out.tid] = has_filter(u) or any(g.needs_grad[t.tid] for t in u.inputs)
    g.consumers, g.n_consumers = {}, {}
    for u in units:
        for t in u.inputs:
            g.consumers.setdefault(t.tid, []).append(u)
            g.n_consumers[t.tid] = g.n_consumers.get(t.tid, 0) + 1
    for t in outputs:
        g.n_consumers[t.tid] = g.n_consumers.get(t.tid, 0) + 1
    _plan_param_buffers(g, units)
    _plan_fused_reduce(g, units, tensors, opts)
    _plan_filter_planes(g, units, opts)
    _plan_fp32_copies(g, units, opts)
    _plan_bounds(g, units, tensors)
    return g


def _plan_param_buffers(g, units):
    wT = f32 = f64 = 0
    for u in units:
        if u.kind == "conv" and u.bn:
            u.bn_f32_off = f32
            f32 += 4 * u.cout
            u.bn_f64_off = f64
            f64 += ops.BN_STAT_SLOTS * 2 * u.cout
        if has_filter(u):
            u.wT_off = wT
            wT += u.cout * u.k * u.k * u.src.c
    g.bn_stats_total = f64
    for u in units:
        if u.kind == "conv" and u.bn:
            u.bn_red_off = f64
            f64 += (ops.BN_RED_SLOTS + 1) * 2 * u.cout
    g.wT_total, g.bn_f32_total, g.bn_f64_total = wT, f32, f64


def _plan_fused_reduce(g, units, tensors, opts):
    last = {}
    for u in reversed(units):
        u.bnred_for = None
        if u.kind == "conv" and u.bn and u.residual is not None and g.needs_grad[u.residual.tid]:
            last[u.residual.tid] = ("add", u)
        if has_filter(u):
            if g.needs_grad[u.src.tid]:
                last[u.src.tid] = ("dgrad", u)
        else:
            for t in u.inputs:
                if g.needs_grad[t.tid]:
                    last[t.tid] = ("other", u)
    mode = opts.bn_fused_reduce
    if mode == "0":
        return
    for tid, (how, w) in last.items():
        p = tensors[tid].producer
        if how != "dgrad":
            continue
        one_launch = w.stride == 1 or (w.stride == 2 and w.k == 3 and opts.dgrad_classes)
        if not (one_launch and p is not None and p.kind == "conv" and p.bn and p.cout % 4 == 0):
            continue
        if w.kind == "head":
            cls = "h"
        elif w.stride == 2:
            cls = "s"
        elif w.k == 1:
            cls = "p"
        else:
            cls = "w"
        w.bnred_class = cls
        if mode == "1" or cls in mode or (cls == "w" and "t" in mode):
            w.bnred_for = p


def _plan_filter_planes(g, units, opts):
    total = 0

    def region(nbytes):
        nonlocal total
        off = total
        total += (nbytes + 255) // 256 * 256
        return off, nbytes
    for u in filter(has_filter, units):
        cin, taps = u.src.c, u.k * u.k
        u.planes_fwd = ops.planes_fwd_ok(cin, u.cout)
        u.planes_dgrad = ops.planes_dgrad_ok(cin, u.cout) and g.needs_grad[u.src.tid]
        u.planes_wgrad = u.planes_fwd and ops.planes_wgrad_ok(cin, u.cout, taps, u.stride)
        u.wp_off = u.wTp_off = -1
        u.cpad = 0
        if u.kind == "head" and u.cout % 16 != 0 and not u.planes_dgrad and opts.head_pad:
            cp = (u.cout + 15) // 16 * 16
            if u.planes_fwd and ops.planes_wgrad_ok(cin, cp, 1) and ops.planes_dgrad_ok(cin, cp):
                u.cpad = cp
                u.wTp_pad_off, u.wTp_pad_bytes = region(ops.planes_bytes(cin, cp))
        if u.planes_fwd:
            u.wp_off, u.wp_bytes = region(ops.planes_bytes(u.cout, taps * cin))
        if u.planes_dgrad:
            u.wTp_off, u.wTp_bytes = region(ops.planes_bytes(cin, taps * u.cout))
    g.wplanes_total = total

# ... 82 lines not shown
```

Before: 1068.

## Fuse Adam update into weight-gradient kernel epilogue for plane-based convs

For conv layers whose weight gradient uses the planes path, the wgrad kernel now applies the Adam update to params, m and v directly in its epilogue instead of accumulating into dw. The remaining parameters (biases, BN, other kernels) go through a chunked Adam kernel driven by a chunk table stored after the hyperparameter buffer. The goal is to avoid writing and re-reading the full gradient buffer and to skip the separate full-size optimizer pass. It is on by default through YOLO_FUSED_UPDATE, and it changes step ordering, gradient zeroing and the graph-capture key, which adds correctness risk around split-K slabs and distributed reduction.

```diff
diff --git a/include/yolo_hip.h b/include/yolo_hip.h
--- a/include/yolo_hip.h
+++ b/include/yolo_hip.h
@@ -114,6 +114,8 @@
                                  void* stream);
 int yolo_conv2d_wgrad_planes(const yolo_conv_desc* d, const void* x_planes, const void* dy_planes,
                              float* dw, void* stream);
+int yolo_conv2d_wgrad_planes_adam(const yolo_conv_desc* d, const void* x_planes, const void* dy_planes, float* dw,
+                                  float* p, float* m, float* v, const float* hyper, void* stream);
 
 size_t yolo_wgrad_workspace_bytes(void);
 int yolo_set_wgrad_workspace(void* p, size_t bytes);
@@ -253,6 +255,7 @@
 int yolo_adam_step(float* p, float* g, float* m, float* v, long long n, float lr, float beta1,
                    float beta2, float eps, int step, float grad_scale, int zero_grad, void* stream);
 float yolo_adam_lr_t(float lr, float beta1, float beta2, int step);
+#define YOLO_ADAM_CHUNKED 2
 int yolo_adam_step_dev(float* p, float* g, float* m, float* v, long long n, const float* hyper, int zero_grad, void* stream);
 int yolo_sgd_step(float* p, float* g, long long n, float lr, float grad_scale, int zero_grad,
                   void* stream);
diff --git a/tf2_yolo_amd/_lib.py b/tf2_yolo_amd/_lib.py
--- a/tf2_yolo_amd/_lib.py
+++ b/tf2_yolo_amd/_lib.py
@@ -87,6 +87,7 @@
     "yolo_conv2d_fwd_absmax": (c_int, [POINTER(ConvDesc), _P, _P, _P, _P, _P, _P, _P]),
     "yolo_conv2d_dgrad_planes": (c_int, [POINTER(ConvDesc), _P, _P, _P, c_int, _P]),
     "yolo_conv2d_wgrad_planes": (c_int, [POINTER(ConvDesc), _P, _P, _P, _P]),
+    "yolo_conv2d_wgrad_planes_adam": (c_int, [POINTER(ConvDesc), _P, _P, _P, _P, _P, _P, _P, _P]),
     "yolo_wgrad_workspace_bytes": (c_size_t, []),
     "yolo_set_wgrad_workspace": (c_int, [_P, c_size_t]),
     "yolo_bn_stats": (c_int, [_P, _LL, c_int, _P, _P]),
diff --git a/tf2_yolo_amd/capture.py b/tf2_yolo_amd/capture.py
--- a/tf2_yolo_amd/capture.py
+++ b/tf2_yolo_amd/capture.py
@@ -42,7 +42,7 @@
     @staticmethod
     def key_of(model, x):
         return (tuple(x.shape), getattr(model.net, "alloc_gen", 0), tuple(id(l) for l in model.loss), id(model.optimizer),
-                id(model._reducer), model.net.anchors_trainable)
+                id(model._reducer), model.net.anchors_trainable, model.fuses_update())
 
     def _capture(self, net, opt):
         model = self.model
@@ -82,12 +82,13 @@
                 outs = net.forward(self.x, training=True)
                 for i, (o, yt) in enumerate(zip(outs, self.ys)):
                     model.loss[i].fwd_bwd(yt, o, grad_scale=1.0, dpred=model._dpred[i], loss_out=model._loss_bufs[i])
-                net.backward(model._dpred)
+                fused = model.fuses_update()
+                model._backward_and_update(fused)
                 net._dyp_events = [None, None]
                 if red is not None:
                     end(("finish",))
                     begin()
-                opt.step_captured()
+                opt.step_captured(**({"fused": True} if fused else {}))
                 end(None)
         except Exception:
             _LEAKED.extend(g for g, _ in self.segments)
@@ -127,6 +128,7 @@
                     dist.all_reduce(net.anchor_grads, group=red.pg)
                 red.finish()
         net.mark_params_changed()
+        net.grads_dirty = False
         return model._loss_bufs
 
 
@@ -152,13 +154,14 @@
             outs = net.forward(self.x, training=True)
             for i, (o, yt) in enumerate(zip(outs, self.ys)):
                 model.loss[i].fwd_bwd(yt, o, grad_scale=1.0, dpred=model._dpred[i], loss_out=model._loss_bufs[i])
-            net.backward(model._dpred)
+            fused = model.fuses_update()
+            model._backward_and_update(fused)
             if red is not None:
                 if net.anchors_trainable and red.world > 1:
                     import torch.distributed as dist
                     tape_mod.host_call(lambda: dist.all_reduce(net.anchor_grads, group=red.pg))
                 tape_mod.host_call(red.finish)
-            opt.step_captured()
+            opt.step_captured(**({"fused": True} if fused else {}))
         finally:
             tape_mod.ACTIVE = None
         net.mark_params_changed()
@@ -170,4 +173,5 @@
         opt.refresh_hyper(grad_scale=(1.0 / red.world) if red is not None else 1.0)
         self.tape.replay()
         net.mark_params_changed()
+        net.grads_dirty = False
         return model._loss_bufs
diff --git a/tf2_yolo_amd/csrc/adam_update.hpp b/tf2_yolo_amd/csrc/adam_update.hpp
--- /dev/null
+++ b/tf2_yolo_amd/csrc/adam_update.hpp
@@ -0,0 +1,47 @@
+#pragma once
+#include "common.hpp"
+
+namespace yolo {
+
+struct AdamArgs {
+  float lr_t, b1, b2, eps;
+};
+
+template <bool AMSGRAD>
+__device__ __forceinline__ void adam_update(float& p, float& m, float& v, float& vhat, float gg, const AdamArgs& h) {
+#pragma clang fp contract(off)
+  m = fmaf(h.b1, m, (1.f - h.b1) * gg);
+  v = fmaf(h.b2, v, ((1.f - h.b2) * gg) * gg);
+  if (AMSGRAD) {
+    vhat = fmaxf(vhat, v);
+    p -= (h.lr_t * m) / (sqrtf(vhat) + h.eps);
+  } else {
+    p -= (h.lr_t * m) / (sqrtf(v) + h.eps);
+  }
+}
+
+__device__ __forceinline__ void adam_apply_rows(float* __restrict__ p, float* __restrict__ m, float* __restrict__ v,
+                                                long long ld, const f32x4& g, int n, const float* __restrict__ hyper) {
+#pragma clang fp contract(off)
+  const AdamArgs h = {hyper[0], hyper[1], hyper[2], hyper[3]};
+  const float gs = hyper[4];
+  float pp[4], mm[4], vv[4];
+#pragma unroll
+  for (int e = 0; e < 4; ++e)
+    if (e < n) {
+      pp[e] = p[e * ld];
+      mm[e] = m[e * ld];
+      vv[e] = v[e * ld];
+    }
+#pragma unroll
+  for (int e = 0; e < 4; ++e)
+    if (e < n) {
+      float unused = 0.f;
+      adam_update<false>(pp[e], mm[e], vv[e], unused, g[e] * gs, h);
+      p[e * ld] = pp[e];
+      m[e * ld] = mm[e];
+      v[e * ld] = vv[e];
+    }
+}
+
+}
diff --git a/tf2_yolo_amd/csrc/conv.hip b/tf2_yolo_amd/csrc/conv.hip
--- a/tf2_yolo_amd/csrc/conv.hip
+++ b/tf2_yolo_amd/csrc/conv.hip
@@ -1267,6 +1267,26 @@
   return launch_wgrad_planes(a, as_stream(stream));
 }
 
+extern "C" int yolo_conv2d_wgrad_planes_adam(const yolo_conv_desc* d, const void* x_planes, const void* dy_planes, float* dw,
+                                             float* p, float* m, float* v, const float* hyper, void* stream) {
+  if (int rc = validate_desc(d)) return rc;
+  YOLO_REQUIRE(x_planes && dy_planes && dw && p && m && v && hyper, "conv_wgrad_planes_adam: null pointer");
+  WgradArgs a{};
+  a.src = reinterpret_cast<const float*>(x_planes);
+  a.dy = reinterpret_cast<const float*>(dy_planes);
+  a.dw = dw;
+  a.upd_p = p;
+  a.upd_m = m;
+  a.upd_v = v;
+  a.upd_hyper = hyper;
+  fill_wgrad_args(d, a);
+  YOLO_REQUIRE(wgrad_planes_supported(a),
+               "conv_wgrad_planes_adam: needs Cin %% 16 == 0, Cout %% 16 == 0, Cout >= 32 and kh*kw*Cin >= 64");
+  if (int rc = launch_wgrad_planes(a, as_stream(stream))) return rc;
+  if (a.slabs != nullptr) return YOLO_OK;
+  return yolo_adam_step_dev(p, dw, m, v, (long long)d->Cout * a.ldw, hyper, 1, stream);
+}
+
 extern "C" int yolo_conv2d_wgrad(const yolo_conv_desc* d, const float* x, const float* dy, float* dw, float* dbias,
                                  void* stream) {
   if (int rc = validate_desc(d)) return rc;
diff --git a/tf2_yolo_amd/csrc/conv_args.hpp b/tf2_yolo_amd/csrc/conv_args.hpp
--- a/tf2_yolo_amd/csrc/conv_args.hpp
+++ b/tf2_yolo_amd/csrc/conv_args.hpp
@@ -105,6 +105,10 @@
   int zero_blk_src, zero_blk_dy;
   float* slabs;
   int splits;
+  float* upd_p;
+  float* upd_m;
+  float* upd_v;
+  const float* upd_hyper;
 };
 
 int launch_gather_split(GatherConvArgs& a, hipStream_t st);
diff --git a/tf2_yolo_amd/csrc/conv_wgrad_planes.hip b/tf2_yolo_amd/csrc/conv_wgrad_planes.hip
--- a/tf2_yolo_amd/csrc/conv_wgrad_planes.hip
+++ b/tf2_yolo_amd/csrc/conv_wgrad_planes.hip
@@ -1,4 +1,5 @@
 #include "planes.hpp"
+#include "adam_update.hpp"
 #include <type_traits>
 #include <cstdlib>
 
@@ -296,6 +297,14 @@
   const float unscale =
       reinterpret_cast<const float*>(reinterpret_cast<const unsigned char*>(a.dy) + a.dy_bytes - PL_HEADER)[2] *
       reinterpret_cast<const float*>(reinterpret_cast<const unsigned char*>(a.src) + a.src_bytes - PL_HEADER)[2];
+  if (a.upd_p != nullptr) {
+    f32x4 g;
+#pragma unroll
+    for (int e = 0; e < 4; ++e) g[e] = 0.f + t[e] * unscale;
+    const long long at = (long long)co * a.ldw + cj;
+    adam_apply_rows(a.upd_p + at, a.upd_m + at, a.upd_v + at, a.ldw, g, a.Cout - co, a.upd_hyper);
+    return;
+  }
 #pragma unroll
   for (int e = 0; e < 4; ++e)
     if (co + e < a.Cout) a.dw[(long long)(co + e) * a.ldw + cj] += t[e] * unscale;
diff --git a/tf2_yolo_amd/csrc/conv_wgrad_win.hip b/tf2_yolo_amd/csrc/conv_wgrad_win.hip
--- a/tf2_yolo_amd/csrc/conv_wgrad_win.hip
+++ b/tf2_yolo_amd/csrc/conv_wgrad_win.hip
@@ -1,4 +1,5 @@
 #include "planes.hpp"
+#include "adam_update.hpp"
 #include <cstdlib>
 
 namespace yolo {
@@ -493,6 +494,14 @@
   const float unscale =
       reinterpret_cast<const float*>(reinterpret_cast<const unsigned char*>(a.dy) + a.dy_bytes - PL_HEADER)[2] *
       reinterpret_cast<const float*>(reinterpret_cast<const unsigned char*>(a.src) + a.src_bytes - PL_HEADER)[2];
+  if (a.upd_p != nullptr) {
+    f32x4 g;
+#pragma unroll
+    for (int e = 0; e < 4; ++e) g[e] = 0.f + sum[e] * unscale;
+    const long long at = (long long)co * a.ldw + cj;
+    adam_apply_rows(a.upd_p + at, a.upd_m + at, a.upd_v + at, a.ldw, g, 4, a.upd_hyper);
+    return;
+  }
 #pragma unroll
   for (int e = 0; e < 4; ++e) a.dw[(long long)(co + e) * a.ldw + cj] += sum[e] * unscale;
 }
@@ -747,6 +756,14 @@
   const float unscale =
       reinterpret_cast<const float*>(reinterpret_cast<const unsigned char*>(a.dy) + a.dy_bytes - PL_HEADER)[2] *
       reinterpret_cast<const float*>(reinterpret_cast<const unsigned char*>(a.src) + a.src_bytes - PL_HEADER)[2];
+  if (a.upd_p != nullptr) {
+    f32x4 g;
+#pragma unroll
+    for (int e = 0; e < 4; ++e) g[e] = 0.f + sum[e] * unscale;
+    const long long at = (long long)co * a.ldw + cj;
+    adam_apply_rows(a.upd_p + at, a.upd_m + at, a.upd_v + at, a.ldw, g, 4, a.upd_hyper);
+    return;
+  }
 #pragma unroll
   for (int e = 0; e < 4; ++e) a.dw[(long long)(co + e) * a.ldw + cj] += sum[e] * unscale;
 }
diff --git a/tf2_yolo_amd/csrc/elementwise.hip b/tf2_yolo_amd/csrc/elementwise.hip
--- a/tf2_yolo_amd/csrc/elementwise.hip
+++ b/tf2_yolo_amd/csrc/elementwise.hip
@@ -1,4 +1,5 @@
 #include "common.hpp"
+#include "adam_update.hpp"
 #include "planes.hpp"
 #include <cfloat>
 
@@ -421,16 +422,59 @@
   if ((threadIdx.x & 63) == 0) atomicAdd(&danchors[slot], (float)(s / (double)anchors[slot]));
 }
 
+__device__ __forceinline__ void adam_chunks(float* __restrict__ p, float* __restrict__ g, float* __restrict__ m,
+                                            float* __restrict__ v, long long n, const float* __restrict__ hyper, int zero) {
+  const AdamArgs h = {hyper[0], hyper[1], hyper[2], hyper[3]};
+  const float gs = hyper[4];
+  const int chunks = (int)hyper[7];
+  const unsigned* table = reinterpret_cast<const unsigned*>(hyper + 8);
+  for (int c = blockIdx.x; c < chunks; c += gridDim.x) {
+    const long long off = table[2 * c], len = table[2 * c + 1];
+    if (off + len > n) continue;
+    const long long n4 = (off & 3) == 0 ? len >> 2 : 0;
+    for (long long i = threadIdx.x; i < n4; i += blockDim.x) {
+      f32x4 pv = reinterpret_cast<f32x4*>(p + off)[i];
+      const f32x4 gv = reinterpret_cast<f32x4*>(g + off)[i];
+      f32x4 mv = reinterpret_cast<f32x4*>(m + off)[i];
+      f32x4 vv = reinterpret_cast<f32x4*>(v + off)[i];
+#pragma unroll
+      for (int e = 0; e < 4; ++e) {
+        float pp = pv[e], mm = mv[e], v1 = vv[e], unused = 0.f;
+        adam_update<false>(pp, mm, v1, unused, gv[e] * gs, h);
+        pv[e] = pp;
+        mv[e] = mm;
+        vv[e] = v1;
+      }
+      reinterpret_cast<f32x4*>(p + off)[i] = pv;
+      reinterpret_cast<f32x4*>(m + off)[i] = mv;
+      reinterpret_cast<f32x4*>(v + off)[i] = vv;
+      if (zero) reinterpret_cast<f32x4*>(g + off)[i] = f32x4{0.f, 0.f, 0.f, 0.f};
+    }
+    for (long long i = off + (n4 << 2) + threadIdx.x; i < off + len; i += blockDim.x) {
+      float pp = p[i], mm = m[i], v1 = v[i], unused = 0.f;
+      adam_update<false>(pp, mm, v1, unused, g[i] * gs, h);
+      p[i] = pp;
+      m[i] = mm;
+      v[i] = v1;
+      if (zero) g[i] = 0.f;
+    }
+  }
+}
+
 __global__ __launch_bounds__(256) void adam_kernel(float* __restrict__ p, float* __restrict__ g,
                                                    float* __restrict__ m, float* __restrict__ v, long long n,
                                                    float lr_t, float b1, float b2, float eps, float gs, int zero,
-                                                   const float* __restrict__ hyper) {
+                                                   const float* __restrict__ hyper, int chunked) {
   if (hyper != nullptr) {
     lr_t = hyper[0];
     b1 = hyper[1];
     b2 = hyper[2];
     eps = hyper[3];
     gs = hyper[4];
+  }
+  if (chunked) {
+    adam_chunks(p, g, m, v, n, hyper, zero);
+    return;
   }
   const long long n4 = n >> 2;
   for (long long i = (long long)blockIdx.x * blockDim.x + threadIdx.x; i < n4; i += (long long)gridDim.x * blockDim.x) {
@@ -685,7 +729,7 @@
   YOLO_REQUIRE(p && g && m && v && n > 0 && step >= 1, "adam_step: bad args");
   const double lr_t = (double)lr * sqrt(1.0 - pow((double)beta2, (double)step)) / (1.0 - pow((double)beta1, (double)step));
   hipLaunchKernelGGL(adam_kernel, dim3(stream_grid(n / 4 + 1, 256)), dim3(256), 0, as_stream(stream), p, g, m, v, n,
-                     (float)lr_t, beta1, beta2, eps, grad_scale, zero_grad, (const float*)nullptr);
+                     (float)lr_t, beta1, beta2, eps, grad_scale, zero_grad, (const float*)nullptr, 0);
   return check_launch("adam_kernel");
 }
 
@@ -695,9 +739,9 @@
 
 extern "C" int yolo_adam_step_dev(float* p, float* g, float* m, float* v, long long n, const float* hyper, int zero_grad,
                                   void* stream) {
-  YOLO_REQUIRE(p && g && m && v && hyper && n > 0, "adam_step_dev: bad args");
+  YOLO_REQUIRE(p && g && m && v && hyper && n > 0 && (zero_grad & ~(1 | YOLO_ADAM_CHUNKED)) == 0, "adam_step_dev: bad args");
   hipLaunchKernelGGL(adam_kernel, dim3(stream_grid(n / 4 + 1, 256)), dim3(256), 0, as_stream(stream), p, g, m, v, n, 0.f,
-                     0.f, 0.f, 0.f, 0.f, zero_grad, hyper);
+                     0.f, 0.f, 0.f, 0.f, zero_grad & 1, hyper, (zero_grad & YOLO_ADAM_CHUNKED) != 0);
   return check_launch("adam_kernel");
 }
 
diff --git a/tf2_yolo_amd/csrc/optim.hip b/tf2_yolo_amd/csrc/optim.hip
--- a/tf2_yolo_amd/csrc/optim.hip
+++ b/tf2_yolo_amd/csrc/optim.hip
@@ -1,5 +1,6 @@
 #include <cmath>
 #include "common.hpp"
+#include "adam_update.hpp"
 
 #pragma clang fp contract(off)
 
@@ -94,21 +95,6 @@
   k.value = mode == CLIP_VALUE;
   k.c = mode == CLIP_NORM ? factors[var] : mode == CLIP_GLOBAL ? factors[0] : 1.f;
   return k;
-}
-
-struct AdamArgs {
-  float lr_t, b1, b2, eps;
-};
-template <bool AMSGRAD>
-__device__ __forceinline__ void adam_update(float& p, float& m, float& v, float& vhat, float gg, const AdamArgs& h) {
-  m = fmaf(h.b1, m, (1.f - h.b1) * gg);
-  v = fmaf(h.b2, v, ((1.f - h.b2) * gg) * gg);
-  if (AMSGRAD) {
-    vhat = fmaxf(vhat, v);
-    p -= (h.lr_t * m) / (sqrtf(vhat) + h.eps);
-  } else {
-    p -= (h.lr_t * m) / (sqrtf(v) + h.eps);
-  }
 }
 
 template <bool AMSGRAD>
diff --git a/tf2_yolo_amd/engine.py b/tf2_yolo_amd/engine.py
--- a/tf2_yolo_amd/engine.py
+++ b/tf2_yolo_amd/engine.py
@@ -242,6 +242,21 @@
 
 def _epilogue(u):
     return _EPILOGUES.get(u.act, ops.EPI_AFFINE)
+
+
+def declare_params(units, params, state):
+    for u in units:
+        if u.kind == "conv":
+            u.p_kernel = params.add(f"{u.name}_conv/kernel", (u.cout, u.k, u.k, u.src.c), u.kernel_init)
+            u.p_bias = params.add(f"{u.name}_conv/bias", (u.cout,), init_zeros) if u.bias else None
+            if u.bn:
+                u.p_gamma = params.add(f"{u.name}_bn/gamma", (u.cout,), init_ones)
+                u.p_beta = params.add(f"{u.name}_bn/beta", (u.cout,), init_zeros)
+                u.s_mean = state.add(f"{u.name}_bn/moving_mean", (u.cout,), init_zeros)
+                u.s_var = state.add(f"{u.name}_bn/moving_variance", (u.cout,), init_ones)
+        elif u.kind == "head":
+            u.p_kernel = params.add(f"{u.name}/kernel", (u.cout, 1, 1, u.src.c), u.kernel_init)
+            u.p_bias = params.add(f"{u.name}/bias", (u.cout,), init_zeros)
 
 
 class Network:
@@ -271,6 +286,10 @@
         self.params.materialize(self.device, rng)
         self.state.materialize(self.device, rng)
         self.grads = torch.zeros_like(self.params.data)
+        self._fused_ranges, self._tail_chunks = plan.fused_update_plan(
+            self.units, [(n, self.params.specs[n].offset, self.params.specs[n].size) for n in self.params.order])
+        self._upd = None
+        self.grads_dirty = False
         self._init_anchors()
         ops.create_side_streams(self.device)
         ops.ensure_conv_workspace()
@@ -296,18 +315,7 @@
             u.concat_reads_through = False
 
     def _declare_params(self):
-        for u in self.units:
-            if u.kind == "conv":
-                u.p_kernel = self.params.add(f"{u.name}_conv/kernel", (u.cout, u.k, u.k, u.src.c), u.kernel_init)
-                u.p_bias = self.params.add(f"{u.name}_conv/bias", (u.cout,), init_zeros) if u.bias else None
-                if u.bn:
-                    u.p_gamma = self.params.add(f"{u.name}_bn/gamma", (u.cout,), init_ones)
-                    u.p_beta = self.params.add(f"{u.name}_bn/beta", (u.cout,), init_zeros)
-                    u.s_mean = self.state.add(f"{u.name}_bn/moving_mean", (u.cout,), init_zeros)
-                    u.s_var = self.state.add(f"{u.name}_bn/moving_variance", (u.cout,), init_ones)
-            elif u.kind == "head":
-                u.p_kernel = self.params.add(f"{u.name}/kernel", (u.cout, 1, 1, u.src.c), u.kernel_init)
-                u.p_bias = self.params.add(f"{u.name}/bias", (u.cout,), init_zeros)
+        declare_params(self.units, self.params, self.state)
 
     def _init_anchors(self):
         self._anchors_dev, self._anchor_grad_views = {}, {}
@@ -810,6 +818,11 @@
         if self._wT_event is not None:
             tape.wait_event(torch.cuda.current_stream(), self._wT_event)
             self._wT_event = None
+        if self._upd is None:
+            self.grads_dirty = True
+        elif self._wp_event is not None:
+            tape.wait_event(torch.cuda.current_stream(), self._wp_event)
+            self._wp_event = None
         self._refresh_wT()
         self._refresh_wTplanes()
         for u in self.units:
@@ -869,7 +882,12 @@
 
     def _filter_and_data_grad(self, u, dy, dyp, dbias, grads):
         with self._beside_backward(dy):
-            if u.planes_wgrad:
+            if u.planes_wgrad and self._upd is not None and u.name in self._fused_ranges:
+                k = u.p_kernel
+                p, m, v = (t[k.offset:k.offset + k.size] for t in self._upd[:3])
+                ops.conv2d_wgrad_planes_adam(u.desc, self._xplanes[u.src.tid], dyp, self._gview(k), p, m, v, self._upd[3],
+                                             dy=dy, dbias=dbias)
+            elif u.planes_wgrad:
                 ops.conv2d_wgrad_planes(u.desc, self._xplanes[u.src.tid], dyp, self._gview(u.p_kernel), dy=dy, dbias=dbias)
             else:
                 ops.conv2d_wgrad(u.desc, self.act[u.src.tid], dy, self._gview(u.p_kernel), dbias)
@@ -956,6 +974,14 @@
         if ev is not None:
             self._dyp_events[self._dyp_idx] = ev
         self._wgrad_pending = True
+
+    @contextlib.contextmanager
+    def fused_update(self, m, v, hyper):
+        self._upd = (self.params.data, m, v, hyper)
+        try:
+            yield
+        finally:
+            self._upd = None
 
     def _join_wgrad(self):
         if self._wgrad_pending:
diff --git a/tf2_yolo_amd/model.py b/tf2_yolo_amd/model.py
--- a/tf2_yolo_amd/model.py
+++ b/tf2_yolo_amd/model.py
@@ -335,6 +335,18 @@
                 _ops.zero_bytes(self.net.grads)
             return None
 
+    def fuses_update(self):
+        net = self.net
+        return bool(net._fused_update and getattr(self.optimizer, "fusable", False) and self._reducer is None
+                    and net.grad_ready_hook is None and not net.grads_dirty)
+
+    def _backward_and_update(self, fused):
+        if not fused:
+            return self.net.backward(self._dpred)
+        opt = self.optimizer
+        with self.net.fused_update(opt.m, opt.v, opt._hyper_buffers()[1]):
+            self.net.backward(self._dpred)
+
     def train_step_device(self, x, y_list, with_metrics=False):
         if self.optimizer is None:
             raise YoloHipError("compile() the model before training")
@@ -343,6 +355,9 @@
             bufs = self._captured_step(x, y_list)
             if bufs is not None:
                 return bufs, None
+        fused = self.fuses_update()
+        if fused:
+            self.optimizer.begin_step()
         outs = self.net.forward(x, training=True)
         if self._dpred is None or self._dpred[0].shape != outs[0].shape:
             self._dpred = [torch.empty_like(o) for o in outs]
@@ -351,7 +366,10 @@
         mvals = None
         if with_metrics:
             mvals = [[m(yt, o) for m in ms] for ms, o, yt in zip(self.metrics, outs, y_list)]
-        self.net.backward(self._dpred)
+        self._backward_and_update(fused)
+        if fused:
+            self.optimizer.finish_step()
+            return self._loss_bufs, mvals
         if self._reducer is not None and self.net.anchors_trainable and self._reducer.world > 1:
             import torch.distributed as dist
             dist.all_reduce(self.net.anchor_grads, group=self._reducer.pg)
diff --git a/tf2_yolo_amd/ops.py b/tf2_yolo_amd/ops.py
--- a/tf2_yolo_amd/ops.py
+++ b/tf2_yolo_amd/ops.py
@@ -541,6 +541,28 @@
     return dw
 
 
+def conv2d_wgrad_planes_adam(d, xp, dyp, dw, p, m, v, hyper, dy=None, dbias=None):
+    _chk_f32(dw, dy, dbias, p, m, v)
+    _chk_hyper(hyper)
+    n = d.Cout * d.kh * d.kw * d.Cin
+    if any(t.numel() != n for t in (dw, p, m, v)):
+        raise YoloHipError("conv2d_wgrad_planes_adam: dw / p / m / v size does not match the descriptor")
+    if xp.numel() < planes_bytes(d.N * d.H * d.W, d.Cin) or dyp.numel() < planes_bytes(d.N * d.Ho * d.Wo, d.Cout):
+        raise YoloHipError("conv2d_wgrad_planes_adam: planes buffers do not match the descriptor")
+    def run():
+        check(_lib.load().yolo_conv2d_wgrad_planes_adam(byref(d), _p(xp), _p(dyp), _p(dw), _p(p), _p(m), _p(v), _p(hyper),
+                                                        _stream()), "yolo_conv2d_wgrad_planes_adam")
+    if TIMER is not None:
+        TIMER.bracket(_conv_flops(d), run, _layer_key(d, "wgrad"))
+    else:
+        run()
+    if dbias is not None:
+        if dy is None:
+            raise YoloHipError("conv2d_wgrad_planes_adam: dbias needs the fp32 dy")
+        check(_lib.load().yolo_conv2d_wgrad_bias(_p(dy), d.N * d.Ho * d.Wo, d.Cout, _p(dbias), _stream()),
+              "yolo_conv2d_wgrad_bias")
+
+
 def conv2d_wgrad_bias(dy, rows, c, dbias):
     _chk_f32(dy, dbias)
     if dy.numel() != rows * c or dbias.numel() != c:
@@ -947,9 +969,27 @@
     return float(_lib.load().yolo_adam_lr_t(float(lr), float(beta1), float(beta2), int(step)))
 
 
-def adam_step_dev(p, g, m, v, hyper, zero_grad=True):
-    check(_lib.load().yolo_adam_step_dev(_p(p), _p(g), _p(m), _p(v), p.numel(), _p(hyper), int(zero_grad), _stream()),
+ADAM_CHUNKED = 2
+
+
+def adam_step_dev(p, g, m, v, hyper, zero_grad=True, chunked=False):
+    flags = int(bool(zero_grad))
+    if chunked:
+        _chk_hyper(hyper)
+        flags |= ADAM_CHUNKED
+    check(_lib.load().yolo_adam_step_dev(_p(p), _p(g), _p(m), _p(v), p.numel(), _p(hyper), flags, _stream()),
           "yolo_adam_step_dev")
+
+
+def adam_tail_hyper(chunks, device="cuda"):
+    import numpy as np
+    table = np.asarray(list(chunks), dtype=np.int64).reshape(-1, 2)
+    if len(table) >= 1 << 24 or (len(table) and (table.min() < 0 or (table[:, 0] + table[:, 1]).max() >= 1 << 32)):
+        raise YoloHipError("adam_tail_hyper: chunk table out of range")
+    buf = torch.zeros(OPT_HYPER + 2 * len(table), dtype=torch.float32, device=device)
+    if len(table):
+        buf[OPT_HYPER:].view(torch.int32).copy_(torch.from_numpy(table.astype(np.uint32).view(np.int32).reshape(-1)))
+    return buf, len(table)
 
 
 def sgd_step(p, g, lr, grad_scale=1.0, zero_grad=True):
diff --git a/tf2_yolo_amd/optimizers/__init__.py b/tf2_yolo_amd/optimizers/__init__.py
--- a/tf2_yolo_amd/optimizers/__init__.py
+++ b/tf2_yolo_amd/optimizers/__init__.py
@@ -59,6 +59,7 @@
     def bind(self, net):
         self.net = net
         self._anch = None
+        self._hyper_dev = None
         if not self._extended:
             return
         p = net.params
@@ -85,8 +86,11 @@
         if getattr(self, "_hyper_dev", None) is None:
             self._hyper_host = torch.zeros(self._HYPER_SLOTS, ops.OPT_HYPER, dtype=torch.float32).pin_memory()
             self._hyper_events = [None] * self._HYPER_SLOTS
-            self._hyper_dev = torch.zeros(ops.OPT_HYPER, dtype=torch.float32, device="cuda")
+            self._hyper_dev, self._tail_n = self._alloc_hyper_dev()
         return self._hyper_host, self._hyper_dev
+
+    def _alloc_hyper_dev(self):
+        return torch.zeros(ops.OPT_HYPER, dtype=torch.float32, device="cuda"), 0
 
     def _fill_hyper(self, host, grad_scale):
         raise NotImplementedError
@@ -99,7 +103,8 @@
             self._hyper_events[slot].synchronize()
         host = ring[slot]
         self._fill_hyper(host, float(grad_scale))
-        dev.copy_(host, non_blocking=True)
+        host[7] = self._tail_n
+        dev[:ops.OPT_HYPER].copy_(host, non_blocking=True)
         ev = torch.cuda.Event()
         ev.record(torch.cuda.current_stream())
         self._hyper_events[slot] = ev
@@ -161,7 +166,22 @@
             s.update({"vhat": self.vhat, "anchors/vhat": self.avhat})
         return s
 
+    @property
+    def fusable(self):
+        return not self._extended
+
+    def _alloc_hyper_dev(self):
+        return ops.adam_tail_hyper(self.net._tail_chunks)
+
+    def begin_step(self, grad_scale=1.0):
+        self.refresh_hyper(grad_scale)
+
+    def finish_step(self):
+        self.step_captured(fused=True)
+        self.net.mark_params_changed()
+
     def step(self, grad_scale=1.0):
+        self.net.grads_dirty = False
         if self._extended:
             return self._extended_step(grad_scale)
         self.iterations += 1
@@ -179,11 +199,12 @@
         host[1], host[2], host[3], host[4] = self.beta_1, self.beta_2, self.epsilon, grad_scale
         host[5], host[6] = 0.0, self._clip_threshold
 
-    def step_captured(self):
+    def step_captured(self, fused=False):
         _, dev = self._hyper_buffers()
         net = self.net
+        net.grads_dirty = False
         if not self._extended:
-            ops.adam_step_dev(net.params.data, net.grads, self.m, self.v, dev, zero_grad=True)
+            ops.adam_step_dev(net.params.data, net.grads, self.m, self.v, dev, zero_grad=True, chunked=fused)
             if self._with_anchors():
                 ops.adam_step_dev(net.anchors_flat, net.anchor_grads, self.am, self.av, dev, zero_grad=True)
             return
@@ -223,6 +244,7 @@
         return {"momentum": self.a, "anchors/momentum": self.aa} if self.a is not None else {}
 
     def step(self, grad_scale=1.0):
+        self.net.grads_dirty = False
         if self._extended:
             return self._extended_step(grad_scale)
         self.iterations += 1
@@ -240,6 +262,7 @@
     def step_captured(self):
         _, dev = self._hyper_buffers()
         net = self.net
+        net.grads_dirty = False
         f, fa = self._enqueue_clip(dev)
         nesterov = self.nesterov and self.a is not None
         ops.sgd_step_clip(net.params.data, net.grads, self._table, dev, accum=self.a, nesterov=nesterov, factors=f,
diff --git a/tf2_yolo_amd/plan.py b/tf2_yolo_amd/plan.py
--- a/tf2_yolo_amd/plan.py
+++ b/tf2_yolo_amd/plan.py
@@ -32,6 +32,7 @@
         o.infer_onepass = on("YOLO_INFER_ONEPASS")
         o.infer_small_fuse = on("YOLO_INFER_SMALL_FUSE")
         o.dgrad_classes = on("YOLO_DGRAD_CLASSES")
+        o.fused_update = on("YOLO_FUSED_UPDATE")
         return o
 
 
@@ -66,6 +67,24 @@
     _plan_fp32_copies(g, units, opts)
     _plan_bounds(g, units, tensors)
     return g
+
+
+def fusable_update(u):
+    return has_filter(u) and bool(u.planes_wgrad) and not u.cpad
+
+
+def kernel_name(u):
+    return f"{u.name}_conv/kernel" if u.kind == "conv" else f"{u.name}/kernel"
+
+
+def fused_update_plan(units, variables, chunk=None):
+    chunk = ops.OPT_CHUNK if chunk is None else int(chunk)
+    where = {name: (int(off), int(size)) for name, off, size in variables}
+    fused = {u.name: where[kernel_name(u)] for u in units if fusable_update(u)}
+    taken = {off for off, _ in fused.values()}
+    rest = [(off, size) for _, off, size in variables if int(off) not in taken]
+    off, ln, _, _ = ops.build_chunk_table(rest, chunk)
+    return fused, [(int(o), int(n)) for o, n in zip(off, ln)]
 
 
 def _plan_param_buffers(g, units):
```

Result: no change. 1074, median of 6 (+0.6%).
